# dmuley/sph-code

Hardware: AMD Instinct MI355X
Metric: particle-steps/sec + achieved HBM GB/s, 10^6-particle 3D sphere, 1/2/4/8 GPUs (higher is better)
Workload: dtype f64

## Files before the change

### include/sphx.h

```cpp
#ifndef SPHX_H
#define SPHX_H

#include <stddef.h>
#include <stdint.h>

#ifdef __cplusplus
extern "C" {
#endif

#define SPHX_OK            0
#define SPHX_E_ARG        -1
#define SPHX_E_HIP        -2
#define SPHX_E_NOMEM      -3
#define SPHX_E_STATE      -4

#define SPHX_MAX_K        64
#define SPHX_MAX_SPECIES  32

typedef struct sphx_ctx sphx_ctx;

typedef struct sphx_constants {
    double k_B;
    double amu;
    double m_h;
    double m_0;
    double dt_0;
    double max_age;
    double pos_clamp;
} sphx_constants;

typedef struct sphx_stats {
    double ms_grid;
    double ms_search;
    double ms_prep;
    double ms_density;
    double ms_pi;
    double ms_visc;
    double ms_integrate;
    double ms_total;
    int64_t n;
    int64_t steps;
    int64_t candidates;
    int64_t retries;
    int64_t cells;
    int64_t refresh_steps;
    int64_t rebuild_steps;
    double  cell_size;
    double  ms_gravity;
    int64_t fallback_queries;
    double  ms_species;
    int64_t short_rows;
    int64_t detail_steps;
    int64_t far_queries;
    int64_t outlier_levels;
    int64_t bad_accel;
    int64_t bad_energy;
    int64_t bad_state;
    int64_t bad_h;
    int64_t search_steps;
} sphx_stats;

int         sphx_create(sphx_ctx** out, int device);
void        sphx_destroy(sphx_ctx* ctx);
const char* sphx_last_error(const sphx_ctx* ctx);
int         sphx_version(void);
const char* sphx_build_info(void);
const char* sphx_tunables(const sphx_ctx* ctx);
int sphx_selftest_scan(sphx_ctx* ctx, int n, unsigned seed, long long* mismatches, int* single_launch);
int sphx_selftest_mfma_cull(sphx_ctx* ctx, double E, int blocks, unsigned seed, double* max_err_over_E2,
                            double* wrong_signs, double* kappa);
int         sphx_host_alloc(void** out, size_t bytes);
int         sphx_host_free(void* p);
int         sphx_set_constants(sphx_ctx* ctx, const sphx_constants* c);
int         sphx_get_constants(const sphx_ctx* ctx, sphx_constants* c);
int         sphx_set_tuning(sphx_ctx* ctx, double rscale, double cell_factor);
int         sphx_set_timing_detail(sphx_ctx* ctx, int on);
int         sphx_set_incremental(sphx_ctx* ctx, int verlet, double rscale_build);

int sphx_neighbors(sphx_ctx* ctx, int64_t n, int k, const double* points, double dist,
                   double eps, int64_t* idx, double* dist_out, int64_t* nontriv, double* h);

int sphx_hydro_update(sphx_ctx* ctx, int64_t n, int k, int s, const int64_t* neighbor,
                      const double* points, const double* mass, const double* sizes,
                      const double* f_un, const double* particle_type, const double* T,
                      const double* mu_array, const double* gamma_array,
                      const double* velocities, int visc_mode,
                      double* hydro_accel, double* visc_accel, double* visc_heat,
                      double* rho, double* nden, double* f_un_nb, double* rho_dust);

int sphx_density(sphx_ctx* ctx, int64_t n, int k, const double* points, const double* mass,
                 const double* particle_type, const int64_t* neighbor, double d, double* out);
int sphx_dust_density(sphx_ctx* ctx, int64_t n, int k, const double* points, const double* mass,
                      const int64_t* neighbor, const double* particle_type, const double* sizes,
                      double* out);
int sphx_num_dens(sphx_ctx* ctx, int64_t n, int k, const double* mass, const double* points,
                  const double* mu_array, const int64_t* neighbor, double d, double* out);
int sphx_del_pressure(sphx_ctx* ctx, int64_t n, int k, const double* points, const double* mass,
                      const double* particle_type, const int64_t* neighbor,
                      const double* E_internal, const double* gamma_array, double d,
                      double* out );
int sphx_artificial_viscosity(sphx_ctx* ctx, int64_t n, int k, const int64_t* neighbor,
                              const double* points, const double* particle_type,
                              const double* sizes, const double* mass, const double* densities,
                              const double* velocities, const double* T,
                              const double* gamma_array, const double* mu_array, double d,
                              double* visc_accel , double* visc_heat );
int sphx_crossing_time(sphx_ctx* ctx, int64_t n, int k, const int64_t* neighbor,
                       const double* velocities, const double* sizes,
                       const double* particle_type, double* out );
int sphx_net_impulse(sphx_ctx* ctx, int64_t n, int k, const double* points, const double* mass,
                     const double* sizes, const double* velocities, const double* particle_type,
                     const int64_t* neighbor, const double* mean_grain_mass,
                     const double* mean_cross, double* accel_onto ,
                     double* accel_reaction );

int sphx_gravity_direct(sphx_ctx* ctx, int64_t n, const double* mass, const double* points,
                        const double* sizes, double softening, double G, double* accel);

int sphx_gravity_tree(sphx_ctx* ctx, int64_t n, const double* mass, const double* points,
                      const double* sizes, double softening, double G, int ws, int k_cells,
                      double* accel);

int sphx_agb_yields(sphx_ctx* ctx, int64_t n, const double* masses, const double* metallicities,
                    int nspl, const int32_t* ntx, const int32_t* nty, const double* tx,
                    const double* ty, const double* coeffs, const int32_t* mapto, double divisor,
                    int nspecies, const double* mu_specie, const double* composition,
                    double solar_mass, double* dust_out ,
                    double* gas_out );

int sphx_dt_rule(sphx_ctx* ctx, int64_t n, const double* ct, const int32_t* first, double* dt);
int sphx_clamp_arrays(sphx_ctx* ctx, int64_t n, double* points, double* velocities);
int sphx_leapfrog(sphx_ctx* ctx, int64_t n, double* points, double* velocities, double* total_accel,
                  const double* old_accel, double* E_internal, double* T, const double* mass,
                  const double* mu, const double* gamma, const double* ptype, const double* grav_accel,
                  const double* delp, const double* densities, const double* dust_densities,
                  const double* drag_on_gas, const double* drag_reaction, const double* av_accel,
                  const double* av_heat, double dt);

int sphx_state_upload(sphx_ctx* ctx, int64_t n, int s, const double* pos, const double* vel,
                      const double* mass, const double* ptype, const double* f_un,
                      const double* T, const double* mu, const double* gamma,
                      const double* E_internal, const double* accel_old);
int sphx_state_set_drag(sphx_ctx* ctx, const double* mean_grain_mass, const double* mean_cross);
int sphx_state_set_agb(sphx_ctx* ctx, int nspl, const int32_t* ntx, const int32_t* nty, const double* tx,
                       const double* ty, const double* coeffs, const int32_t* mapto, double divisor,
                       const double* mu_specie, double solar_mass);
int sphx_state_download_species(sphx_ctx* ctx, double* F, double* Z, double* agb_dust);
int sphx_state_set_loop_forms(sphx_ctx* ctx, int on, double d);
int sphx_set_clip_grad(sphx_ctx* ctx, int on);
int sphx_set_visc_mode(sphx_ctx* ctx, int mode);
int sphx_state_set_gravity(sphx_ctx* ctx, int mode, double G);
int sphx_set_gravity_order(sphx_ctx* ctx, int order);
int sphx_step(sphx_ctx* ctx, int nsteps, int k, double dist, int first, double fixed_dt);
int sphx_state_download(sphx_ctx* ctx, double* pos, double* vel, double* accel,
                        double* E_internal, double* T, double* sizes, double* rho,
                        double* nden, double* visc_heat, double* dt_last);
int sphx_state_download_pressure(sphx_ctx* ctx, double* pressure);
int sphx_get_stats(sphx_ctx* ctx, sphx_stats* out);
int sphx_reset_stats(sphx_ctx* ctx);

int sphx_set_stream(sphx_ctx* ctx, void* hip_stream );
int sphx_reset_stream(sphx_ctx* ctx);
int sphx_sync(sphx_ctx* ctx);
int sphx_dev_set_mean_h(sphx_ctx* ctx, double mean_h);
int sphx_dev_search(sphx_ctx* ctx, int64_t n_total, int64_t n_owned, int k, const double* pos,
                    const double* hint, double rscale, double dist, double* h_out);
int sphx_dev_get_order(sphx_ctx* ctx, int64_t n_total, int32_t* out);
int sphx_dev_prep(sphx_ctx* ctx, const double* pos, const double* vel, const double* mass,
                  const double* h, const double* T, const double* mu, const double* gamma,
                  const double* ptype);
int sphx_dev_density(sphx_ctx* ctx, double* rho, double* rho_dust, double* nden, double* hydro_accel);
int sphx_dev_pi(sphx_ctx* ctx, const double* rho_complete, double* Pi, double* Bw, double* ct_out);
int sphx_dev_visc(sphx_ctx* ctx, const double* Bw_complete, const double* mass, double* visc_accel,
                  double* visc_heat);
int sphx_dev_visc_pairwise(sphx_ctx* ctx, const double* rho_complete, const double* mass, double* visc_accel,
                           double* visc_heat, double* ct_out);
int sphx_dev_clamp(sphx_ctx* ctx, int64_t n, double* pos, double* vel);
int sphx_dev_pack_rows(sphx_ctx* ctx, int64_t n, const int64_t* idx, int nf, const double* const* fields,
                       const int32_t* widths, double* rows);
int sphx_dev_regroup(sphx_ctx* ctx, int64_t n_sel, const int64_t* sel, int64_t n_rows, const double* rows,
                     int nf, const double* const* fields_in, const int32_t* widths,
                     double* const* fields_out);
int sphx_dev_need_map(sphx_ctx* ctx, int64_t n, const double* pos, const double* w, const double* g_lo,
                      double g_cs, int G, unsigned char* out);
int sphx_dev_integrate_auto(sphx_ctx* ctx, int64_t n_owned, double* pos, double* vel, double* accel_old,
                            double* E_internal, double* T, const double* mass, const double* mu,
                            const double* gamma, const double* ptype, const double* hydro_accel,
                            const double* visc_accel, const double* visc_heat, const double* red2,
                            int first, double fixed_dt, double* dt_out);
int sphx_dev_loop_prep(sphx_ctx* ctx, const double* pos, const double* vel, const double* mass, const double* T,
                       const double* mu, const double* gamma, const double* ptype, const double* E_internal, double d);
int sphx_dev_loop_pass1(sphx_ctx* ctx, const double* h_complete, double* rho, double* rho_dust, double* nden, double* delp);
int sphx_dev_loop_pass2(sphx_ctx* ctx, const double* rho_complete, double* visc_accel, double* visc_heat, double* ct_out);
int sphx_dev_loop_pass2_interior(sphx_ctx* ctx);
int sphx_dev_set_reach_cap(sphx_ctx* ctx, double cap);
int sphx_dev_select_blobs(sphx_ctx* ctx, int part);
int sphx_dev_blob_split_counts(sphx_ctx* ctx, int32_t counts[3]);
int sphx_dev_integrate_loop(sphx_ctx* ctx, int64_t n_owned, double* pos, double* vel, double* accel_old,
                            double* E_internal, double* T, const double* mass, const double* mu, const double* gamma,
                            const double* ptype, const double* delp, const double* rho, const double* av_accel,
                            const double* av_heat, const double* red2, int first, double fixed_dt, double dt,
                            double* dt_out);
int sphx_dev_drag(sphx_ctx* ctx, const double* mass, const double* ptype, const double* mean_grain_mass,
                  const double* mean_cross, double* drag_on, double* drag_reaction);
int sphx_dev_set_drag_terms(sphx_ctx* ctx, const double* drag_on, const double* drag_reaction, const double* rho,
                            const double* rho_dust);
int sphx_dev_set_agb(sphx_ctx* ctx, int nspecies, int nspl, const int32_t* ntx, const int32_t* nty, const double* tx,
                     const double* ty, const double* coeffs, const int32_t* mapto, double divisor,
                     const double* mu_specie, double solar_mass);
int sphx_dev_species(sphx_ctx* ctx, int nspecies, const double* f_un, const double* mass, double* F, double* Z,
                     double* agb_dust);
int sphx_dev_reach(sphx_ctx* ctx, int64_t n, const double* h, const double* vel, double halo_scale,
                   double skin_frac, double dt_last, double* w);
int sphx_dev_reach_dt(sphx_ctx* ctx, int64_t n, const double* h, const double* vel, double halo_scale,
                      double skin_frac, const double* dt_dev, double* w);
int sphx_dev_plan_mask(sphx_ctx* ctx, int64_t n, const double* pos, const double* g_lo, double g_cs, int G,
                       int world, int rank, const unsigned char* maps, unsigned char* mask, int64_t* counts);
int sphx_dev_step_scalars(sphx_ctx* ctx, int64_t n_owned, const double* h, const double* w_plan, double D,
                          double hclip, const double* ct, double* out4);
int sphx_dev_integrate(sphx_ctx* ctx, int64_t n_owned, double* pos, double* vel, double* accel_old,
                       double* E_internal, double* T, const double* mass, const double* mu,
                       const double* gamma, const double* ptype, const double* hydro_accel,
                       const double* visc_accel, const double* visc_heat, double dt);

#ifdef __cplusplus
}
#endif
#endif
```

### sph-code_amd/_lib.py

```python
import ctypes as C
import os
import threading
import weakref

import numpy as np

HERE = os.path.dirname(os.path.abspath(__file__))
LIB_PATH = os.environ.get("SPHX_LIB") or os.path.join(HERE, "libsphx.so")

c_double_p = C.POINTER(C.c_double)
c_int64_p = C.POINTER(C.c_int64)


class SphxConstants(C.Structure):
    _fields_ = [(n, C.c_double) for n in ("k_B", "amu", "m_h", "m_0", "dt_0", "max_age", "pos_clamp")]


class SphxStats(C.Structure):
    _fields_ = [(n, C.c_double) for n in ("ms_grid", "ms_search", "ms_prep", "ms_density", "ms_pi",
                                          "ms_visc", "ms_integrate", "ms_total")] + \
               [(n, C.c_int64) for n in ("n", "steps", "candidates", "retries", "cells", "refresh_steps",
                                         "rebuild_steps")] + \
               [("cell_size", C.c_double), ("ms_gravity", C.c_double), ("fallback_queries", C.c_int64),
                ("ms_species", C.c_double), ("short_rows", C.c_int64), ("detail_steps", C.c_int64), ("far_queries", C.c_int64),
                ("outlier_levels", C.c_int64), ("bad_accel", C.c_int64), ("bad_energy", C.c_int64), ("bad_state", C.c_int64),
                ("bad_h", C.c_int64), ("search_steps", C.c_int64)]

    def as_dict(self):
        return {n: getattr(self, n) for n, _ in self._fields_}


SPHX_E_STATE = -4
_P = C.c_void_p
_D = c_double_p
_I = c_int64_p
SIGNATURES = {
    "sphx_create": (C.c_int, [C.POINTER(_P), C.c_int]),
    "sphx_destroy": (None, [_P]),
    "sphx_last_error": (C.c_char_p, [_P]),
    "sphx_version": (C.c_int, []),
    "sphx_build_info": (C.c_char_p, []),
    "sphx_tunables": (C.c_char_p, [_P]),
    "sphx_selftest_scan": (C.c_int, [_P, C.c_int, C.c_uint, C.POINTER(C.c_longlong), C.POINTER(C.c_int)]),
    "sphx_selftest_mfma_cull": (C.c_int, [_P, C.c_double, C.c_int, C.c_uint, _D, _D, _D]),
    "sphx_host_alloc": (C.c_int, [C.POINTER(_P), C.c_size_t]),
    "sphx_host_free": (C.c_int, [_P]),
    "sphx_set_constants": (C.c_int, [_P, C.POINTER(SphxConstants)]),
    "sphx_get_constants": (C.c_int, [_P, C.POINTER(SphxConstants)]),
    "sphx_set_tuning": (C.c_int, [_P, C.c_double, C.c_double]),
    "sphx_set_incremental": (C.c_int, [_P, C.c_int, C.c_double]),
    "sphx_neighbors": (C.c_int, [_P, C.c_int64, C.c_int, _D, C.c_double, C.c_double, _I, _D, _I, _D]),
    "sphx_hydro_update": (C.c_int, [_P, C.c_int64, C.c_int, C.c_int, _I] + [_D] * 9 + [C.c_int] + [_D] * 7),
    "sphx_density": (C.c_int, [_P, C.c_int64, C.c_int, _D, _D, _D, _I, C.c_double, _D]),
    "sphx_dust_density": (C.c_int, [_P, C.c_int64, C.c_int, _D, _D, _I, _D, _D, _D]),
    "sphx_num_dens": (C.c_int, [_P, C.c_int64, C.c_int, _D, _D, _D, _I, C.c_double, _D]),
    "sphx_del_pressure": (C.c_int, [_P, C.c_int64, C.c_int, _D, _D, _D, _I, _D, _D, C.c_double, _D]),
    "sphx_artificial_viscosity": (C.c_int, [_P, C.c_int64, C.c_int, _I] + [_D] * 9 + [C.c_double, _D, _D]),
    "sphx_crossing_time": (C.c_int, [_P, C.c_int64, C.c_int, _I, _D, _D, _D, _D]),
    "sphx_net_impulse": (C.c_int, [_P, C.c_int64, C.c_int, _D, _D, _D, _D, _D, _I, _D, _D, _D, _D]),
    "sphx_agb_yields": (C.c_int, [_P, C.c_int64, _D, _D, C.c_int, C.POINTER(C.c_int32), C.POINTER(C.c_int32), _D, _D, _D,
                                  C.POINTER(C.c_int32), C.c_double, C.c_int, _D, _D, C.c_double, _D, _D]),
    "sphx_dt_rule": (C.c_int, [_P, C.c_int64, _D, C.POINTER(C.c_int32), _D]),
    "sphx_clamp_arrays": (C.c_int, [_P, C.c_int64, _D, _D]),
    "sphx_leapfrog": (C.c_int, [_P, C.c_int64] + [_D] * 18 + [C.c_double]),
    "sphx_state_upload": (C.c_int, [_P, C.c_int64, C.c_int] + [_D] * 10),
    "sphx_state_set_drag": (C.c_int, [_P, _D, _D]),
    "sphx_state_set_agb": (C.c_int, [_P, C.c_int, C.POINTER(C.c_int32), C.POINTER(C.c_int32), _D, _D, _D,
                                     C.POINTER(C.c_int32), C.c_double, _D, C.c_double]),
    "sphx_state_download_species": (C.c_int, [_P, _D, _D, _D]),
    "sphx_state_set_loop_forms": (C.c_int, [_P, C.c_int, C.c_double]),
    "sphx_set_clip_grad": (C.c_int, [_P, C.c_int]),
    "sphx_set_visc_mode": (C.c_int, [_P, C.c_int]),
    "sphx_state_set_gravity": (C.c_int, [_P, C.c_int, C.c_double]),
    "sphx_set_gravity_order": (C.c_int, [_P, C.c_int]),
    "sphx_gravity_direct": (C.c_int, [_P, C.c_int64, _D, _D, _D, C.c_double, C.c_double, _D]),
    "sphx_gravity_tree": (C.c_int, [_P, C.c_int64, _D, _D, _D, C.c_double, C.c_double, C.c_int, C.c_int, _D]),
    "sphx_step": (C.c_int, [_P, C.c_int, C.c_int, C.c_double, C.c_int, C.c_double]),
    "sphx_state_download": (C.c_int, [_P] + [_D] * 10),
    "sphx_state_download_pressure": (C.c_int, [_P, _D]),
    "sphx_get_stats": (C.c_int, [_P, C.POINTER(SphxStats)]),
    "sphx_reset_stats": (C.c_int, [_P]),
    "sphx_set_stream": (C.c_int, [_P, C.c_void_p]),
    "sphx_reset_stream": (C.c_int, [_P]),
    "sphx_sync": (C.c_int, [_P]),
    "sphx_dev_set_mean_h": (C.c_int, [_P, C.c_double]),
    "sphx_dev_search": (C.c_int, [_P, C.c_int64, C.c_int64, C.c_int, _P, _P, C.c_double, C.c_double, _P]),
    "sphx_dev_get_order": (C.c_int, [_P, C.c_int64, _P]),
    "sphx_dev_prep": (C.c_int, [_P] + [_P] * 8),
    "sphx_dev_density": (C.c_int, [_P] + [_P] * 4),
    "sphx_dev_pi": (C.c_int, [_P] + [_P] * 4),
    "sphx_dev_visc": (C.c_int, [_P] + [_P] * 4),
    "sphx_dev_visc_pairwise": (C.c_int, [_P] + [_P] * 5),
    "sphx_dev_clamp": (C.c_int, [_P, C.c_int64, _P, _P]),
    "sphx_dev_pack_rows": (C.c_int, [_P, C.c_int64, _P, C.c_int, C.POINTER(C.c_void_p), C.POINTER(C.c_int32), _P]),
    "sphx_dev_regroup": (C.c_int, [_P, C.c_int64, _P, C.c_int64, _P, C.c_int, C.POINTER(C.c_void_p),
                                   C.POINTER(C.c_int32), C.POINTER(C.c_void_p)]),
    "sphx_dev_need_map": (C.c_int, [_P, C.c_int64, _P, _P, C.POINTER(C.c_double), C.c_double, C.c_int, _P]),
    "sphx_dev_integrate_auto": (C.c_int, [_P, C.c_int64] + [_P] * 13 + [C.c_int, C.c_double, _P]),
    "sphx_dev_reach": (C.c_int, [_P, C.c_int64, _P, _P, C.c_double, C.c_double, C.c_double, _P]),
    "sphx_set_timing_detail": (C.c_int, [_P, C.c_int]),
    "sphx_dev_reach_dt": (C.c_int, [_P, C.c_int64, _P, _P, C.c_double, C.c_double, _P, _P]),
    "sphx_dev_plan_mask": (C.c_int, [_P, C.c_int64, _P, C.POINTER(C.c_double), C.c_double, C.c_int, C.c_int, C.c_int, _P, _P, _P]),
    "sphx_dev_step_scalars": (C.c_int, [_P, C.c_int64, _P, _P, C.c_double, C.c_double, _P, _P]),
    "sphx_dev_integrate": (C.c_int, [_P, C.c_int64] + [_P] * 12 + [C.c_double]),
    "sphx_dev_drag": (C.c_int, [_P] + [_P] * 6),
    "sphx_dev_set_drag_terms": (C.c_int, [_P] + [_P] * 4),
    "sphx_dev_set_agb": (C.c_int, [_P, C.c_int, C.c_int, C.POINTER(C.c_int32), C.POINTER(C.c_int32), _D, _D, _D,
                                   C.POINTER(C.c_int32), C.c_double, _D, C.c_double]),
    "sphx_dev_species": (C.c_int, [_P, C.c_int] + [_P] * 5),
    "sphx_dev_loop_prep": (C.c_int, [_P] + [_P] * 8 + [C.c_double]),
    "sphx_dev_loop_pass1": (C.c_int, [_P] + [_P] * 5),
    "sphx_dev_loop_pass2": (C.c_int, [_P] + [_P] * 4),
    "sphx_dev_loop_pass2_interior": (C.c_int, [_P]),
    "sphx_dev_set_reach_cap": (C.c_int, [_P, C.c_double]),
    "sphx_dev_select_blobs": (C.c_int, [_P, C.c_int]),
    "sphx_dev_blob_split_counts": (C.c_int, [_P, _P]),
    "sphx_dev_integrate_loop": (C.c_int, [_P, C.c_int64] + [_P] * 14 + [C.c_int, C.c_double, C.c_double, _P]),
}

_lib = None
_lock = threading.Lock()


def load_library():
    global _lib
    with _lock:
        if _lib is not None:
            return _lib
        if not os.path.exists(LIB_PATH):
            raise RuntimeError(
                "libsphx.so is not built (%s). Run `python -c 'import __graft_entry__ as g; g.build()'` "
                "or `python sph-code_amd/build.py`. There is no CPU fallback." % LIB_PATH)
        lib = C.CDLL(LIB_PATH)
        for name, (res, args) in SIGNATURES.items():
            fn = getattr(lib, name)
            fn.restype = res
            fn.argtypes = args
        _lib = lib
        return lib


def f64(a, shape=None):
    out = np.ascontiguousarray(a, dtype=np.float64)
    if shape is not None and out.shape != shape:
        raise ValueError("expected shape %s, got %s" % (shape, out.shape))
    return out


def i64(a, shape=None):
    out = np.ascontiguousarray(a, dtype=np.int64)
    if shape is not None and out.shape != shape:
        raise ValueError("expected shape %s, got %s" % (shape, out.shape))
    return out


class _PinnedPool:
    MIN_BYTES = 8 << 20
    KEEP_PER_SIZE = 3

    def __init__(self):
        self.free = {}
        self.lock = threading.Lock()

    def empty(self, shape, dtype):
        dtype = np.dtype(dtype)
        nbytes = int(np.prod(shape)) * dtype.itemsize
        if nbytes < self.MIN_BYTES:
            return np.empty(shape, dtype)
        with self.lock:
            lst = self.free.get(nbytes)
            ptr = lst.pop() if lst else None
        if ptr is None:
            lib = load_library()
            p = _P()
            if lib.sphx_host_alloc(C.byref(p), nbytes) != 0 or not p.value:
                return np.empty(shape, dtype)
            ptr = p.value
        buf = (C.c_byte * nbytes).from_address(ptr)
        weakref.finalize(buf, self._release, ptr, nbytes)
        return np.frombuffer(buf, dtype=dtype).reshape(shape)

    def _release(self, ptr, nbytes):
        with self.lock:
            lst = self.free.setdefault(nbytes, [])
            if len(lst) < self.KEEP_PER_SIZE:
                lst.append(ptr)
                return
        try:
            load_library().sphx_host_free(_P(ptr))
        except Exception:
            pass


pinned = _PinnedPool()


def dp(a):
    return None if a is None else a.ctypes.data_as(c_double_p)


def ip(a):
    return None if a is None else a.ctypes.data_as(c_int64_p)


class Context:

    def __init__(self, device=None):
        self.lib = load_library()
        if device is None:
            device = int(os.environ.get("LOCAL_RANK", "0"))
        self.device = device
        h = C.c_void_p()
        rc = self.lib.sphx_create(C.byref(h), device)
        if rc != 0 or not h:
            raise RuntimeError("sphx_create(device=%d) failed with %d: no usable MI355X/HIP device "
                               "(libsphx has no CPU path)" % (device, rc))
        self.h = h

    def close(self):
        if getattr(self, "h", None):
            self.lib.sphx_destroy(self.h)
            self.h = None

    def __del__(self):
        try:
            self.close()
        except Exception:
            pass

    def check(self, rc):
        if rc == 0:
            return
        msg = self.lib.sphx_last_error(self.h)
        msg = msg.decode() if msg else ""
        if rc == -1:
            raise ValueError("libsphx: " + msg)
        raise RuntimeError("libsphx error %d: %s" % (rc, msg))

    def constants(self):
        c = SphxConstants()
        self.check(self.lib.sphx_get_constants(self.h, C.byref(c)))
        return c

    def set_constants(self, **kw):
        c = self.constants()
        for k_, v in kw.items():
            setattr(c, k_, v)
        self.check(self.lib.sphx_set_constants(self.h, C.byref(c)))

    def set_tuning(self, rscale=0.0, cell_factor=0.0):
        self.check(self.lib.sphx_set_tuning(self.h, float(rscale), float(cell_factor)))

    def set_incremental(self, verlet=True, rscale_build=0.0):
        self.check(self.lib.sphx_set_incremental(self.h, 1 if verlet else 0, float(rscale_build)))

    def stats(self):
        s = SphxStats()
        self.check(self.lib.sphx_get_stats(self.h, C.byref(s)))
        return s.as_dict()

    def reset_stats(self):
        self.check(self.lib.sphx_reset_stats(self.h))

    def build_info(self):
        return {"library": self.lib.sphx_build_info().decode(), "tunables": self.lib.sphx_tunables(self.h).decode(),
                "lib_path": LIB_PATH}

    def set_timing_detail(self, on=True):
        self.check(self.lib.sphx_set_timing_detail(self.h, 1 if on else 0))


_default = None


def default_context():
    global _default
    if _default is None:
        _default = Context()
    return _default
```

### sph-code_amd/csrc/sphx_api.hip

```cpp
#include "sphx_internal.h"
#include <stdarg.h>
#include <stdlib.h>
#include <new>

int sphx_set_err(sphx_ctx* ctx, int code, const char* fmt, ...) {
    if (ctx) {
        va_list ap;
        va_start(ap, fmt);
        vsnprintf(ctx->err, sizeof(ctx->err), fmt, ap);
        va_end(ap);
    }
    return code;
}

void sphx_release(sphx_ctx* ctx, DevBuf& b) {
    for (size_t q = 0; q < ctx->allocs.size(); ++q)
        if (ctx->allocs[q] == b.p) { ctx->allocs[q] = ctx->allocs.back(); ctx->allocs.pop_back(); break; }
    if (b.p) (void)hipFree(b.p);
    b.p = nullptr;
    b.cap = 0;
}

int sphx_ensure(sphx_ctx* ctx, DevBuf& b, size_t bytes, hipStream_t in_use_on) {
    if (bytes == 0) bytes = 8;
    if (b.cap >= bytes) return SPHX_OK;
    if (b.p) {
        HIPCHK(hipStreamSynchronize(in_use_on));
        sphx_release(ctx, b);
    }
    size_t want = bytes + bytes / 8 + 256;
    hipError_t e = hipMalloc(&b.p, want);
    if (e != hipSuccess) {
        b.p = nullptr;
        return sphx_set_err(ctx, SPHX_E_NOMEM, "hipMalloc(%zu) failed: %s", want, hipGetErrorString(e));
    }
    b.cap = want;
    ctx->allocs.push_back(b.p);
    return SPHX_OK;
}

static void default_constants(sphx_constants* c) {
    c->k_B = 1.380649e-23;
    c->amu = 1.66053906892e-27;
    c->m_h = 1.0008 * c->amu;
    c->m_0 = 31.622776601683793 * 1.989e30;
    c->dt_0 = 60. * 60. * 24. * 365. * 250000.;
    c->max_age = 3e7 * 60. * 60. * 24. * 365.;
    c->pos_clamp = 1e11 * 149597870700.0;
}

extern "C" int sphx_version(void) { return 100; }

extern "C" const char* sphx_build_info(void) { return "gfx950 experiments=0"; }
extern "C" const char* sphx_tunables(const sphx_ctx* ctx) { return ctx ? ctx->tunables : ""; }

extern "C" int sphx_host_alloc(void** out, size_t bytes) {
    if (!out) return SPHX_E_ARG;
    *out = nullptr;
    if (bytes == 0) bytes = 8;
    if (hipHostMalloc(out, bytes, hipHostMallocDefault) != hipSuccess) {
        (void)hipGetLastError();
        *out = nullptr;
        return SPHX_E_NOMEM;
    }
    return SPHX_OK;
}
extern "C" int sphx_host_free(void* p) {
    if (p && hipHostFree(p) != hipSuccess) return SPHX_E_HIP;
    return SPHX_OK;
}

static hipError_t sphx_stream_create(hipStream_t* st, int side) {
    int least = 0, greatest = 0;
    if (hipDeviceGetStreamPriorityRange(&least, &greatest) != hipSuccess) return hipStreamCreateWithFlags(st, hipStreamNonBlocking);
    return hipStreamCreateWithPriority(st, hipStreamNonBlocking, side ? least : greatest);
}

extern "C" int sphx_create(sphx_ctx** out, int device) {
    if (!out) return SPHX_E_ARG;
    *out = nullptr;
    int count = 0;
    if (hipGetDeviceCount(&count) != hipSuccess || count <= 0 || device < 0 || device >= count) {
        fprintf(stderr, "sphx_create: no usable HIP device %d (found %d). libsphx has no CPU path.\n",
                device, count);
        return SPHX_E_HIP;
    }
    sphx_ctx* ctx = new (std::nothrow) sphx_ctx();
    if (!ctx) return SPHX_E_NOMEM;
    ctx->device = device;
    memset(&ctx->stats, 0, sizeof(ctx->stats));
    memset(&ctx->grid, 0, sizeof(ctx->grid));
    default_constants(&ctx->cst);
    auto env = [&](const char* name) -> const char* {
        const char* e = getenv(name);
        if (e) {
            const size_t used = strlen(ctx->tunables);
            snprintf(ctx->tunables + used, sizeof(ctx->tunables) - used, "%s%s=%s", used ? " " : "", name, e);
        }
        return e;
    };
    if (const char* e = env("SPHX_RSCALE")) { double v = atof(e); if (v >= 1.0) ctx->rscale = v; }
    if (const char* e = env("SPHX_CELL")) { double v = atof(e); if (v > 0.0) ctx->cell_factor = v; }
    if (const char* e = env("SPHX_RSCALE_BUILD")) { double v = atof(e); if (v >= 1.0) ctx->rscale_build = v; }
    if (const char* e = env("SPHX_VERLET")) ctx->use_verlet = atoi(e) != 0;
    if (const char* e = env("SPHX_BLOB")) ctx->use_blob = atoi(e) != 0;
    if (const char* e = env("SPHX_BLOB_CURVE")) ctx->blob_curve = atoi(e);
    if (const char* e = env("SPHX_KNN_GROUP")) ctx->use_group = atoi(e) != 0;
    if (const char* e = env("SPHX_HCLIP")) { double v = atof(e); if (v > 1.0) ctx->h_clip_factor = v; }
    if (const char* e = env("SPHX_TIMING_DETAIL")) ctx->timing_detail = atoi(e) != 0;
    if (const char* e = env("SPHX_MAX_CELLS")) { long long v = atoll(e); if (v > 0) ctx->max_cells = v; }
    if (const char* e = env("SPHX_CELL_FEEDBACK")) ctx->cell_feedback = atoi(e) != 0;
    if (const char* e = env("SPHX_CELL_FB_HI")) ctx->cell_fb_hi = atof(e);
    if (const char* e = env("SPHX_CELL_FB_LO")) ctx->cell_fb_lo = atof(e);
    if (const char* e = env("SPHX_DRAG_LDS")) ctx->drag_lds = atoi(e) != 0;
    if (const char* e = env("SPHX_BLOB_SPLIT")) ctx->blob_split_on = atoi(e) != 0;
    if (const char* e = env("SPHX_SPECIES_FUSED")) ctx->species_fused = atoi(e) != 0;
    if (const char* e = env("SPHX_SPECIES_LDS")) ctx->species_lds = atoi(e) != 0;
    if (const char* e = env("SPHX_HINT_DISTRUST")) ctx->distrust_mode = atoi(e);
    if (const char* e = env("SPHX_OUTLIER_LEVELS")) ctx->olev_mode = atoi(e);
    if (const char* e = env("SPHX_BOX_SIGMAS")) { double v = atof(e); if (v >= 1.0) ctx->box_sigmas = v; }
    if (const char* e = env("SPHX_GRAV_KERNEL")) ctx->grav_per_thread = atoi(e) == 0;
    if (const char* e = env("SPHX_GRAV_ORDER")) { int v = atoi(e); if (v == 1 || v == 2) ctx->grav_order = v; }
    if (const char* e = env("SPHX_GRAV_WS")) { int v = atoi(e); if (v >= 1 && v <= 4) ctx->grav_ws = v; }
    if (const char* e = env("SPHX_LDS")) ctx->use_lds = atoi(e) != 0;
    if (const char* e = env("SPHX_BLOB_SLOTS")) ctx->blob_slots = atoi(e);
    if (const char* e = env("SPHX_BLOB_WGS")) {
        int cus = 256;
        (void)hipDeviceGetAttribute(&cus, hipDeviceAttributeMultiprocessorCount, ctx->device);
        if (atoi(e) > 0) ctx->blob_grid = ((cus * atoi(e) + 7) / 8) * 8;
    }
    bool ok = hipSetDevice(device) == hipSuccess &&
              sphx_stream_create(&ctx->stream, 0) == hipSuccess &&
              hipHostMalloc(&ctx->pinned, 16384, hipHostMallocDefault) == hipSuccess;
    ctx->own_stream = ctx->stream;
    for (int i = 0; ok && i < 10; ++i) ok = hipEventCreate(&ctx->ev[i]) == hipSuccess;
    for (int r = 0; ok && r < 3; ++r)
        for (int i = 0; ok && i < 10; ++i) ok = hipEventCreate(&ctx->evring[r][i]) == hipSuccess;
    for (int r = 0; ok && r < 2; ++r)
        ok = hipEventCreateWithFlags(&ctx->lag_bev[r], hipEventDisableTiming) == hipSuccess &&
             hipEventCreateWithFlags(&ctx->lag_hev[r], hipEventDisableTiming) == hipSuccess;
    if (ok) ok = sphx_stream_create(&ctx->side_stream, 1) == hipSuccess &&
                 hipEventCreateWithFlags(&ctx->ev_join, hipEventDisableTiming) == hipSuccess &&
                 hipEventCreateWithFlags(&ctx->ev_perm, hipEventDisableTiming) == hipSuccess;
    if (ok) ok = sphx_ensure(ctx, ctx->scal, SC_NSLOTS * 8) == SPHX_OK &&
                 hipMemsetAsync(ctx->scal.p, 0, SC_NSLOTS * 8, ctx->stream) == hipSuccess &&
                 sphx_ensure(ctx, ctx->badc, (size_t)BADC_BUCKETS * BADC_STRIDE * sizeof(u64)) == SPHX_OK &&
                 hipMemsetAsync(ctx->badc.p, 0, (size_t)BADC_BUCKETS * BADC_STRIDE * sizeof(u64), ctx->stream) == hipSuccess;
    if (!ok) {
        fprintf(stderr, "sphx_create: HIP initialisation failed on device %d\n", device);
        delete ctx;
        return SPHX_E_HIP;
    }
    *out = ctx;
    return SPHX_OK;
}

extern "C" void sphx_destroy(sphx_ctx* ctx) {
    if (!ctx) return;
    (void)hipSetDevice(ctx->device);
    if (ctx->stream) (void)hipStreamSynchronize(ctx->stream);
    for (void* p : ctx->allocs) (void)hipFree(p);
    for (int i = 0; i < 10; ++i)
        if (ctx->ev[i]) (void)hipEventDestroy(ctx->ev[i]);
    for (int r = 0; r < 3; ++r)
        for (int i = 0; i < 10; ++i)
            if (ctx->evring[r][i]) (void)hipEventDestroy(ctx->evring[r][i]);
    for (int r = 0; r < 2; ++r) {
        if (ctx->lag_bev[r]) (void)hipEventDestroy(ctx->lag_bev[r]);
        if (ctx->lag_hev[r]) (void)hipEventDestroy(ctx->lag_hev[r]);
    }
    if (ctx->pinned) (void)hipHostFree(ctx->pinned);
    if (ctx->olev_ev) (void)hipEventDestroy(ctx->olev_ev);
    if (ctx->ev_join) (void)hipEventDestroy(ctx->ev_join);
    if (ctx->ev_perm) (void)hipEventDestroy(ctx->ev_perm);
    if (ctx->side_stream) (void)hipStreamDestroy(ctx->side_stream);
    if (ctx->own_stream) (void)hipStreamDestroy(ctx->own_stream);
    delete ctx;
}

extern "C" const char* sphx_last_error(const sphx_ctx* ctx) { return ctx ? ctx->err : "null context"; }

extern "C" int sphx_set_constants(sphx_ctx* ctx, const sphx_constants* c) {
    if (!ctx || !c) return SPHX_E_ARG;
    ctx->cst = *c;
    return SPHX_OK;
}
extern "C" int sphx_set_tuning(sphx_ctx* ctx, double rscale, double cell_factor) {
    if (!ctx) return SPHX_E_ARG;
    if (rscale > 0.0) {
        if (rscale < 1.0) return sphx_set_err(ctx, SPHX_E_ARG, "rscale %g < 1", rscale);
        ctx->rscale = rscale;
    }
    if (cell_factor > 0.0) ctx->cell_factor = cell_factor;
    return SPHX_OK;
}
extern "C" int sphx_set_incremental(sphx_ctx* ctx, int verlet, double rscale_build) {
    if (!ctx) return SPHX_E_ARG;
    ctx->use_verlet = verlet != 0;
    if (!ctx->use_verlet) ctx->list_valid = false;
    if (rscale_build > 0.0) {
        if (rscale_build < 1.0) return sphx_set_err(ctx, SPHX_E_ARG, "rscale_build %g < 1", rscale_build);
        ctx->rscale_build = rscale_build;
    }
    return SPHX_OK;
}
extern "C" int sphx_get_constants(const sphx_ctx* ctx, sphx_constants* c) {
    if (!ctx || !c) return SPHX_E_ARG;
    *c = ctx->cst;
    return SPHX_OK;
}

static int upload(sphx_ctx* ctx, DevBuf& b, const void* host, size_t bytes) {
    SPHX_TRY(sphx_ensure(ctx, b, bytes));
    HIPCHK(hipMemcpyAsync(b.p, host, bytes, hipMemcpyHostToDevice, ctx->stream));
    return SPHX_OK;
}
static int download(sphx_ctx* ctx, void* host, const void* dev, size_t bytes) {
    if (!host) return SPHX_OK;
    HIPCHK(hipMemcpyAsync(host, dev, bytes, hipMemcpyDeviceToHost, ctx->stream));
    return SPHX_OK;
}

extern "C" int sphx_neighbors(sphx_ctx* ctx, int64_t n, int k, const double* points, double dist,
                              double eps, int64_t* idx, double* dist_out, int64_t* nontriv,
                              double* h) {
    (void)eps;
    if (!ctx) return SPHX_E_ARG;
    NEED(points);
    if (n < 1) return sphx_set_err(ctx, SPHX_E_ARG, "n=%lld < 1", (long long)n);
    if (k < 1 || k > SPHX_MAX_K) return sphx_set_err(ctx, SPHX_E_ARG, "N_NEIGH=%d not in 1..%d", k, SPHX_MAX_K);
    HIPCHK(hipSetDevice(ctx->device));
    ctx->map_perm = nullptr;
    ctx->qorder = nullptr;
    const size_t nb = (size_t)n * sizeof(double);
    SPHX_TRY(upload(ctx, ctx->in_a, points, 3 * nb));
    SPHX_TRY(sphx_ensure(ctx, ctx->in_b, nb));
    SPHX_TRY(sphx_ensure(ctx, ctx->in_c, nb));
    SPHX_TRY(sphx_ensure(ctx, ctx->in_d, nb));
    SPHX_TRY(sphx_ensure(ctx, ctx->in_e, nb));
    SPHX_TRY(sphx_ensure(ctx, ctx->in_f, nb));
    SPHX_TRY(sphx_ensure(ctx, ctx->in_g, nb));
    double *x = ctx->in_b.as<double>(), *y = ctx->in_c.as<double>(), *z = ctx->in_d.as<double>();
    double *xs = ctx->in_e.as<double>(), *ys = ctx->in_f.as<double>(), *zs = ctx->in_g.as<double>();
    SPHX_TRY(sphx_aos_to_soa3(ctx, n, ctx->in_a.as<double>(), x, y, z));
    ctx->clip_valid = false;
    SPHX_TRY(sphx_build_grid(ctx, n, k, x, y, z, 0.0));
    SPHX_TRY(sphx_gather3(ctx, n, ctx->perm.as<int>(), x, y, z, xs, ys, zs));
    SPHX_TRY(sphx_ensure(ctx, ctx->idx64, (size_t)n * k * sizeof(int64_t)));
    SPHX_TRY(sphx_ensure(ctx, ctx->dist_out, (size_t)n * k * sizeof(double)));
    SPHX_TRY(sphx_ensure(ctx, ctx->nontriv, (size_t)n * sizeof(int64_t)));
    SPHX_TRY(sphx_ensure(ctx, ctx->h_api, nb));
    KnnOut o;
    o.nbr = nullptr; o.h_sorted = nullptr;
    o.idx64 = ctx->idx64.as<int64_t>(); o.dist = ctx->dist_out.as<double>();
    o.nontriv = ctx->nontriv.as<int64_t>(); o.h_by_id = ctx->h_api.as<double>();
    KnnIn in;
    in.xs = xs; in.ys = ys; in.zs = zs;
    in.id = ctx->perm.as<int>();
    in.rbound = dist;
    SPHX_TRY(sphx_knn(ctx, n, k, in, o));
    SPHX_TRY(download(ctx, idx, o.idx64, (size_t)n * k * sizeof(int64_t)));
    SPHX_TRY(download(ctx, dist_out, o.dist, (size_t)n * k * sizeof(double)));
    SPHX_TRY(download(ctx, nontriv, o.nontriv, (size_t)n * sizeof(int64_t)));
    SPHX_TRY(download(ctx, h, o.h_by_id, nb));
    HIPCHK(hipStreamSynchronize(ctx->stream));
    return SPHX_OK;
}

extern "C" int sphx_hydro_update(sphx_ctx* ctx, int64_t n, int k, int s, const int64_t* neighbor,
                                 const double* points, const double* mass, const double* sizes,
                                 const double* f_un, const double* particle_type, const double* T,
                                 const double* mu_array, const double* gamma_array,
                                 const double* velocities, int visc_mode, double* hydro_accel,
                                 double* visc_accel, double* visc_heat, double* rho, double* nden,
                                 double* f_un_nb, double* rho_dust) {
    if (!ctx) return SPHX_E_ARG;
    NEED(points); NEED(mass); NEED(sizes); NEED(particle_type); NEED(T);
// ... 141 lines not shown
    if (!ctx->has_state) return sphx_set_err(ctx, SPHX_E_STATE, "sphx_state_set_loop_forms before sphx_state_upload");
    if (on && !(d > 0.0)) return sphx_set_err(ctx, SPHX_E_ARG, "the loop forms need the driver's global d > 0 (drv:68)");
    if (on && ctx->use_verlet) return sphx_set_err(ctx, SPHX_E_STATE, "loop-form steps are not combined with incremental search");
    if (on && ctx->visc_mode != 0)
        return sphx_set_err(ctx, SPHX_E_ARG, "loop-form steps have their own (pairwise) viscosity: visc_mode must be 0");
    ctx->loop_forms = on ? 1 : 0;
    ctx->loop_d = d;
    return SPHX_OK;
}

extern "C" int sphx_set_gravity_order(sphx_ctx* ctx, int order) {
    if (!ctx) return SPHX_E_ARG;
    if (order != 1 && order != 2) return sphx_set_err(ctx, SPHX_E_ARG, "gravity order %d not 1 (monopole) or 2 (quadrupole)", order);
    ctx->grav_order = order;
    return SPHX_OK;
}

extern "C" int sphx_set_clip_grad(sphx_ctx* ctx, int on) {
    if (!ctx) return SPHX_E_ARG;
    ctx->clip_grad = on ? 1 : 0;
    return SPHX_OK;
}

extern "C" int sphx_set_visc_mode(sphx_ctx* ctx, int mode) {
    if (!ctx) return SPHX_E_ARG;
    if (mode != 0 && mode != 1)
        return sphx_set_err(ctx, SPHX_E_ARG, "visc_mode %d unknown (0 = ref_axis0, 1 = pairwise)", mode);
    if (mode != 0 && ctx->loop_forms)
        return sphx_set_err(ctx, SPHX_E_ARG, "loop-form steps have their own (pairwise) viscosity: visc_mode must be 0");
    ctx->visc_mode = mode;
    return SPHX_OK;
}

extern "C" int sphx_state_set_gravity(sphx_ctx* ctx, int mode, double G) {
    if (!ctx) return SPHX_E_ARG;
    if (!ctx->has_state) return sphx_set_err(ctx, SPHX_E_STATE, "sphx_state_set_gravity before sphx_state_upload");
    if (mode < 0 || mode > 2) return sphx_set_err(ctx, SPHX_E_ARG, "gravity mode %d not in {0, 1, 2}", mode);
    if (mode == 2 && ctx->use_verlet)
        return sphx_set_err(ctx, SPHX_E_STATE, "tree gravity needs the cell grid of every step: not with incremental search");
    ctx->gravity = mode;
    ctx->grav_G = G;
    return SPHX_OK;
}

static PrepIn prep_in_of_state(const StateArrays& s) {
    PrepIn in;
    in.x = s.x.as<double>(); in.y = s.y.as<double>(); in.z = s.z.as<double>(); in.ps = 1;
    in.vx = s.vx.as<double>(); in.vy = s.vy.as<double>(); in.vz = s.vz.as<double>(); in.vs = 1;
    in.m = s.m.as<double>(); in.h = s.hprev.as<double>(); in.T = s.T.as<double>();
    in.mu = s.mu.as<double>(); in.gam = s.gam.as<double>(); in.ptype = s.ptype.as<double>();
    return in;
}

static int step_cell_hint(sphx_ctx* ctx, int64_t n, double* cell_hint) {
    *cell_hint = 0.0;
    if (ctx->step_count == 0) return SPHX_OK;
    const double* hs;
    if (ctx->lag_hvalid[ctx->lag_hslot]) {
        HIPCHK(hipEventSynchronize(ctx->lag_halias[ctx->lag_hslot] ? ctx->lag_halias[ctx->lag_hslot]
                                                                     : ctx->lag_hev[ctx->lag_hslot]));
        hs = (const double*)((char*)ctx->pinned + LAG_OFF + 512 * ctx->lag_hslot + 256);
        const u64* sv = (const u64*)hs;
        for (int q = 0; q < 10; ++q) ctx->knn_lag[q] = sv[(SC_NFAILQ - SC_HSUM) + q];
        ctx->knn_lag_valid = true;
    } else {
        HIPCHK(hipMemcpyAsync((char*)ctx->pinned + 256, ctx->scal.as<double>() + SC_HSUM, 4 * sizeof(double),
                              hipMemcpyDeviceToHost, ctx->stream));
        HIPCHK(hipStreamSynchronize(ctx->stream));
        hs = (const double*)((char*)ctx->pinned + 256);
    }
    const double hmean = hs[3] > 0.0 ? hs[0] / hs[3] : 0.0;
    if (hmean > 0.0 && isfinite(hmean)) {
        *cell_hint = ctx->cell_factor * sphx_cell_feedback(ctx, n) * hmean;
        ctx->h_clip = ctx->h_clip_factor * hmean;
    }
    return SPHX_OK;
}

static int step_search(sphx_ctx* ctx, int k, double dist, hipEvent_t* ev) {
    const int64_t n = ctx->n;
    if (ctx->use_verlet) SPHX_TRY(sphx_clamp(ctx, n, ctx->st));
    SPHX_TRY(sphx_ensure(ctx, ctx->nbr, (size_t)k * ctx->npad * sizeof(int)));
    if (ctx->use_verlet && ctx->list_valid && ctx->list_n == n && ctx->list_k == k) {
        StateArrays& r = ctx->st;
        HIPCHK(hipEventRecord(ev[1], ctx->stream));
        int64_t nfail = 0;
        SPHX_TRY(sphx_knn_refresh(ctx, n, k, r.x.as<double>(), r.y.as<double>(), r.z.as<double>(),
                                  ctx->nbr.as<int>(), r.hprev.as<double>(), &nfail));
        if (nfail == 0) {
            ctx->stats.refresh_steps++;
            return SPHX_OK;
        }
        ctx->list_valid = false;
    }
    double cell_hint = 0.0;
    SPHX_TRY(step_cell_hint(ctx, n, &cell_hint));
    {
        StateArrays& r = ctx->st;
        const bool blob = ctx->use_blob && !ctx->use_verlet;
        GridBuildOpts g;
        g.lagged = true;
        g.alias_ev = ev[1];
        g.sort_cells_later = blob;
        if (!ctx->use_verlet) { g.clamp_vel[0] = r.vx.as<double>(); g.clamp_vel[1] = r.vy.as<double>(); g.clamp_vel[2] = r.vz.as<double>(); }
        SPHX_TRY(sphx_build_grid(ctx, n, k, r.x.as<double>(), r.y.as<double>(), r.z.as<double>(), cell_hint, g));
        if (blob) SPHX_TRY(sphx_build_blob_order(ctx, n, true));
    }
    const bool split = ctx->side_stream && !ctx->use_verlet;
    SPHX_TRY(sphx_permute_state(ctx, n, split, ev[1]));
    StateArrays& r = ctx->st;
    KnnIn in;
    in.xs = r.x.as<double>(); in.ys = r.y.as<double>(); in.zs = r.z.as<double>();
    in.id = r.id.as<int>(); in.inv = ctx->inv.as<int>();
    in.rsearch = r.hprev.as<double>();
    in.hinted = ctx->step_count > 0 && !ctx->use_verlet;
    in.lag_external = true;
    in.rscale = ctx->rscale;
    in.rbound = dist;
    KnnOut o;
    o.nbr = ctx->nbr.as<int>();
    o.h_sorted = r.hprev.as<double>();
    o.idx64 = nullptr; o.dist = nullptr; o.nontriv = nullptr; o.h_by_id = nullptr;
    if (ctx->use_verlet) {
        SPHX_TRY(sphx_ensure(ctx, ctx->list64, (size_t)n * 64 * sizeof(int)));
        SPHX_TRY(sphx_ensure(ctx, ctx->dref, (size_t)n * sizeof(double)));
        o.list64 = ctx->list64.as<int>();
        o.dref = ctx->dref.as<double>();
        in.rscale = ctx->rscale_build;
    }
    SPHX_TRY(sphx_knn(ctx, n, k, in, o));
    if (split) HIPCHK(hipStreamWaitEvent(ctx->stream, ctx->ev_perm, 0));
    if (ctx->use_verlet) {
        SPHX_TRY(sphx_save_list_positions(ctx, n, r.x.as<double>(), r.y.as<double>(), r.z.as<double>()));
        ctx->list_valid = true;
        ctx->list_n = n;
        ctx->list_k = k;
    }
    ctx->stats.rebuild_steps++;
    return SPHX_OK;
}

static int step_h_sums_out(sphx_ctx* ctx, int64_t n, const double* h, hipStream_t stream) {
    SPHX_TRY(sphx_hsum(ctx, n, h, stream));
    const int hsl = ctx->lag_hslot ^ 1;
    HIPCHK(hipMemcpyAsync((char*)ctx->pinned + LAG_OFF + 512 * hsl + 256, ctx->scal.as<double>() + SC_HSUM,
                          (SC_KGDBG + 2 - SC_HSUM + 1) * sizeof(double), hipMemcpyDeviceToHost, stream));
    HIPCHK(hipEventRecord(ctx->lag_hev[hsl], stream));
    ctx->lag_halias[hsl] = nullptr;
    ctx->lag_hvalid[hsl] = true;
    ctx->lag_hslot = hsl;
    return SPHX_OK;
}

static int step_sums(sphx_ctx* ctx, int k, hipEvent_t* ev, hipEvent_t search_end, bool detail) {
    const int64_t n = ctx->n;
    StateArrays& s = ctx->st;
    const bool pairwise = ctx->visc_mode == 1 && !ctx->loop_forms;
    const bool fork = ctx->qorder && ctx->use_lds && !ctx->loop_forms && ctx->side_stream;
    if (fork) HIPCHK(hipStreamWaitEvent(ctx->side_stream, search_end, 0));
    else SPHX_TRY(step_h_sums_out(ctx, n, s.hprev.as<double>(), ctx->stream));
    if (ctx->qorder && ctx->use_lds) SPHX_TRY(sphx_blob_translate(ctx, n, k));
    const bool species = ctx->s > 0 && ctx->fun_id.p;
    if (ctx->loop_forms) {
        if (ctx->drag || species)
            SPHX_TRY(sphx_prep(ctx, n, prep_in_of_state(s), pairwise, ctx->stream));
        if (detail) HIPCHK(hipEventRecord(ev[3], ctx->stream));
        SPHX_TRY(sphx_loop_step_sums(ctx, n, k, ctx->loop_d));
        if (detail) HIPCHK(hipEventRecord(ev[9], ctx->stream));
        if (species) SPHX_TRY(sphx_step_species(ctx, n, k));
        if (detail) HIPCHK(hipEventRecord(ev[4], ctx->stream));
        if (detail) HIPCHK(hipEventRecord(ev[5], ctx->stream));
    } else {
        SPHX_TRY(sphx_prep(ctx, n, prep_in_of_state(s), pairwise, fork ? ctx->side_stream : ctx->stream));
        if (fork) {
            HIPCHK(hipEventRecord(ctx->ev_join, ctx->side_stream));
            HIPCHK(hipStreamWaitEvent(ctx->stream, ctx->ev_join, 0));
            SPHX_TRY(step_h_sums_out(ctx, n, s.hprev.as<double>(), ctx->side_stream));
        }
        if (detail) HIPCHK(hipEventRecord(ev[3], ctx->stream));
        const bool sp_fused = species && ctx->species_fused && ctx->species_lds && ctx->use_lds && ctx->qorder && ctx->blob_lists &&
                              !ctx->map_perm && ctx->sp == 16 && ctx->s <= 16 && k <= SPHX_MAX_K;
        if (sp_fused) {
            const int S = ctx->s;
            SPHX_TRY(sphx_ensure(ctx, ctx->rho, (size_t)n * sizeof(double)));
            SPHX_TRY(sphx_ensure(ctx, ctx->rhod, (size_t)n * sizeof(double)));
            SPHX_TRY(sphx_ensure(ctx, ctx->nden, (size_t)n * sizeof(double)));
            SPHX_TRY(sphx_ensure(ctx, ctx->G, (size_t)n * 3 * sizeof(double)));
            SPHX_TRY(sphx_ensure(ctx, ctx->ha, (size_t)n * 3 * sizeof(double)));
            SPHX_TRY(sphx_ensure(ctx, ctx->F, (size_t)n * S * sizeof(double)));
            if (ctx->agb_on) {
                SPHX_TRY(sphx_ensure(ctx, ctx->Zmet, (size_t)n * sizeof(double)));
                SPHX_TRY(sphx_ensure(ctx, ctx->agb_dust, (size_t)n * S * sizeof(double)));
            }
            SPHX_TRY(sphx_blob_density_species(ctx, n, k, true, S, ctx->fun_id.as<double>(), s.id.as<int>(),
                                               s.m.as<double>(), ctx->F.as<double>(), ctx->Zmet.as<double>(),
                                               ctx->agb_dust.as<double>(), (ctx->agb_on && ctx->Zmet.p && ctx->agb_dust.p) ? 1 : 0));
        } else {
            SPHX_TRY(sphx_pass_density(ctx, n, k, true));
        }
        if (detail) HIPCHK(hipEventRecord(ev[9], ctx->stream));
        if (species && !sp_fused) SPHX_TRY(sphx_step_species(ctx, n, k));
        if (detail) HIPCHK(hipEventRecord(ev[4], ctx->stream));
        if (ctx->visc_mode == 1) {
            SPHX_TRY(sphx_pass_visc_pw(ctx, n, k, s.m.as<double>()));
        } else {
            SPHX_TRY(sphx_pass_pi(ctx, n, k, s.hprev.as<double>(), s.ptype.as<double>()));
            if (detail) HIPCHK(hipEventRecord(ev[5], ctx->stream));
            SPHX_TRY(sphx_pass_visc(ctx, n, k, s.m.as<double>()));
        }
    }
    if (ctx->drag)
        SPHX_TRY(sphx_pass_drag(ctx, n, k, s.m.as<double>(), s.ptype.as<double>(), s.mgm.as<double>(), s.mcs.as<double>()));
    return SPHX_OK;
}

static int one_step(sphx_ctx* ctx, int k, double dist, int first, double fixed_dt, bool call_first, bool call_last) {
    const int64_t n = ctx->n;
    const int ring = (int)(ctx->step_count % 3);
    hipEvent_t* ev = ctx->evring[ring];
    const bool detail = ctx->timing_detail;
    ctx->ev_detail[ring] = detail;
    const bool rec0 = detail || call_first, rec7 = detail || call_last;
    ctx->ev_has07[ring] = (rec0 ? 1 : 0) | (rec7 ? 2 : 0) | (ctx->visc_mode == 1 && !ctx->loop_forms ? 4 : 0);
    ctx->map_perm = nullptr;
    ctx->qorder = nullptr;
    ctx->blob_lists = false;
    ctx->blob_split_valid = false;
    ctx->pass_part = 0;
    ctx->nbr_api_valid = false;
    if (rec0) HIPCHK(hipEventRecord(ev[0], ctx->stream));
    SPHX_TRY(step_search(ctx, k, dist, ev));
    HIPCHK(hipEventRecord(ev[2], ctx->stream));
    SPHX_TRY(step_sums(ctx, k, ev, ev[2], detail));
    if (detail) HIPCHK(hipEventRecord(ev[6], ctx->stream));
    StateArrays& s = ctx->st;
    if (ctx->gravity) {
        SPHX_TRY(sphx_ensure(ctx, ctx->grav, (size_t)n * 3 * sizeof(double)));
        double* eps = ctx->scal.as<double>() + SC_GRAV_EPS;
        SPHX_TRY(sphx_median(ctx, n, s.hprev.as<double>(), eps));
        if (ctx->gravity == 1)
            SPHX_TRY(sphx_gravity_launch(ctx, n, s.x.as<double>(), s.y.as<double>(), s.z.as<double>(), 1,
                                         s.m.as<double>(), eps, 0.0, ctx->grav_G, nullptr, ctx->grav.as<double>()));
        else
            SPHX_TRY(sphx_gravity_tree_launch(ctx, n, s.x.as<double>(), s.y.as<double>(), s.z.as<double>(),
                                              s.m.as<double>(), ctx->grav_ws, eps, 0.0, ctx->grav_G, nullptr,
                                              ctx->grav.as<double>()));
    }
    if (detail) HIPCHK(hipEventRecord(ev[8], ctx->stream));
    SPHX_TRY(sphx_integrate(ctx, n, 1, first, fixed_dt));
    if (rec7) HIPCHK(hipEventRecord(ev[7], ctx->stream));
    ctx->step_count++;
    return SPHX_OK;
}

static int collect_stats(sphx_ctx* ctx, int ring) {
    if (!(ctx->ev_pending & (1u << ring))) return SPHX_OK;
    ctx->ev_pending &= ~(1u << ring);
    hipEvent_t* ev = ctx->evring[ring];
    const int has = ctx->ev_has07[ring];
    HIPCHK(hipEventSynchronize((has & 2) ? ev[7] : ev[2]));
    sphx_stats& st = ctx->stats;
    float ms[7] = {0.f, 0.f, 0.f, 0.f, 0.f, 0.f, 0.f};
    HIPCHK(hipEventElapsedTime(&ms[1], ev[1], ev[2]));
    st.ms_search += ms[1];
    st.steps += 1;
    st.search_steps += 1;
    st.n = ctx->n;
    if (!ctx->ev_detail[ring]) return SPHX_OK;
    float tot;
    HIPCHK(hipEventElapsedTime(&tot, ev[0], ev[7]));
    HIPCHK(hipEventElapsedTime(&ms[0], ev[0], ev[1]));
    st.ms_grid += ms[0]; st.ms_total += tot;
    for (int i = 2; i < 6; ++i) {
        if ((has & 4) && i >= 4) break;
        HIPCHK(hipEventElapsedTime(&ms[i], ev[i], ev[i + 1]));
    }
    if (has & 4) HIPCHK(hipEventElapsedTime(&ms[5], ev[4], ev[6]));
    st.ms_prep += ms[2];
    float mg = 0.f, mi = 0.f;
    HIPCHK(hipEventElapsedTime(&mg, ev[6], ev[8]));
    HIPCHK(hipEventElapsedTime(&mi, ev[8], ev[7]));
    ms[6] = mi;
    st.ms_gravity += mg;
    {
        float md = 0.f, msp = 0.f;
        HIPCHK(hipEventElapsedTime(&md, ev[3], ev[9]));
        HIPCHK(hipEventElapsedTime(&msp, ev[9], ev[4]));
        ms[3] = md;
        st.ms_species += msp;
    }
    st.ms_density += ms[3]; st.ms_pi += ms[4]; st.ms_visc += ms[5]; st.ms_integrate += ms[6];
    st.detail_steps += 1;
    return SPHX_OK;
}

extern "C" int sphx_step(sphx_ctx* ctx, int nsteps, int k, double dist, int first, double fixed_dt) {
    if (!ctx) return SPHX_E_ARG;
    if (!ctx->has_state) return sphx_set_err(ctx, SPHX_E_STATE, "sphx_step before sphx_state_upload");
    if (k < 1 || k > SPHX_MAX_K) return sphx_set_err(ctx, SPHX_E_ARG, "N_NEIGH=%d not in 1..%d", k, SPHX_MAX_K);
    if (nsteps < 1) return sphx_set_err(ctx, SPHX_E_ARG, "nsteps=%d < 1", nsteps);
    HIPCHK(hipSetDevice(ctx->device));
    if (!(dist > 0.0) || !isfinite(dist)) dist = 0.0;
    ctx->k = k;
    const bool per_call = !ctx->timing_detail;
    if (per_call) HIPCHK(hipEventRecord(ctx->ev[8], ctx->stream));
    for (int it = 0; it < nsteps; ++it) {
        const int ring = (int)(ctx->step_count % 3);
        SPHX_TRY(collect_stats(ctx, ring));
        SPHX_TRY(one_step(ctx, k, dist, first && it == 0, fixed_dt, false, false));
        ctx->ev_pending |= 1u << ring;
        SPHX_TRY(collect_stats(ctx, (ring + 1) % 3));
    }
    if (per_call) HIPCHK(hipEventRecord(ctx->ev[9], ctx->stream));
    HIPCHK(hipMemcpyAsync(ctx->pinned, ctx->scal.p, SC_NSLOTS * 8, hipMemcpyDeviceToHost, ctx->stream));
    HIPCHK(hipStreamSynchronize(ctx->stream));
    for (int r = 0; r < 3; ++r) SPHX_TRY(collect_stats(ctx, (int)((ctx->step_count + r) % 3)));
    if (per_call) {
        float tot = 0.f;
        HIPCHK(hipEventElapsedTime(&tot, ctx->ev[8], ctx->ev[9]));
        ctx->stats.ms_total += tot;
    }
    const u64* sc = (const u64*)ctx->pinned;
    ctx->dt_last = ((const double*)ctx->pinned)[SC_DT];
    ctx->stats.candidates = (int64_t)sc[SC_CAND];
    ctx->stats.retries = (int64_t)sc[SC_RETRY];
    ctx->stats.fallback_queries = (int64_t)(u32)sc[SC_NFAILQ];
    ctx->stats.short_rows = (int64_t)sc[SC_SHORT];
    SPHX_TRY(sphx_badc_read(ctx));
    return SPHX_OK;
}

extern "C" int sphx_state_download(sphx_ctx* ctx, double* pos, double* vel, double* accel,
                                   double* E_internal, double* T, double* sizes, double* rho,
                                   double* nden, double* visc_heat, double* dt_last) {
    if (!ctx) return SPHX_E_ARG;
    if (!ctx->has_state) return sphx_set_err(ctx, SPHX_E_STATE, "no state uploaded");
    HIPCHK(hipSetDevice(ctx->device));
    const int64_t n = ctx->n;
    const size_t nb = (size_t)n * sizeof(double);
    StateArrays& s = ctx->st;
    const int* id = s.id.as<int>();
    SPHX_TRY(sphx_ensure(ctx, ctx->out_a, 3 * nb));
    double* stage = ctx->out_a.as<double>();
    struct V3 { double* host; DevBuf *a, *b, *c; };
    V3 v3[] = {{pos, &s.x, &s.y, &s.z}, {vel, &s.vx, &s.vy, &s.vz}, {accel, &s.ax, &s.ay, &s.az}};
    for (V3& v : v3) {
        if (!v.host) continue;
        SPHX_TRY(sphx_soa3_to_aos_by_id(ctx, n, id, v.a->as<double>(), v.b->as<double>(), v.c->as<double>(), stage));
        SPHX_TRY(download(ctx, v.host, stage, 3 * nb));
        HIPCHK(hipStreamSynchronize(ctx->stream));
    }
    struct V1 { double* host; const double* dev; };
    const bool stepped = ctx->step_count > 0;
    V1 v1[] = {{E_internal, s.E.as<double>()}, {T, s.T.as<double>()}, {sizes, s.hprev.as<double>()},
               {rho, stepped ? ctx->rho.as<double>() : nullptr},
               {nden, stepped ? ctx->nden.as<double>() : nullptr},
               {visc_heat, stepped ? ctx->vh.as<double>() : nullptr}};
    for (V1& v : v1) {
        if (!v.host) continue;
        if (!v.dev) { memset(v.host, 0, nb); continue; }
        SPHX_TRY(sphx_scatter_rows_by_id(ctx, n, 1, id, v.dev, stage));
        SPHX_TRY(download(ctx, v.host, stage, nb));
        HIPCHK(hipStreamSynchronize(ctx->stream));
    }
    if (dt_last) *dt_last = ctx->dt_last;
    return SPHX_OK;
}

int sphx_agb_table_set(sphx_ctx* ctx, int S, int nspl, const int32_t* ntx, const int32_t* nty, const double* tx, const double* ty,
                       const double* coeffs, const int32_t* mapto, double divisor, const double* mu_specie, double solar_mass) {
    ctx->agb_on = false;
    if (nspl == 0) return SPHX_OK;
    if (S < 7 || S > AGB_MAX_SPEC) return sphx_set_err(ctx, SPHX_E_ARG, "AGB table: %d species (7..%d)", S, AGB_MAX_SPEC);
    if (!ntx || !nty || !tx || !ty || !coeffs || !mapto || !mu_specie)
        return sphx_set_err(ctx, SPHX_E_ARG, "AGB table: NULL argument");
    if (nspl < 1 || nspl > AGB_MAX_SPL) return sphx_set_err(ctx, SPHX_E_ARG, "AGB table: %d splines", nspl);
    if (!(divisor != 0.0)) return sphx_set_err(ctx, SPHX_E_ARG, "AGB table: divisor is 0");
    HIPCHK(hipSetDevice(ctx->device));
    AgbTable& t = ctx->agb;
    t.nspl = nspl; t.nspec = S;
    size_t ntx_tot = 0, nty_tot = 0, nc_tot = 0;
    for (int o = 0; o < nspl; ++o) {
        if (ntx[o] < 4 || nty[o] < 4) return sphx_set_err(ctx, SPHX_E_ARG, "AGB table: spline %d has fewer than 4 knots", o);
        if (mapto[o] < 0 || mapto[o] >= S) return sphx_set_err(ctx, SPHX_E_ARG, "AGB table: mapto[%d]=%d out of range", o, mapto[o]);
        ntx_tot += ntx[o]; nty_tot += nty[o]; nc_tot += (size_t)(ntx[o] - 2) * (nty[o] - 2);
    }
    size_t ox = 0, oy = ntx_tot, oc = ntx_tot + nty_tot;
    for (int o = 0; o < nspl; ++o) {
        t.tx_off[o] = (int)ox; t.ty_off[o] = (int)oy; t.c_off[o] = (int)oc;
        t.ntx[o] = ntx[o]; t.nty[o] = nty[o]; t.mapto[o] = mapto[o];
        ox += ntx[o]; oy += nty[o]; oc += (size_t)(ntx[o] - 2) * (nty[o] - 2);
    }
    for (int s = 0; s < S; ++s) t.mu[s] = mu_specie[s];
    t.divisor = divisor; t.solar = solar_mass;
    SPHX_TRY(sphx_ensure(ctx, ctx->agb_knots, (ntx_tot + nty_tot + nc_tot + 6 * (size_t)nspl) * sizeof(double)));
    double* kd = ctx->agb_knots.as<double>();
    {
        double meta[6 * AGB_MAX_SPL];
        t.covered = 0u;
        for (int o = 0; o < nspl; ++o) {
            bool later = false;
            for (int o2 = o + 1; o2 < nspl; ++o2) later = later || mapto[o2] == mapto[o];
// ... 112 lines not shown
```

### sph-code_amd/csrc/sphx_blob.hip

```cpp
#include "sphx_blob.h"
#include "sphx_wave.h"
#pragma clang fp contract(off)
#include <float.h>
#include <stdlib.h>
#include <stdio.h>

#define DD_TAB 2048
#define DD_PROBES 64
__device__ __forceinline__ unsigned dd_hash(int j) { return ((unsigned)j * 2654435761u) >> 21; }

__global__ __launch_bounds__(BLOB_T) void blob_dedup_kernel(int n, int npad, int k, int slots,
                                                            const int* __restrict__ nbr, u16* slot16,
                                                            int* uniq, const int* __restrict__ qorder,
                                                            const int* __restrict__ omap, int n_active,
                                                            unsigned char* bclass) {
    __builtin_amdgcn_s_setprio(DEDUP_PRIO);
    extern __shared__ u16 dd_tile[];
    __shared__ int key[DD_TAB];
    __shared__ u16 slot_of[DD_TAB];
    __shared__ int wave_tot[BLOB_T / 64];
    const int b = xcd_block(blockIdx.x, gridDim.x);
    const int t = threadIdx.x >> 1, half = threadIdx.x & 1;
    const int p = b * BLOB_P + t;
    for (int q = threadIdx.x; q < DD_TAB; q += BLOB_T) key[q] = -1;
    __syncthreads();
    {
        const int nm = (k + 1) >> 1;
        const bool live = p < n;
        int jn[DD_BATCH];
#pragma unroll
        for (int u = 0; u < DD_BATCH; ++u) {
            const int kk = 2 * u + half;
            jn[u] = (kk < k && live) ? nbr[(size_t)kk * npad + p] : -1;
        }
        for (int m0 = 0; m0 < nm; m0 += DD_BATCH) {
            int jb[DD_BATCH];
#pragma unroll
            for (int u = 0; u < DD_BATCH; ++u) {
                jb[u] = jn[u];
                const int kk = 2 * (m0 + DD_BATCH + u) + half;
                jn[u] = (kk < k && live) ? nbr[(size_t)kk * npad + p] : -1;
            }
            unsigned hb[DD_BATCH];
            int eb[DD_BATCH];
#pragma unroll
            for (int u = 0; u < DD_BATCH; ++u) {
                hb[u] = dd_hash(jb[u] < 0 ? 0 : jb[u]);
                eb[u] = key[hb[u]];
            }
#pragma unroll
            for (int u = 0; u < DD_BATCH; ++u)
                if (jb[u] >= 0 && eb[u] == -1) {
                    const int old = atomicCAS(&key[hb[u]], -1, jb[u]);
                    eb[u] = (old == -1) ? jb[u] : old;
                }
#pragma unroll
            for (int u = 0; u < DD_BATCH; ++u) {
                const int kk = 2 * (m0 + u) + half;
                if (kk >= k) continue;
                const int j = jb[u];
                unsigned s = SLOT_NONE;
                if (j >= 0) {
                    unsigned h = hb[u];
                    s = SLOT_OVER;
                    if (eb[u] == j) {
                        s = h;
                    } else {
                        for (int probe = 1; probe < DD_PROBES; ++probe) {
                            h = (h + 1) & (DD_TAB - 1);
                            int e = key[h];
                            if (e == -1) {
                                e = atomicCAS(&key[h], -1, j);
                                if (e == -1) e = j;
                            }
                            if (e == j) { s = h; break; }
                        }
                    }
                }
                dd_tile[kk * BLOB_P + t] = (u16)s;
            }
        }
    }
    __syncthreads();
    constexpr int EPT = DD_TAB / BLOB_T;
    const int e0 = threadIdx.x * EPT;
    int cnt = 0;
#pragma unroll
    for (int q = 0; q < EPT; ++q) cnt += key[e0 + q] != -1;
    const int incl = wave_scan_incl(cnt);
    const int lane = threadIdx.x & 63, wv = threadIdx.x >> 6;
    if (lane == 63) wave_tot[wv] = incl;
    __syncthreads();
    int base = incl - cnt, total = 0;
#pragma unroll
    for (int w = 0; w < BLOB_T / 64; ++w) {
        const int tw = wave_tot[w];
        if (w < wv) base += tw;
        total += tw;
    }
    int* uq = uniq + (size_t)b * BLOB_S;
    int needs_ghost = 0;
#pragma unroll
    for (int q = 0; q < EPT; ++q) {
        const int j = key[e0 + q];
        if (j != -1) {
            slot_of[e0 + q] = (u16)(base < slots ? base : SLOT_OVER);
            if (base < slots) uq[base] = j;
            ++base;
            if (bclass && omap[j] >= n_active) needs_ghost = 1;
        }
    }
    for (int q = (total < slots ? total : slots) + threadIdx.x; q < BLOB_S; q += BLOB_T) uq[q] = -1;
    __syncthreads();
    const int pieces = k * (BLOB_P / 8);
    for (int q = threadIdx.x; q < pieces; q += BLOB_T) {
        u16* src = dd_tile + q * 8;
        const int kk = q / (BLOB_P / 8), c = q % (BLOB_P / 8);
        unsigned v[8];
#pragma unroll
        for (int u = 0; u < 8; ++u) {
            const unsigned e = src[u];
            v[u] = e < DD_TAB ? (unsigned)slot_of[e] : e;
            if (v[u] == SLOT_OVER) needs_ghost = 1;
        }
        if ((size_t)b * BLOB_P + c * 8 < (size_t)npad)
            *reinterpret_cast<uint4*>(slot16 + (size_t)kk * npad + (size_t)b * BLOB_P + c * 8) =
                make_uint4(v[0] | (v[1] << 16), v[2] | (v[3] << 16), v[4] | (v[5] << 16), v[6] | (v[7] << 16));
    }
    if (bclass) {
        const int owned_q = (half == 0 && p < n && omap[qorder[p]] < n_active) ? 1 : 0;
        const int any_owned = __syncthreads_or(owned_q);
        const int any_ghost = __syncthreads_or(needs_ghost);
        if (threadIdx.x == 0) bclass[b] = (unsigned char)(!any_owned ? 2 : (any_ghost ? 1 : 0));
    }
}

#define SPLIT_T 1024
__global__ __launch_bounds__(SPLIT_T) void blob_split_kernel(int nblk, const unsigned char* __restrict__ bclass, int* list,
                                                             int* cnt) {
    __shared__ int wsum[2][SPLIT_T / 64];
    const int per = (nblk + SPLIT_T - 1) / SPLIT_T;
    const int b0 = threadIdx.x * per, b1 = (b0 + per < nblk) ? b0 + per : nblk;
    int c0 = 0, c1 = 0;
    for (int b = b0; b < b1; ++b) { const int c = bclass[b]; c0 += c == 0; c1 += c == 1; }
    const int i0 = wave_scan_incl(c0), i1 = wave_scan_incl(c1);
    const int lane = threadIdx.x & 63, wv = threadIdx.x >> 6;
    if (lane == 63) { wsum[0][wv] = i0; wsum[1][wv] = i1; }
    __syncthreads();
    int o0 = i0 - c0, o1 = i1 - c1, t0 = 0, t1 = 0;
    for (int w = 0; w < SPLIT_T / 64; ++w) {
        if (w < wv) { o0 += wsum[0][w]; o1 += wsum[1][w]; }
        t0 += wsum[0][w]; t1 += wsum[1][w];
    }
    for (int b = b0; b < b1; ++b) {
        const int c = bclass[b];
        if (c == 0) list[o0++] = b;
        else if (c == 1) list[t0 + o1++] = b;
    }
// ... 94 lines not shown
                if (m0 + NB < nm) load_slots(sl, tile, m0 + NB, half, t);
                const size_t col0 = (size_t)(LPP * m0 + half) * npad + p;
                const bool fast = all_staged(cur);
                double wo[NB];
                if (fast && !clip) density_batch<true, false>(a, wo, cur, img, rec, nbr, col0, LPP * (size_t)npad, xr, yr, zr, hi2, ci, Ai);
                else if (fast) density_batch<true, true>(a, wo, cur, img, rec, nbr, col0, LPP * (size_t)npad, xr, yr, zr, hi2, ci, Ai);
                else if (!clip) density_batch<false, false>(a, wo, cur, img, rec, nbr, col0, LPP * (size_t)npad, xr, yr, zr, hi2, ci, Ai);
                else density_batch<false, true>(a, wo, cur, img, rec, nbr, col0, LPP * (size_t)npad, xr, yr, zr, hi2, ci, Ai);
            }
            const double s_rho = group_total(a.rho), s_rd = group_total(a.rd), s_n = group_total(a.n);
            const double gx = group_total(a.gx), gy = group_total(a.gy), gz = group_total(a.gz);
            if (!half) {
                rho[o] = s_rho; rhod[o] = s_rd; nden[o] = s_n;
                rho_s[i] = s_rho;
                if (G) { G[3 * (size_t)o + 0] = -gx; G[3 * (size_t)o + 1] = -gy; G[3 * (size_t)o + 2] = -gz; }
                ha[3 * (size_t)o + 0] = -gx / s_rho;
                ha[3 * (size_t)o + 1] = -gy / s_rho;
                ha[3 * (size_t)o + 2] = -gz / s_rho;
            }
        }
        __syncthreads();
    }
}

template <bool FAST>
__device__ __forceinline__ void pi_batch(double& s_pi, double& maxrel, const unsigned (&sl)[NB], const double2* img,
                                         const double* lrho, const RecB* __restrict__ recb,
                                         const double* __restrict__ rho_s, const int* __restrict__ nbr, size_t col0,
                                         size_t colstep, const Q4& r0, const Q4& rv, double rho_i, double cs_i) {
    Q4 q0b[NB], qvb[NB];
    double rhob[NB];
#pragma unroll
    for (int u = 0; u < NB; ++u) {
        if (FAST || sl[u] < SLOT_OVER) {
            q0b[u] = lload4(img, (int)sl[u], 0); qvb[u] = lload4(img, (int)sl[u], 1);
            rhob[u] = lrho[sl[u]];
        } else if (sl[u] == SLOT_OVER) {
            const int jj = nbr[col0 + u * colstep];
            const double* qb = reinterpret_cast<const double*>(&recb[jj]);
            q0b[u] = gload4(qb); qvb[u] = gload4(qb + 4);
            rhob[u] = rho_s[jj];
        } else { q0b[u] = r0; qvb[u] = rv; rhob[u] = rho_i; }
    }
    if (FAST) __builtin_amdgcn_sched_barrier(0);
#pragma unroll
    for (int u = 0; u < NB; ++u) {
        if (!FAST && sl[u] == SLOT_NONE) continue;
        const PiPair t = pi_term<SqrtMid>(q0b[u], qvb[u], rhob[u], r0, rv, rho_i, cs_i);
        s_pi += t.pi;
        maxrel = fmax(maxrel, t.rel);
    }
}

__global__ __launch_bounds__(PASS_T, PASS_MINW) void blob_pi_kernel(int n, int npad, int k, int nblk,
                                                         const int* __restrict__ nbr,
                                                         const u16* __restrict__ slot16,
                                                         const int* __restrict__ uniq,
                                                         const int* __restrict__ qorder,
                                                         const int* __restrict__ omap, int n_active,
                                                         const RecB* __restrict__ recb,
                                                         const double* __restrict__ rho_s,
                                                         const RecSelf* __restrict__ selfr, RecBC* bc, double* Pi,
                                                         double* BwOut, u64* ct_bits, BlobSel sel) {
    extern __shared__ double2 img[];
    double* lrho = reinterpret_cast<double*>(img + 4 * BLOB_S);
    u16* tile = reinterpret_cast<u16*>(lrho + BLOB_S);
    const int t = threadIdx.x / LPP, half = threadIdx.x & (LPP - 1);
    u64 my_ct = SPHX_CT_NONE;
    const int nsel = blob_sel_count(sel, nblk);
    for (int bi = blockIdx.x; bi < nsel; bi += gridDim.x) {
        const int b = blob_sel_at(sel, bi, nsel);
        const int p = b * BLOB_P + t;
        const int i = (p < n) ? qorder[p] : 0;
        stage<1>(img, lrho, tile, recb, rho_s, 1, nullptr, 0, uniq + (size_t)b * BLOB_S, slot16, npad, k, b);
        const RecSelf sf = selfr[i];
        const double rho_i = rho_s[i];
        const double* selfq = reinterpret_cast<const double*>(&recb[i]);
        const Q4 self0 = gload4(selfq), selfv = gload4(selfq + 4);
        const int o = (p < n) ? (omap ? omap[i] : i) : 0x7FFFFFFF;
        __syncthreads();
        if (o < n_active) {
            Q4 r0 = self0, rv = selfv;
            {
                const unsigned sl0 = tile[t];
                if (sl0 < SLOT_OVER) { r0 = lload4(img, (int)sl0, 0); rv = lload4(img, (int)sl0, 1); }
                else if (sl0 == SLOT_OVER) {
                    const double* rq = reinterpret_cast<const double*>(&recb[nbr[p]]);
                    r0 = gload4(rq); rv = gload4(rq + 4);
                }
            }
            const double cs_i = sf.csi, ms_i = sf.mg, h_i = sf.h;
            double s_pi = 0.0, maxrel = 0.0;
            const int nm = KPAD(k) / LPP;
            unsigned sl[NB];
            load_slots(sl, tile, 0, half, t);
            for (int m0 = 0; m0 < nm; m0 += NB) {
                unsigned cur[NB];
#pragma unroll
                for (int u = 0; u < NB; ++u) cur[u] = sl[u];
                if (m0 + NB < nm) load_slots(sl, tile, m0 + NB, half, t);
                const size_t col0 = (size_t)(LPP * m0 + half) * npad + p;
                if (all_staged(cur))
                    pi_batch<true>(s_pi, maxrel, cur, img, lrho, recb, rho_s, nbr, col0, LPP * (size_t)npad, r0, rv, rho_i, cs_i);
                else
                    pi_batch<false>(s_pi, maxrel, cur, img, lrho, recb, rho_s, nbr, col0, LPP * (size_t)npad, r0, rv, rho_i, cs_i);
            }
            s_pi = group_total(s_pi);
            maxrel = group_max(maxrel);
            if (!half) {
                Pi[o] = s_pi;
                const double bw = fmax(ms_i, 0.0) * s_pi;
                bc[i].Bw = bw;
                if (BwOut) BwOut[o] = bw;
                if (ms_i > 0.0) {
                    const u64 cb = ct_vote_bits(h_i, maxrel);
                    my_ct = cb < my_ct ? cb : my_ct;
                }
            }
        }
        __syncthreads();
    }
    block_min_vote<PASS_T>(my_ct, ct_bits);
}

template <bool FAST, bool CLIP>
__device__ __forceinline__ void visc_batch(ViscAcc& a, const unsigned (&sl)[NB], const double2* img,
                                           const double* lc1, const RecB* __restrict__ recb,
                                           const RecBC* __restrict__ bc, const int* __restrict__ nbr, size_t col0,
                                           size_t colstep, const Q4& r0, const Q4& rv, double hi2, double ci,
                                           double Bi) {
    Q4 q0b[NB], qvb[NB];
    double c1b[NB];
#pragma unroll
    for (int u = 0; u < NB; ++u) {
        if (FAST || sl[u] < SLOT_OVER) {
            q0b[u] = lload4(img, (int)sl[u], 0); qvb[u] = lload4(img, (int)sl[u], 1);
            c1b[u] = lc1[sl[u]];
        } else if (sl[u] == SLOT_OVER) {
            const int jj = nbr[col0 + u * colstep];
            const double* qb = reinterpret_cast<const double*>(&recb[jj]);
            q0b[u] = gload4(qb); qvb[u] = gload4(qb + 4);
            const double2 tt = *reinterpret_cast<const double2*>(&bc[jj]);
            qvb[u].d = tt.x; c1b[u] = tt.y;
        } else { q0b[u] = r0; qvb[u] = rv; c1b[u] = 0.0; }
    }
    if (FAST) __builtin_amdgcn_sched_barrier(0);
#pragma unroll
    for (int u = 0; u < NB; ++u) {
        if (!FAST && sl[u] == SLOT_NONE) continue;
        visc_term<SqrtMid>(a, q0b[u], qvb[u], qvb[u].d, c1b[u], r0, rv, hi2, ci, Bi, CLIP);
    }
}

__global__ __launch_bounds__(PASS_T, PASS_MINW) void blob_visc_kernel(int n, int npad, int k, int nblk,
                                                           const int* __restrict__ nbr,
                                                           const u16* __restrict__ slot16,
                                                           const int* __restrict__ uniq,
                                                           const int* __restrict__ qorder, int clip,
                                                           const int* __restrict__ omap, int n_active,
                                                           const RecB* __restrict__ recb,
                                                           const RecBC* __restrict__ bc,
                                                           const double* __restrict__ m, double* va, double* vh,
                                                           BlobSel sel) {
    extern __shared__ double2 img[];
    double* lc1 = reinterpret_cast<double*>(img + 4 * BLOB_S);
    u16* tile = reinterpret_cast<u16*>(lc1 + BLOB_S);
    const int t = threadIdx.x / LPP, half = threadIdx.x & (LPP - 1);
    const double* bcd = reinterpret_cast<const double*>(bc);
    const int nsel = blob_sel_count(sel, nblk);
    for (int bi = blockIdx.x; bi < nsel; bi += gridDim.x) {
        const int b = blob_sel_at(sel, bi, nsel);
        const int p = b * BLOB_P + t;
        const int i = (p < n) ? qorder[p] : 0;
        stage<2>(img, lc1, tile, recb, bcd, 2, bcd + 1, 2, uniq + (size_t)b * BLOB_S, slot16, npad, k, b);
        const double2 bci = *reinterpret_cast<const double2*>(&bc[i]);
        const double* selfq = reinterpret_cast<const double*>(&recb[i]);
        const Q4 self0 = gload4(selfq), selfv = gload4(selfq + 4);
        const int o = (p < n) ? (omap ? omap[i] : i) : 0x7FFFFFFF;
        const double mi = (o < n_active) ? m[o] : 0.0;
        __syncthreads();
        if (o < n_active) {
            Q4 r0 = self0, rv = selfv;
            {
                const unsigned sl0 = tile[t];
                if (sl0 < SLOT_OVER) { r0 = lload4(img, (int)sl0, 0); rv = lload4(img, (int)sl0, 1); }
                else if (sl0 == SLOT_OVER) {
                    const double* rq = reinterpret_cast<const double*>(&recb[nbr[p]]);
                    r0 = gload4(rq); rv = gload4(rq + 4);
                }
            }
            const double hi2 = self0.d, ci = -6.0 * bci.y, Bi = bci.x;
            ViscAcc a{0.0, 0.0, 0.0, 0.0};
            const int nm = KPAD(k) / LPP;
            unsigned sl[NB];
            load_slots(sl, tile, 0, half, t);
            for (int m0 = 0; m0 < nm; m0 += NB) {
                unsigned cur[NB];
#pragma unroll
                for (int u = 0; u < NB; ++u) cur[u] = sl[u];
                if (m0 + NB < nm) load_slots(sl, tile, m0 + NB, half, t);
                const size_t col0 = (size_t)(LPP * m0 + half) * npad + p;
                const bool fast = all_staged(cur);
                if (fast && !clip) visc_batch<true, false>(a, cur, img, lc1, recb, bc, nbr, col0, LPP * (size_t)npad, r0, rv, hi2, ci, Bi);
                else if (fast) visc_batch<true, true>(a, cur, img, lc1, recb, bc, nbr, col0, LPP * (size_t)npad, r0, rv, hi2, ci, Bi);
                else if (!clip) visc_batch<false, false>(a, cur, img, lc1, recb, bc, nbr, col0, LPP * (size_t)npad, r0, rv, hi2, ci, Bi);
                else visc_batch<false, true>(a, cur, img, lc1, recb, bc, nbr, col0, LPP * (size_t)npad, r0, rv, hi2, ci, Bi);
            }
            const double ax = group_total(a.x), ay = group_total(a.y), az = group_total(a.z), heat = group_total(a.h);
            if (!half) {
                va[3 * (size_t)o + 0] = -ax; va[3 * (size_t)o + 1] = -ay; va[3 * (size_t)o + 2] = -az;
                vh[o] = heat * mi / 2.0;
            }
        }
        __syncthreads();
    }
}

template <bool FAST, bool CLIP>
__device__ __forceinline__ void visc_pw_batch(ViscAcc& a, double& maxrel, const unsigned (&sl)[NB], const double2* img,
                                              const double* lrho, const RecB* __restrict__ recb,
                                              const double* __restrict__ rho_s, const RecBC* __restrict__ bc,
                                              const int* __restrict__ nbr, size_t col0, size_t colstep, const Q4& r0,
                                              const Q4& rv, double rho_i, double cs_i, double hi2, double ci) {
    Q4 q0b[NB], qvb[NB];
    double rhob[NB], mcb[NB];
#pragma unroll
    for (int u = 0; u < NB; ++u) {
        if (FAST || sl[u] < SLOT_OVER) {
            q0b[u] = lload4(img, (int)sl[u], 0); qvb[u] = lload4(img, (int)sl[u], 1);
            rhob[u] = lrho[sl[u]];
            mcb[u] = bc[nbr[col0 + u * colstep]].Bw;
        } else if (sl[u] == SLOT_OVER) {
            const int jj = nbr[col0 + u * colstep];
            const double* qb = reinterpret_cast<const double*>(&recb[jj]);
            q0b[u] = gload4(qb); qvb[u] = gload4(qb + 4);
            rhob[u] = rho_s[jj]; mcb[u] = bc[jj].Bw;
        } else { q0b[u] = r0; qvb[u] = rv; rhob[u] = rho_i; mcb[u] = 0.0; }
    }
    if (FAST) __builtin_amdgcn_sched_barrier(0);
#pragma unroll
    for (int u = 0; u < NB; ++u) {
        if (!FAST && sl[u] == SLOT_NONE) continue;
        maxrel = fmax(maxrel, visc_pw_term<SqrtMid>(a, q0b[u], qvb[u], rhob[u], mcb[u], r0, rv, rho_i, cs_i, hi2, ci, CLIP));
    }
}

__global__ __launch_bounds__(PASS_T, PASS_MINW) void blob_visc_pw_kernel(int n, int npad, int k, int nblk,
                                                              const int* __restrict__ nbr,
                                                              const u16* __restrict__ slot16,
                                                              const int* __restrict__ uniq,
                                                              const int* __restrict__ qorder, int clip,
                                                              const int* __restrict__ omap, int n_active,
                                                              const RecB* __restrict__ recb,
                                                              const double* __restrict__ rho_s,
                                                              const RecBC* __restrict__ bc,
                                                              const RecSelf* __restrict__ selfr,
                                                              const double* __restrict__ m, double* va, double* vh,
                                                              u64* ct_bits, BlobSel sel) {
    extern __shared__ double2 img[];
    double* lrho = reinterpret_cast<double*>(img + 4 * BLOB_S);
    u16* tile = reinterpret_cast<u16*>(lrho + BLOB_S);
    const int t = threadIdx.x / LPP, half = threadIdx.x & (LPP - 1);
    u64 my_ct = SPHX_CT_NONE;
    const int nsel = blob_sel_count(sel, nblk);
    for (int bi = blockIdx.x; bi < nsel; bi += gridDim.x) {
        const int b = blob_sel_at(sel, bi, nsel);
        const int p = b * BLOB_P + t;
        const int i = (p < n) ? qorder[p] : 0;
        stage<1>(img, lrho, tile, recb, rho_s, 1, nullptr, 0, uniq + (size_t)b * BLOB_S, slot16, npad, k, b);
        const RecSelf sf = selfr[i];
        const double rho_i = rho_s[i], mci = bc[i].Bw;
        const double* selfq = reinterpret_cast<const double*>(&recb[i]);
        const Q4 self0 = gload4(selfq), selfv = gload4(selfq + 4);
        const int o = (p < n) ? (omap ? omap[i] : i) : 0x7FFFFFFF;
        const double mi = (o < n_active) ? m[o] : 0.0;
        __syncthreads();
        if (o < n_active) {
            Q4 r0 = self0, rv = selfv;
            {
                const unsigned sl0 = tile[t];
                if (sl0 < SLOT_OVER) { r0 = lload4(img, (int)sl0, 0); rv = lload4(img, (int)sl0, 1); }
                else if (sl0 == SLOT_OVER) {
                    const double* rq = reinterpret_cast<const double*>(&recb[nbr[p]]);
                    r0 = gload4(rq); rv = gload4(rq + 4);
                }
            }
            const double cs_i = sf.csi, h_i = sf.h, hi2 = self0.d, ci = -6.0 * mci;
            ViscAcc a{0.0, 0.0, 0.0, 0.0};
            double maxrel = 0.0;
            const int nm = KPAD(k) / LPP;
            unsigned sl[NB];
            load_slots(sl, tile, 0, half, t);
            for (int m0 = 0; m0 < nm; m0 += NB) {
                unsigned cur[NB];
#pragma unroll
                for (int u = 0; u < NB; ++u) cur[u] = sl[u];
                if (m0 + NB < nm) load_slots(sl, tile, m0 + NB, half, t);
                const size_t col0 = (size_t)(LPP * m0 + half) * npad + p;
                const bool fast = all_staged(cur);
                if (fast && !clip) visc_pw_batch<true, false>(a, maxrel, cur, img, lrho, recb, rho_s, bc, nbr, col0, LPP * (size_t)npad, r0, rv, rho_i, cs_i, hi2, ci);
                else if (fast) visc_pw_batch<true, true>(a, maxrel, cur, img, lrho, recb, rho_s, bc, nbr, col0, LPP * (size_t)npad, r0, rv, rho_i, cs_i, hi2, ci);
                else if (!clip) visc_pw_batch<false, false>(a, maxrel, cur, img, lrho, recb, rho_s, bc, nbr, col0, LPP * (size_t)npad, r0, rv, rho_i, cs_i, hi2, ci);
                else visc_pw_batch<false, true>(a, maxrel, cur, img, lrho, recb, rho_s, bc, nbr, col0, LPP * (size_t)npad, r0, rv, rho_i, cs_i, hi2, ci);
            }
            const double ax = group_total(a.x), ay = group_total(a.y), az = group_total(a.z), heat = group_total(a.h);
            maxrel = group_max(maxrel);
            if (!half) {
                va[3 * (size_t)o + 0] = -ax; va[3 * (size_t)o + 1] = -ay; va[3 * (size_t)o + 2] = -az;
                vh[o] = heat * mi / 2.0;
                if (sf.mg > 0.0) {
                    const u64 cb = ct_vote_bits(h_i, maxrel);
                    my_ct = cb < my_ct ? cb : my_ct;
                }
            }
        }
        __syncthreads();
    }
    block_min_vote<PASS_T>(my_ct, ct_bits);
}

template <int SPEC_MAXM>
__device__ __forceinline__ void species_sweeps(const double (&w)[SPEC_MAXM], double2* img, const u16* tile,
                                               const int* __restrict__ uq, const int* __restrict__ nbr, int n, int npad,
                                               int nm, int p, int i, int t, int half, bool live, int S,
                                               const double* __restrict__ fun, const int* __restrict__ row_of,
                                               const double* __restrict__ m, const AgbTable& agb, int agb_on, double* F,
                                               double* Zout, double* agb_out) {
    double tot[16];
#pragma unroll
    for (int hh = 0; hh < 2; ++hh) {
        __syncthreads();
        {
            int ju[NSTAGE];
#pragma unroll
            for (int r = 0; r < NSTAGE; ++r) {
                const int s = threadIdx.x + r * PASS_T;
                ju[r] = (s < BLOB_S) ? uq[s] : -1;
            }
            double2 c[NSTAGE][4];
#pragma unroll
            for (int r = 0; r < NSTAGE; ++r) {
                const int jr = ju[r] < 0 ? 0 : ju[r];
                const double2* g = reinterpret_cast<const double2*>(fun + (size_t)(row_of ? row_of[jr] : jr) * 16) + 4 * hh;
                c[r][0] = g[0]; c[r][1] = g[1]; c[r][2] = g[2]; c[r][3] = g[3];
            }
#pragma unroll
            for (int r = 0; r < NSTAGE; ++r) {
                const int s = threadIdx.x + r * PASS_T;
                if (ju[r] >= 0) {
                    img[0 * BLOB_S + s] = c[r][0]; img[1 * BLOB_S + s] = c[r][1];
                    img[2 * BLOB_S + s] = c[r][2]; img[3 * BLOB_S + s] = c[r][3];
                }
            }
        }
        __syncthreads();
        double acc[8];
#pragma unroll
        for (int q = 0; q < 8; ++q) acc[q] = 0.0;
#pragma unroll
        for (int mm = 0; mm < SPEC_MAXM; ++mm) {
            if (mm < nm) {
                const unsigned sl = tile[(LPP * mm + half) * BLOB_P + t];
                if (sl != SLOT_NONE && live) {
                    Q4 f0, f1;
// ... 165 lines not shown
                                                           const double* __restrict__ mgm,
                                                           const double* __restrict__ mcs,
                                                           const int* __restrict__ id, double* onto, DragScatter sc) {
    extern __shared__ double2 img[];
    u16* tile = reinterpret_cast<u16*>(img + (FILL ? 4 * BLOB_S : 0));
    int* cntL = reinterpret_cast<int*>(tile + KPAD(k) * BLOB_P);
    int* baseL = cntL + BLOB_S;
    unsigned char* dust = reinterpret_cast<unsigned char*>(baseL + BLOB_S);
    const int t = threadIdx.x / LPP, part = threadIdx.x & (LPP - 1);
    const int nm = KPAD(k) / LPP;
    for (int bi = blockIdx.x; bi < nblk; bi += gridDim.x) {
        const int b = xcd_block(bi, nblk);
        const int p = b * BLOB_P + t;
        const bool live = p < n;
        const int i = live ? qorder[p] : 0;
        const int* uq = uniq + (size_t)b * BLOB_S;
        if (FILL) {
            stage<0>(img, nullptr, tile, recb, nullptr, 0, nullptr, 0, uq, slot16, npad, k, b);
        } else {
            const int pieces = KPAD(k) * (BLOB_P / 8);
            for (int q = threadIdx.x; q < pieces; q += PASS_T) {
                const int kk = q / (BLOB_P / 8), c = q % (BLOB_P / 8);
                uint4 v = make_uint4(0xFFFFFFFFu, 0xFFFFFFFFu, 0xFFFFFFFFu, 0xFFFFFFFFu);
                if (kk < k) v = *reinterpret_cast<const uint4*>(slot16 + (size_t)kk * npad + (size_t)b * BLOB_P + c * 8);
                *reinterpret_cast<uint4*>(tile + kk * BLOB_P + c * 8) = v;
            }
        }
        for (int s = threadIdx.x; s < BLOB_S; s += PASS_T) {
            const int j = uq[s];
            dust[s] = (j >= 0 && ptype[j] == 2.0) ? 1 : 0;
            cntL[s] = 0;
        }
        __syncthreads();
        if (live) {
            for (int m0 = 0; m0 < nm; ++m0) {
                const int kk = LPP * m0 + part;
                const unsigned sl = tile[kk * BLOB_P + t];
                if (sl < SLOT_OVER) {
                    if (dust[sl] && uq[sl] != i) atomicAdd(&cntL[sl], 1);
                } else if (sl == SLOT_OVER && !FILL) {
                    const int j = nbr[(size_t)kk * npad + p];
                    if (j != i && ptype[j] == 2.0) atomicAdd(&sc.cnt[j], 1);
                }
            }
        }
        __syncthreads();
        if (!FILL) {
            for (int s = threadIdx.x; s < BLOB_S; s += PASS_T)
                if (cntL[s]) atomicAdd(&sc.cnt[uq[s]], cntL[s]);
            __syncthreads();
            continue;
        }
        for (int s = threadIdx.x; s < BLOB_S; s += PASS_T) {
            const int c = cntL[s];
            if (c) {
                const int j = uq[s];
                baseL[s] = sc.start[j] + atomicSub(&sc.cnt[j], c) - c;
                cntL[s] = 0;
            }
        }
        const double* rq = reinterpret_cast<const double*>(&recb[i]);
        const Q4 r0 = gload4(rq), rv = gload4(rq + 4);
        __syncthreads();
        double ox = 0.0, oy = 0.0, oz = 0.0;
        if (live) {
            unsigned dm = 0;
            for (int m0 = 0; m0 < nm; ++m0) {
                const int kk = LPP * m0 + part;
                const unsigned sl = tile[kk * BLOB_P + t];
                bool d = false;
                if (sl < SLOT_OVER) d = dust[sl] != 0;
                else if (sl == SLOT_OVER) d = ptype[nbr[(size_t)kk * npad + p]] == 2.0;
                dm |= (d ? 1u : 0u) << m0;
            }
            while (dm) {
                const int m0 = __builtin_ctz(dm);
                dm &= dm - 1;
                const int kk = LPP * m0 + part;
                const unsigned sl = tile[kk * BLOB_P + t];
                int j;
                Q4 q0, qv;
                if (sl < SLOT_OVER) {
                    j = uq[sl];
                    q0 = lload4(img, (int)sl, 0); qv = lload4(img, (int)sl, 1);
                } else {
                    j = nbr[(size_t)kk * npad + p];
                    const double* qb = reinterpret_cast<const double*>(&recb[j]);
                    q0 = gload4(qb); qv = gload4(qb + 4);
                }
                const Vec3 f = drag_term(ox, oy, oz, q0, qv, r0, rv, j, m, mgm, mcs);
                if (j != i) {
                    const int slot = (sl < SLOT_OVER) ? baseL[sl] + atomicAdd(&cntL[sl], 1)
                                                      : sc.start[j] + atomicSub(&sc.cnt[j], 1) - 1;
                    sphx_drag_put(sc, slot, ((u64)(unsigned)id[i] << 8) | (u64)kk, -f.x, -f.y, -f.z);
                }
            }
        }
        const double tx = group_total(ox), ty = group_total(oy), tz = group_total(oz);
        if (live && part == 0) { onto[3 * (size_t)i] = tx; onto[3 * (size_t)i + 1] = ty; onto[3 * (size_t)i + 2] = tz; }
        __syncthreads();
    }
}

BlobSel sphx_blob_sel(sphx_ctx* ctx, int part) {
    if (!ctx->blob_split_valid) return BlobSel{nullptr, nullptr, 0};
    const int* list = ctx->blob_split.as<int>();
    return BlobSel{list, list + (size_t)ctx->blob_split_nblk, part == 0 ? 3 : part};
}

int sphx_blob_grid(sphx_ctx* ctx, int nblk) {
    if (ctx->blob_grid <= 0) {
        int cus = 256;
        (void)hipDeviceGetAttribute(&cus, hipDeviceAttributeMultiprocessorCount, ctx->device);
        ctx->blob_grid = ((cus * 2 + 7) / 8) * 8;
    }
    return nblk < ctx->blob_grid ? nblk : ctx->blob_grid;
}

int sphx_lds_opt_in(sphx_ctx* ctx, const void* kernel, size_t bytes) {
    for (int q = 0; q < ctx->n_lds_raised; ++q)
        if (ctx->lds_raised[q] == kernel) return SPHX_OK;
    if (ctx->n_lds_raised == SPHX_LDS_KERNELS)
        return sphx_set_err(ctx, SPHX_E_HIP, "sphx_lds_opt_in: more than %d kernels", SPHX_LDS_KERNELS);
    HIPCHK(hipFuncSetAttribute(kernel, hipFuncAttributeMaxDynamicSharedMemorySize, (int)bytes));
    ctx->lds_raised[ctx->n_lds_raised++] = kernel;
    return SPHX_OK;
}

template <class Kern, class... Rest>
static int blob_launch(sphx_ctx* ctx, Kern kern, int per_slot, size_t extra, int64_t n, int k, Rest... rest) {
    const int64_t npad = sphx_pad64(n);
    const int nblk = (int)((npad + BLOB_P - 1) / BLOB_P);
    SPHX_TRY(sphx_lds_opt_in(ctx, reinterpret_cast<const void*>(kern), IMG_BYTES(per_slot, SPHX_MAX_K) + extra));
    hipLaunchKernelGGL(kern, dim3(sphx_blob_grid(ctx, nblk)), dim3(PASS_T), IMG_BYTES(per_slot, k) + extra, ctx->stream, (int)n,
                       (int)npad, k, nblk, ctx->nbr.as<int>(), ctx->slot16.as<u16>(), ctx->uniq.as<int>(), ctx->qorder, rest...);
    HIPCHK(hipGetLastError());
    return SPHX_OK;
}
static int blob_n_active(const sphx_ctx* ctx, int64_t n) { return ctx->map_perm ? ctx->map_nactive : (int)n; }

int sphx_blob_density(sphx_ctx* ctx, int64_t n, int k, bool lean) {
    return blob_launch(ctx, blob_density_kernel, 64, 0, n, k, ctx->clip_grad, ctx->map_perm, blob_n_active(ctx, n),
                       ctx->rec1.as<RecA>(), ctx->rho_s.as<double>(), ctx->rho.as<double>(), ctx->rhod.as<double>(),
                       ctx->nden.as<double>(), lean ? nullptr : ctx->G.as<double>(), ctx->ha.as<double>(),
                       sphx_blob_sel(ctx, ctx->pass_part));
}

int sphx_blob_pi(sphx_ctx* ctx, int64_t n, int k, u64* ct_bits) {
    return blob_launch(ctx, blob_pi_kernel, 72, 0, n, k, ctx->map_perm, blob_n_active(ctx, n), ctx->recv.as<RecB>(),
                       ctx->rho_s.as<double>(), ctx->self_s.as<RecSelf>(), ctx->bc_s.as<RecBC>(), ctx->Pi.as<double>(),
                       ctx->map_perm ? ctx->Bw.as<double>() : nullptr, ct_bits, sphx_blob_sel(ctx, ctx->pass_part));
}

int sphx_blob_visc(sphx_ctx* ctx, int64_t n, int k, const double* m) {
    return blob_launch(ctx, blob_visc_kernel, 72, 0, n, k, ctx->clip_grad, ctx->map_perm, blob_n_active(ctx, n),
                       ctx->recv.as<RecB>(), ctx->bc_s.as<RecBC>(), m, ctx->va.as<double>(), ctx->vh.as<double>(),
                       sphx_blob_sel(ctx, ctx->pass_part));
}

int sphx_blob_visc_pw(sphx_ctx* ctx, int64_t n, int k, const double* m, u64* ct_bits) {
    return blob_launch(ctx, blob_visc_pw_kernel, 72, 0, n, k, ctx->clip_grad, ctx->map_perm, blob_n_active(ctx, n),
                       ctx->recv.as<RecB>(), ctx->rho_s.as<double>(), ctx->bc_s.as<RecBC>(), ctx->self_s.as<RecSelf>(), m,
                       ctx->va.as<double>(), ctx->vh.as<double>(), ct_bits, sphx_blob_sel(ctx, ctx->pass_part));
}

int sphx_blob_density_species(sphx_ctx* ctx, int64_t n, int k, bool lean, int S, const double* fun, const int* row_of,
                              const double* m_sorted, double* F, double* Z, double* agb, int agb_on) {
    const auto kern = (KPAD(k) / LPP <= 10) ? blob_density_species_kernel<10> : blob_density_species_kernel<16>;
    return blob_launch(ctx, kern, 64, 0, n, k, ctx->clip_grad, ctx->rec1.as<RecA>(), ctx->rho_s.as<double>(), ctx->rho.as<double>(),
                       ctx->rhod.as<double>(), ctx->nden.as<double>(), lean ? nullptr : ctx->G.as<double>(),
                       ctx->ha.as<double>(), S, fun, row_of, m_sorted, ctx->agb, agb_on, F, Z, agb);
}

int sphx_blob_species(sphx_ctx* ctx, int64_t n, int k, int S, const double* fun, const int* row_of, const double* m_sorted, double* F,
                      double* Z, double* agb, int agb_on) {
    const auto kern = (KPAD(k) / LPP <= 10) ? blob_species_kernel<10> : blob_species_kernel<16>;
    return blob_launch(ctx, kern, 64, 0, n, k, S, ctx->rec1.as<RecA>(), fun, row_of, m_sorted, ctx->agb, agb_on, F, Z, agb);
}

int sphx_blob_drag(sphx_ctx* ctx, int64_t n, int k, bool count_only, const double* m, const double* ptype, const double* mgm,
                   const double* mcs, const int* id, double* onto, const DragScatter& sc) {
    if (count_only)
        return blob_launch(ctx, blob_drag_kernel<false>, 0, DRAG_XLDS, n, k, nullptr, m, ptype, mgm, mcs, id, onto, sc);
    return blob_launch(ctx, blob_drag_kernel<true>, 64, DRAG_XLDS, n, k, ctx->recv.as<RecB>(), m, ptype, mgm, mcs, id, onto, sc);
}
```

### sph-code_amd/csrc/sphx_integrate.hip

```cpp
#include "sphx_internal.h"
#pragma clang fp contract(off)
#include <float.h>

#include "sphx_leapfrog.h"
#define nan_to_num sphx_nan_to_num

__global__ __launch_bounds__(256) void clamp_kernel(int n, double lim, double* x, double* y, double* z,
                                                    double* vx, double* vy, double* vz) {
    int i = blockIdx.x * blockDim.x + threadIdx.x;
    if (i >= n) return;
    double* p[3] = {x, y, z};
    double* v[3] = {vx, vy, vz};
#pragma unroll
    for (int c = 0; c < 3; ++c) {
        p[c][i] = sphx_clamp_pos(p[c][i], lim);
        v[c][i] = nan_to_num(v[c][i]);
    }
}

int sphx_clamp(sphx_ctx* ctx, int64_t n, StateArrays& s) {
    hipLaunchKernelGGL(clamp_kernel, dim3((unsigned)((n + 255) / 256)), dim3(256), 0, ctx->stream, (int)n,
                       ctx->cst.pos_clamp, s.x.as<double>(), s.y.as<double>(), s.z.as<double>(),
                       s.vx.as<double>(), s.vy.as<double>(), s.vz.as<double>());
    HIPCHK(hipGetLastError());
// ... 34 lines not shown
        double2* dst = reinterpret_cast<double2*>(a.fun_dst + (size_t)t * a.s);
        for (int q = 0; q < a.s / 2; ++q) dst[q] = src[q];
    }
}

int sphx_permute_state(sphx_ctx* ctx, int64_t n, bool split, hipEvent_t after_first) {
    StateArrays& a = ctx->st;
    StateArrays& b = ctx->alt;
    DevBuf* src[] = {&a.x, &a.y, &a.z, &a.hprev, &a.vx, &a.vy, &a.vz, &a.ax, &a.ay, &a.az,
                     &a.m, &a.T, &a.mu, &a.gam, &a.E, &a.ptype};
    DevBuf* dst[] = {&b.x, &b.y, &b.z, &b.hprev, &b.vx, &b.vy, &b.vz, &b.ax, &b.ay, &b.az,
                     &b.m, &b.T, &b.mu, &b.gam, &b.E, &b.ptype};
    GatherArgs g;
    g.bs_porder = nullptr;
    if (ctx->blob_scatter_pending) {
        g.bs_g = ctx->grid; g.bs_b = ctx->blob_scatter_bits;
        g.bs_cell_of = ctx->cell_of.as<int>(); g.bs_cell_start = ctx->cell_start.as<int>();
        g.bs_mstart = ctx->blob_scatter_mstart; g.bs_porder = ctx->porder.as<int>();
        g.bs_mcount = ctx->mcount.as<int>();
        ctx->blob_scatter_pending = false;
    }
    g.n = (int)n; g.narr = 16; g.s = ctx->sp;
    g.perm = ctx->perm.as<int>();
    for (int q = 0; q < 16; ++q) {
        SPHX_TRY(sphx_ensure(ctx, *dst[q], (size_t)n * sizeof(double)));
        g.src[q] = src[q]->as<double>();
        g.dst[q] = dst[q]->as<double>();
    }
    if (ctx->drag) {
        SPHX_TRY(sphx_ensure(ctx, b.mgm, (size_t)n * sizeof(double)));
        SPHX_TRY(sphx_ensure(ctx, b.mcs, (size_t)n * sizeof(double)));
        g.src[16] = a.mgm.as<double>(); g.dst[16] = b.mgm.as<double>();
        g.src[17] = a.mcs.as<double>(); g.dst[17] = b.mcs.as<double>();
        g.narr = 18;
    }
    SPHX_TRY(sphx_ensure(ctx, b.id, (size_t)n * sizeof(int)));
    g.id_src = a.id.as<int>(); g.id_dst = b.id.as<int>(); g.inv = nullptr;
    g.fun_src = nullptr; g.fun_dst = nullptr;
    split = split && ctx->side_stream && ctx->ev_perm;
    GatherArgs rest = g;
    if (split) {
        rest.narr = g.narr - 4;
        for (int q = 0; q < rest.narr; ++q) { rest.src[q] = g.src[q + 4]; rest.dst[q] = g.dst[q + 4]; }
        rest.id_src = nullptr;
        rest.bs_porder = nullptr;
        g.narr = 4;
        g.fun_src = nullptr; g.fun_dst = nullptr;
    }
    hipLaunchKernelGGL(gather_kernel, dim3((unsigned)((n + 255) / 256)), dim3(256), 0, ctx->stream, g);
    HIPCHK(hipEventRecord(after_first, ctx->stream));
    if (split) {
        HIPCHK(hipStreamWaitEvent(ctx->side_stream, after_first, 0));
        hipLaunchKernelGGL(gather_kernel, dim3((unsigned)((n + 255) / 256)), dim3(256), 0, ctx->side_stream, rest);
        HIPCHK(hipEventRecord(ctx->ev_perm, ctx->side_stream));
    }
    HIPCHK(hipGetLastError());
    StateArrays tmp = ctx->st; ctx->st = ctx->alt; ctx->alt = tmp;
    return SPHX_OK;
}

__global__ __launch_bounds__(256) void hsum_kernel(int n, const double* h, double clip, double* partial,
                                                   unsigned* ticket, double* out_sum, double* out_cnt, u64* counters) {
    __shared__ double sm[4], sc[4];
    __shared__ bool last;
    double s = 0.0, c = 0.0;
    unsigned nbad = 0;
    for (int i = blockIdx.x * blockDim.x + threadIdx.x; i < n; i += gridDim.x * blockDim.x) {
        const double v = h[i];
        if (v > 0.0 && (clip <= 0.0 || v <= clip)) { s += v; c += 1.0; }
        nbad += (v > 0.0 && v <= DBL_MAX) ? 0u : 1u;
    }
    if (__ballot(nbad != 0u)) {
#pragma unroll
        for (int o = 32; o > 0; o >>= 1) nbad += __shfl_xor(nbad, o, 64);
        if ((threadIdx.x & 63) == 0)
            atomicAdd(&counters[(((blockIdx.x << 2) | (threadIdx.x >> 6)) & (BADC_BUCKETS - 1)) * BADC_STRIDE + BAD_H], (u64)nbad);
    }
#pragma unroll
    for (int o = 32; o > 0; o >>= 1) { s += __shfl_xor(s, o, 64); c += __shfl_xor(c, o, 64); }
    if ((threadIdx.x & 63) == 0) { sm[threadIdx.x >> 6] = s; sc[threadIdx.x >> 6] = c; }
    __syncthreads();
    if (threadIdx.x == 0) {
        partial[2 * blockIdx.x] = sm[0] + sm[1] + sm[2] + sm[3];
        partial[2 * blockIdx.x + 1] = sc[0] + sc[1] + sc[2] + sc[3];
        __threadfence();
        last = atomicInc(ticket, gridDim.x - 1) == gridDim.x - 1;
    }
    __syncthreads();
    if (last) {
        __threadfence();
        double ts = 0.0, tc = 0.0;
        for (unsigned b = threadIdx.x; b < gridDim.x; b += blockDim.x) {
            ts += __builtin_nontemporal_load(&partial[2 * b]);
            tc += __builtin_nontemporal_load(&partial[2 * b + 1]);
        }
#pragma unroll
        for (int o = 32; o > 0; o >>= 1) { ts += __shfl_xor(ts, o, 64); tc += __shfl_xor(tc, o, 64); }
        __syncthreads();
        if ((threadIdx.x & 63) == 0) { sm[threadIdx.x >> 6] = ts; sc[threadIdx.x >> 6] = tc; }
        __syncthreads();
        if (threadIdx.x == 0) {
            *out_sum = (sm[0] + sm[1]) + (sm[2] + sm[3]);
            *out_cnt = (sc[0] + sc[1]) + (sc[2] + sc[3]);
        }
    }
}
#define HSUM_BLOCKS 512
int sphx_hsum(sphx_ctx* ctx, int64_t n, const double* h, hipStream_t stream) {
    double* out = ctx->scal.as<double>() + SC_HSUM;
    double* cnt = ctx->scal.as<double>() + SC_HCNT;
    const bool fresh = ctx->hsum_tmp.p == nullptr;
    SPHX_TRY(sphx_ensure(ctx, ctx->hsum_tmp, (size_t)(2 * HSUM_BLOCKS + 2) * sizeof(double), stream));
    double* partial = ctx->hsum_tmp.as<double>();
    unsigned* ticket = reinterpret_cast<unsigned*>(partial + 2 * HSUM_BLOCKS);
    if (fresh) HIPCHK(hipMemsetAsync(ticket, 0, sizeof(double), stream));
    int blocks = (int)((n + 255) / 256);
    if (blocks > HSUM_BLOCKS) blocks = HSUM_BLOCKS;
    hipLaunchKernelGGL(hsum_kernel, dim3(blocks), dim3(256), 0, stream, (int)n, h, ctx->h_clip, partial, ticket,
                       out, cnt, ctx->badc.as<u64>());
    HIPCHK(hipGetLastError());
    return SPHX_OK;
}

__global__ void prime_ct_kernel(u64* ct_bits) { *ct_bits = SPHX_CT_NONE; }
int sphx_prime_ct(sphx_ctx* ctx, u64* ct_bits) {
    hipLaunchKernelGGL(prime_ct_kernel, dim3(1), dim3(1), 0, ctx->stream, ct_bits);
    HIPCHK(hipGetLastError());
    return SPHX_OK;
}

__global__ void dt_kernel(u64* ct_bits, double* dt_out, int first, double fixed_dt, double dt_0,
                          double max_age) {
    if (threadIdx.x != 0 || blockIdx.x != 0) return;
    double dt;
    const u64 b = *ct_bits;
    *ct_bits = SPHX_CT_NONE;
    if (fixed_dt > 0.0) {
        dt = fixed_dt;
    } else {
        const double ct = sphx_ct_value(b == SPHX_CT_NONE, __longlong_as_double((long long)b), dt_0);
        dt = sphx_dt_rule(ct, first, dt_0, max_age);
    }
    *dt_out = dt;
}

int sphx_compute_dt(sphx_ctx* ctx, int first, double fixed_dt) {
    hipLaunchKernelGGL(dt_kernel, dim3(1), dim3(64), 0, ctx->stream, ctx->scal.as<u64>() + SC_CT_BITS,
                       ctx->scal.as<double>() + SC_DT, first, fixed_dt, ctx->cst.dt_0, ctx->cst.max_age);
    HIPCHK(hipGetLastError());
    ctx->ct_primed = true;
    return SPHX_OK;
}

struct IntegArgs {
    int n;
    double *x, *y, *z, *vx, *vy, *vz, *ax, *ay, *az;
    double *E, *T;
    const double *m, *mu, *gam, *ptype;
    const double *ha, *va, *vh;
    const double *rho, *rhod, *drag_on, *drag_re;
    const double* grav;
    const double* G;
    const double* dt;
    double m_h, kB;
    int no_old;
    const u64* ct_bits;
    double* dt_out;
    int first;
    double fixed_dt, dt_0, max_age;
    u64* counters;
};
__global__ __launch_bounds__(256) void integrate_kernel(IntegArgs a) {
    int i = blockIdx.x * blockDim.x + threadIdx.x;
    if (i >= a.n) return;
    double dt;
    if (a.ct_bits) {
        if (a.fixed_dt > 0.0) {
            dt = a.fixed_dt;
        } else {
            const u64 b = *a.ct_bits;
            const double ct = sphx_ct_value(b == SPHX_CT_NONE, __longlong_as_double((long long)b), a.dt_0);
            dt = sphx_dt_rule(ct, a.first, a.dt_0, a.max_age);
        }
        if (i == 0) *a.dt_out = dt;
    } else {
        dt = *a.dt;
    }
    const double g = (a.ptype[i] == 0.0) ? 1.0 : 0.0;
    const double v[3] = {a.vx[i], a.vy[i], a.vz[i]};
    double pa[3], vis[3];
    bool bad_acc = false;
#pragma unroll
    for (int c = 0; c < 3; ++c) {
        if (a.G) {
            const double praw = a.G[3 * (size_t)i + c] / a.rho[i] * g;
            pa[c] = nan_to_num(praw);
            vis[c] = a.va[3 * (size_t)i + c];
            bad_acc = bad_acc || !sphx_finite(praw) || !sphx_finite(vis[c]);
        } else {
            const double praw = -a.ha[3 * (size_t)i + c] * g, vraw = -a.va[3 * (size_t)i + c] * g;
            pa[c] = nan_to_num(praw);
            vis[c] = nan_to_num(vraw);
            bad_acc = bad_acc || !sphx_finite(praw) || !sphx_finite(vraw);
        }
        if (a.drag_on) {
            const double draw = a.drag_on[3 * (size_t)i + c] * a.rhod[i] / a.rho[i] * g, rraw = a.drag_re[3 * (size_t)i + c];
            const double dg = nan_to_num(draw);
            vis[c] = dg + nan_to_num(rraw) + vis[c];
            bad_acc = bad_acc || !sphx_finite(draw) || !sphx_finite(rraw);
        }
    }
    double x[3] = {a.x[i], a.y[i], a.z[i]};
    double vv[3] = {v[0], v[1], v[2]};
    double gr[3], old[3], tot[3];
#pragma unroll
    for (int c = 0; c < 3; ++c) gr[c] = a.grav ? a.grav[3 * (size_t)i + c] : 0.0;
    old[0] = a.ax[i]; old[1] = a.ay[i]; old[2] = a.az[i];
    sphx_leapfrog_update(dt, x, vv, vis, pa, a.grav ? gr : nullptr, a.no_old ? nullptr : old, tot);
    a.x[i] = x[0]; a.y[i] = x[1]; a.z[i] = x[2];
    a.vx[i] = vv[0]; a.vy[i] = vv[1]; a.vz[i] = vv[2];
    a.ax[i] = tot[0]; a.ay[i] = tot[1]; a.az[i] = tot[2];
    double E = a.E[i], T;
    const double heat = a.vh[i];
    const bool bad_en = !sphx_finite(E) || !sphx_finite(heat * dt);
    sphx_energy_update(dt, heat, a.mu[i], a.gam[i], a.m[i], a.m_h, a.kB, E, T);
    a.E[i] = E;
    a.T[i] = T;
    if (a.counters) {
        bool bad_st = false;
#pragma unroll
        for (int c = 0; c < 3; ++c) bad_st = bad_st || !sphx_finite(x[c]) || !sphx_finite(vv[c]);
        sphx_count_bad(a.counters, BAD_ACCEL, bad_acc);
        sphx_count_bad(a.counters, BAD_ENERGY, bad_en);
        sphx_count_bad(a.counters, BAD_STATE, bad_st);
    }
}

int sphx_integrate(sphx_ctx* ctx, int64_t n, int fold_dt, int first, double fixed_dt) {
    StateArrays& s = ctx->st;
    IntegArgs a;
    a.ct_bits = fold_dt ? ctx->scal.as<u64>() + SC_CT_BITS : nullptr;
    a.dt_out = ctx->scal.as<double>() + SC_DT;
    a.first = first; a.fixed_dt = fixed_dt; a.dt_0 = ctx->cst.dt_0; a.max_age = ctx->cst.max_age;
    a.n = (int)n;
    a.x = s.x.as<double>(); a.y = s.y.as<double>(); a.z = s.z.as<double>();
    a.vx = s.vx.as<double>(); a.vy = s.vy.as<double>(); a.vz = s.vz.as<double>();
    a.ax = s.ax.as<double>(); a.ay = s.ay.as<double>(); a.az = s.az.as<double>();
    SPHX_TRY(sphx_ensure(ctx, ctx->alt.T, (size_t)n * sizeof(double)));
    a.E = s.E.as<double>(); a.T = ctx->alt.T.as<double>();
    a.m = s.m.as<double>(); a.mu = s.mu.as<double>(); a.gam = s.gam.as<double>();
    a.ptype = s.ptype.as<double>();
    a.ha = ctx->ha.as<double>(); a.va = ctx->va.as<double>(); a.vh = ctx->vh.as<double>();
    a.rho = ctx->rho.as<double>(); a.rhod = ctx->rhod.as<double>();
    a.drag_on = ctx->drag ? ctx->drag_on.as<double>() : nullptr;
    a.drag_re = ctx->drag ? ctx->drag_re.as<double>() : nullptr;
    a.grav = ctx->gravity ? ctx->grav.as<double>() : nullptr;
    a.G = ctx->loop_forms ? ctx->G.as<double>() : nullptr;
    a.dt = ctx->scal.as<double>() + SC_DT;
    a.m_h = ctx->cst.m_h; a.kB = ctx->cst.k_B;
    a.no_old = 0;
    a.counters = ctx->badc.as<u64>();
    hipLaunchKernelGGL(integrate_kernel, dim3((unsigned)((n + 255) / 256)), dim3(256), 0, ctx->stream, a);
    HIPCHK(hipGetLastError());
    { DevBuf t = s.T; s.T = ctx->alt.T; ctx->alt.T = t; }
    ctx->tprev_valid = true;
    return SPHX_OK;
}

__global__ __launch_bounds__(256) void pressure_by_id(int n, const int* id, const double* nden, const double* T, double kB,
                                                      double* out) {
    const int t = blockIdx.x * blockDim.x + threadIdx.x;
    if (t < n) out[id[t]] = nden[t] * kB * T[t];
}
extern "C" int sphx_state_download_pressure(sphx_ctx* ctx, double* pressure) {
    if (!ctx || !pressure) return SPHX_E_ARG;
    if (!ctx->has_state) return sphx_set_err(ctx, SPHX_E_STATE, "no state uploaded");
    HIPCHK(hipSetDevice(ctx->device));
    const int64_t n = ctx->n;
    if (ctx->step_count < 1 || !ctx->tprev_valid || !ctx->alt.T.p) { memset(pressure, 0, (size_t)n * sizeof(double)); return SPHX_OK; }
    SPHX_TRY(sphx_ensure(ctx, ctx->out_a, (size_t)n * sizeof(double)));
    hipLaunchKernelGGL(pressure_by_id, dim3((unsigned)((n + 255) / 256)), dim3(256), 0, ctx->stream, (int)n,
                       ctx->st.id.as<int>(), ctx->nden.as<double>(), ctx->alt.T.as<double>(), ctx->cst.k_B, ctx->out_a.as<double>());
    HIPCHK(hipGetLastError());
    HIPCHK(hipMemcpyAsync(pressure, ctx->out_a.p, (size_t)n * sizeof(double), hipMemcpyDeviceToHost, ctx->stream));
    HIPCHK(hipStreamSynchronize(ctx->stream));
    return SPHX_OK;
}

__global__ __launch_bounds__(256) void dt_rule_kernel(int n, const double* ct, const int* first, double dt_0,
                                                      double max_age, double* out) {
    int i = blockIdx.x * blockDim.x + threadIdx.x;
    if (i < n) out[i] = sphx_dt_rule(ct[i], first[i], dt_0, max_age);
}
static int up_(sphx_ctx* ctx, DevBuf& b, const void* host, size_t bytes) {
    SPHX_TRY(sphx_ensure(ctx, b, bytes));
    HIPCHK(hipMemcpyAsync(b.p, host, bytes, hipMemcpyHostToDevice, ctx->stream));
    return SPHX_OK;
}

extern "C" int sphx_dt_rule(sphx_ctx* ctx, int64_t n, const double* ct, const int32_t* first, double* dt) {
    if (!ctx) return SPHX_E_ARG;
    NEED(ct); NEED(first); NEED(dt);
    if (n < 1) return SPHX_OK;
    HIPCHK(hipSetDevice(ctx->device));
    SPHX_TRY(up_(ctx, ctx->in_a, ct, (size_t)n * 8));
    SPHX_TRY(up_(ctx, ctx->in_b, first, (size_t)n * 4));
    SPHX_TRY(sphx_ensure(ctx, ctx->out_a, (size_t)n * 8));
    hipLaunchKernelGGL(dt_rule_kernel, dim3((unsigned)((n + 255) / 256)), dim3(256), 0, ctx->stream, (int)n,
                       ctx->in_a.as<double>(), ctx->in_b.as<int>(), ctx->cst.dt_0, ctx->cst.max_age, ctx->out_a.as<double>());
    HIPCHK(hipGetLastError());
    HIPCHK(hipMemcpyAsync(dt, ctx->out_a.p, (size_t)n * 8, hipMemcpyDeviceToHost, ctx->stream));
    HIPCHK(hipStreamSynchronize(ctx->stream));
    return SPHX_OK;
}

__global__ __launch_bounds__(256) void clamp_aos_kernel(int n3, double lim, double* pos, double* vel) {
    int e = blockIdx.x * blockDim.x + threadIdx.x;
    if (e >= n3) return;
    pos[e] = sphx_clamp_pos(pos[e], lim);
    vel[e] = nan_to_num(vel[e]);
}
extern "C" int sphx_clamp_arrays(sphx_ctx* ctx, int64_t n, double* points, double* velocities) {
    if (!ctx) return SPHX_E_ARG;
    NEED(points); NEED(velocities);
    if (n < 1) return SPHX_OK;
    HIPCHK(hipSetDevice(ctx->device));
    const size_t nb3 = (size_t)n * 24;
    SPHX_TRY(up_(ctx, ctx->in_a, points, nb3));
    SPHX_TRY(up_(ctx, ctx->in_b, velocities, nb3));
    hipLaunchKernelGGL(clamp_aos_kernel, dim3((unsigned)((3 * n + 255) / 256)), dim3(256), 0, ctx->stream, (int)(3 * n),
                       ctx->cst.pos_clamp, ctx->in_a.as<double>(), ctx->in_b.as<double>());
    HIPCHK(hipGetLastError());
    HIPCHK(hipMemcpyAsync(points, ctx->in_a.p, nb3, hipMemcpyDeviceToHost, ctx->stream));
    HIPCHK(hipMemcpyAsync(velocities, ctx->in_b.p, nb3, hipMemcpyDeviceToHost, ctx->stream));
    HIPCHK(hipStreamSynchronize(ctx->stream));
    return SPHX_OK;
}

extern "C" int sphx_leapfrog(sphx_ctx* ctx, int64_t n, double* points, double* velocities, double* total_accel,
                             const double* old_accel, double* E_internal, double* T, const double* mass,
                             const double* mu, const double* gamma, const double* ptype, const double* grav_accel,
                             const double* delp, const double* densities, const double* dust_densities,
                             const double* drag_on_gas, const double* drag_reaction, const double* av_accel,
                             const double* av_heat, double dt) {
    if (!ctx) return SPHX_E_ARG;
    NEED(points); NEED(velocities); NEED(total_accel); NEED(E_internal); NEED(T); NEED(mass); NEED(mu);
    NEED(gamma); NEED(ptype); NEED(delp); NEED(densities); NEED(av_accel); NEED(av_heat);
    if ((drag_on_gas != nullptr) != (drag_reaction != nullptr) || (drag_on_gas && !dust_densities))
        return sphx_set_err(ctx, SPHX_E_ARG, "sphx_leapfrog: drag needs drag_on_gas, drag_reaction and dust_densities");
    if (n < 1) return SPHX_OK;
    if (n > 0x7FFFFFF0ll) return sphx_set_err(ctx, SPHX_E_ARG, "n=%lld out of range", (long long)n);
    HIPCHK(hipSetDevice(ctx->device));
    const size_t nb = (size_t)n * 8;
    DevBuf& w = ctx->out_b;
    SPHX_TRY(sphx_ensure(ctx, w, 40 * nb));
    double* base = w.as<double>();
    size_t off = 0;
    auto take = [&](size_t cols) { double* q = base + off; off += cols * (size_t)n; return q; };
    double *x = take(1), *y = take(1), *z = take(1), *vx = take(1), *vy = take(1), *vz = take(1);
    double *ax = take(1), *ay = take(1), *az = take(1), *E = take(1), *Tt = take(1);
    double *m = take(1), *muu = take(1), *gm = take(1), *pt = take(1), *rho = take(1), *rhod = take(1), *heat = take(1);
    double *aos = take(3), *G = take(3), *av = take(3), *gr = take(3), *don = take(3), *dre = take(3);
    auto h2d = [&](double* d, const double* h, size_t cols) {
        return hipMemcpyAsync(d, h, cols * nb, hipMemcpyHostToDevice, ctx->stream);
    };
    HIPCHK(h2d(aos, points, 3));
    SPHX_TRY(sphx_aos_to_soa3(ctx, n, aos, x, y, z));
    HIPCHK(hipStreamSynchronize(ctx->stream));
    HIPCHK(h2d(aos, velocities, 3));
    SPHX_TRY(sphx_aos_to_soa3(ctx, n, aos, vx, vy, vz));
    HIPCHK(hipStreamSynchronize(ctx->stream));
    if (old_accel) {
        HIPCHK(h2d(aos, old_accel, 3));
        SPHX_TRY(sphx_aos_to_soa3(ctx, n, aos, ax, ay, az));
        HIPCHK(hipStreamSynchronize(ctx->stream));
    }
    HIPCHK(h2d(E, E_internal, 1)); HIPCHK(h2d(m, mass, 1)); HIPCHK(h2d(muu, mu, 1)); HIPCHK(h2d(gm, gamma, 1));
    HIPCHK(h2d(pt, ptype, 1)); HIPCHK(h2d(rho, densities, 1)); HIPCHK(h2d(heat, av_heat, 1));
    HIPCHK(h2d(G, delp, 3)); HIPCHK(h2d(av, av_accel, 3));
    if (dust_densities) HIPCHK(h2d(rhod, dust_densities, 1));
    if (grav_accel) HIPCHK(h2d(gr, grav_accel, 3));
    if (drag_on_gas) { HIPCHK(h2d(don, drag_on_gas, 3)); HIPCHK(h2d(dre, drag_reaction, 3)); }
    double* dtd = ctx->scal.as<double>() + 15;
    HIPCHK(hipMemcpyAsync(dtd, &dt, 8, hipMemcpyHostToDevice, ctx->stream));
    IntegArgs a;
    a.ct_bits = nullptr; a.dt_out = nullptr; a.first = 0; a.fixed_dt = 0.0; a.dt_0 = 0.0; a.max_age = 0.0;
    a.n = (int)n;
    a.x = x; a.y = y; a.z = z; a.vx = vx; a.vy = vy; a.vz = vz; a.ax = ax; a.ay = ay; a.az = az;
    a.E = E; a.T = Tt; a.m = m; a.mu = muu; a.gam = gm; a.ptype = pt;
    a.ha = nullptr; a.va = av; a.vh = heat; a.rho = rho; a.rhod = rhod;
    a.drag_on = drag_on_gas ? don : nullptr; a.drag_re = drag_on_gas ? dre : nullptr;
    a.grav = grav_accel ? gr : nullptr;
    a.G = G;
    a.dt = dtd;
    a.m_h = ctx->cst.m_h; a.kB = ctx->cst.k_B;
    a.no_old = old_accel ? 0 : 1;
    a.counters = nullptr;
    hipLaunchKernelGGL(integrate_kernel, dim3((unsigned)((n + 255) / 256)), dim3(256), 0, ctx->stream, a);
    HIPCHK(hipGetLastError());
    struct Out { double* host; double *a, *b, *c; } outs[] = {{points, x, y, z}, {velocities, vx, vy, vz}, {total_accel, ax, ay, az}};
    for (Out& o : outs) {
        SPHX_TRY(sphx_soa3_to_aos_by_id(ctx, n, nullptr, o.a, o.b, o.c, aos));
        HIPCHK(hipMemcpyAsync(o.host, aos, 3 * nb, hipMemcpyDeviceToHost, ctx->stream));
        HIPCHK(hipStreamSynchronize(ctx->stream));
    }
    HIPCHK(hipMemcpyAsync(E_internal, E, nb, hipMemcpyDeviceToHost, ctx->stream));
    HIPCHK(hipMemcpyAsync(T, Tt, nb, hipMemcpyDeviceToHost, ctx->stream));
    HIPCHK(hipStreamSynchronize(ctx->stream));
    return SPHX_OK;
}

__global__ __launch_bounds__(256) void aos_to_soa3(int n, const double* aos, double* x, double* y, double* z) {
    int i = blockIdx.x * blockDim.x + threadIdx.x;
    if (i >= n) return;
    x[i] = aos[3 * (size_t)i]; y[i] = aos[3 * (size_t)i + 1]; z[i] = aos[3 * (size_t)i + 2];
}
int sphx_aos_to_soa3(sphx_ctx* ctx, int64_t n, const double* aos, double* x, double* y, double* z) {
    hipLaunchKernelGGL(aos_to_soa3, dim3((unsigned)((n + 255) / 256)), dim3(256), 0, ctx->stream, (int)n, aos, x, y, z);
// ... 50 lines not shown
```

### sph-code_amd/csrc/sphx_internal.h

```cpp
#pragma once
#include <hip/hip_runtime.h>
#include <stdint.h>
#include <stdio.h>
#include <string.h>
#include <math.h>
#include <float.h>
#include <vector>
#include "../../include/sphx.h"
#include "sphx_agb.h"

#define SPHX_WAVE 64
#define SPHX_W6_C 1.5666814710608448

typedef unsigned long long u64;
typedef unsigned int u32;

struct DevBuf {
    void* p = nullptr;
    size_t cap = 0;
    template <class T> T* as() const { return (T*)p; }
};

struct __attribute__((aligned(64))) RecA {
    double x, y, z;
    double h2;
    double c1;
    double ms;
    double A;
    double Nw;
};
struct __attribute__((aligned(64))) RecB {
    double x, y, z, h2;
    double vx, vy, vz;
    double cs;
};
struct __attribute__((aligned(16))) RecBC {
    double Bw;
    double c1;
};
struct __attribute__((aligned(32))) RecSelf {
    double csi;
    double h;
    double mg;
    double pad;
};

struct GridParams {
    double xmin, ymin, zmin;
    double cell, inv_cell;
    int nx, ny, nz;
    int ncells;
    float fnx1, fny1, fnz1;
};

#define OLEV_N 32
#define OLEV_MAX 20
#define OLEV_MIN_RC 8.0f
struct OutLevels {
    int L;
    double cx, cy, cz;
    double hmax;
    const int* start;
    const int* list;
};
__device__ __forceinline__ bool sphx_outside_box(const GridParams& g, double x, double y, double z) {
    const double tx = (x - g.xmin) * g.inv_cell, ty = (y - g.ymin) * g.inv_cell, tz = (z - g.zmin) * g.inv_cell;
    return tx < 0.0 || tx >= (double)g.nx || ty < 0.0 || ty >= (double)g.ny || tz < 0.0 || tz >= (double)g.nz;
}

struct BlobBits { int bx, by, bz; int hilbert; };
__device__ __forceinline__ unsigned hilbert_rank(unsigned x, unsigned y, unsigned z, int b) {
    unsigned X[3] = {x, y, z};
    const unsigned M = 1u << (b - 1);
    for (unsigned Q = M; Q > 1; Q >>= 1) {
        const unsigned P = Q - 1;
#pragma unroll
        for (int i = 0; i < 3; ++i) {
            if (X[i] & Q) X[0] ^= P;
            else { const unsigned t = (X[0] ^ X[i]) & P; X[0] ^= t; X[i] ^= t; }
        }
    }
    X[1] ^= X[0]; X[2] ^= X[1];
    unsigned t = 0;
    for (unsigned Q = M; Q > 1; Q >>= 1)
        if (X[2] & Q) t ^= Q - 1;
    X[0] ^= t; X[1] ^= t; X[2] ^= t;
    unsigned out = 0;
    for (int q = 0; q < b; ++q) {
        out |= ((X[2] >> q) & 1u) << (3 * q);
        out |= ((X[1] >> q) & 1u) << (3 * q + 1);
        out |= ((X[0] >> q) & 1u) << (3 * q + 2);
    }
    return out;
}
__device__ __forceinline__ unsigned blob_rank(int cx, int cy, int cz, BlobBits b) {
    if (b.hilbert) return hilbert_rank((unsigned)cx, (unsigned)cy, (unsigned)cz, b.hilbert);
    unsigned out = 0;
    int pos = 0;
    for (int q = 0; q < 11; ++q) {
        if (q < b.bx) out |= (unsigned)((cx >> q) & 1) << pos++;
        if (q < b.by) out |= (unsigned)((cy >> q) & 1) << pos++;
        if (q < b.bz) out |= (unsigned)((cz >> q) & 1) << pos++;
    }
    return out;
}

struct StateArrays {
    DevBuf x, y, z, vx, vy, vz, ax, ay, az;
    DevBuf m, T, mu, gam, E, hprev;
    DevBuf ptype;
    DevBuf id;
    DevBuf fun;
    DevBuf mgm, mcs;
};

#define SPHX_LDS_KERNELS 16

struct sphx_ctx {
    int device = 0;
    hipStream_t stream = nullptr;
    hipStream_t own_stream = nullptr;
    hipStream_t side_stream = nullptr;
    sphx_constants cst;
    char tunables[1024] = {0};
    double rscale = 1.08, cell_factor = 0.55;
    double rscale_build = 1.3;
    bool use_verlet = false;
    bool use_blob = true;
    int blob_curve = 0;
    bool use_group = true;
    bool use_lds = true;
    bool drag_lds = true;
    bool blob_split_on = true;
    bool species_lds = true;
    bool species_fused = true;
    int blob_grid = 0;
    int blob_slots = 1 << 20;
    int olev_mode = 2;
    int distrust_mode = 0;
    bool cell_feedback = true;
    double cell_fb_hi = 0.30, cell_fb_lo = 0.10;
    int64_t max_cells = 0;
    double box_sigmas = 3.0;
    double h_clip_factor = 8.0;
    double reach_cap = 0.0;
    bool timing_detail = false;
    int clip_grad = 0;
    int visc_mode = 0;
    bool drag = false;
    int loop_forms = 0;
    double loop_d = 0.0;
    int gravity = 0;
    double grav_G = 0.0;
    int grav_order = 2;
    bool grav_per_thread = false;
    int grav_ws = 1;
    bool agb_on = false;
    AgbTable agb;
    double dev_hmean = 0.0;

    char err[512] = {0};
    sphx_stats stats;
    int64_t n = 0, npad = 0;
    int k = 0, s = 0;
    int sp = 0;
    bool has_state = false;
    int64_t step_count = 0;
    double dt_last = 0.0;
    bool tprev_valid = false;
    bool ct_primed = false;
    bool recs_pw = false;
    bool nbr_api_valid = false;
    int64_t nbr_api_n = 0;
    int nbr_api_k = 0;
    bool list_valid = false;
    int64_t list_n = 0;
    int list_k = 0;
    const int* map_perm = nullptr;
    int map_nactive = 0;
    const int* qorder = nullptr;
    bool blob_lists = false;
    bool blob_split_valid = false;
    int blob_split_nblk = 0;
    int pass_part = 0;
    bool loop2_interior_done = false;
    bool dev_ev_pending = false;
    const double *dev_drag_on = nullptr, *dev_drag_re = nullptr, *dev_drag_rho = nullptr, *dev_drag_rhod = nullptr;
    GridParams grid;
    const double* tbox = nullptr;
    double tbox_h[6] = {0, 0, 0, 0, 0, 0};
    double clip_lo[3] = {0, 0, 0}, clip_hi[3] = {0, 0, 0};
    bool clip_valid = false;
    double h_clip = 0.0;
    double cell_scale = 1.0;
    bool cells_unsorted = false;
    bool blob_scatter_pending = false;
    BlobBits blob_scatter_bits;
    const int* blob_scatter_mstart = nullptr;
    bool bbox_ticket_zeroed = false;
    const void* cell_fill_zeroed = nullptr;
    const void* mcount_zeroed = nullptr;
    int mcount_zeroed_M = 0;
    const void* fcount_zeroed = nullptr;
    int64_t fcount_zeroed_n = 0;
    const void* ds_cnt_zeroed = nullptr;
    const void* olev_fill_zeroed = nullptr;
    unsigned lbs_epoch[2] = {0u, 0u};
    const void* lds_raised[SPHX_LDS_KERNELS] = {nullptr};
    int n_lds_raised = 0;
    OutLevels olev;
    bool olev_ev_valid = false;
    u64 farq_seen = 0;
    int64_t farq_last = 0;
    int64_t list_len_last = 0;
    bool knn_lag_valid = false;
    u64 knn_lag[10] = {0, 0, 0, 0, 0, 0, 0, 0, 0, 0};
    u64 densep_seen = 0;
    int64_t densep_last = 0;
    u64 crowded_seen = 0;
    int64_t crowded_last = 0;
    bool distrust = false;
    u64 badhint_seen = 0;
    bool ev_detail[3] = {false, false, false};
    int ev_has07[3] = {0, 0, 0};
    unsigned ev_pending = 0;
    hipEvent_t lag_balias[2] = {nullptr, nullptr}, lag_halias[2] = {nullptr, nullptr};
    bool lag_bvalid[2] = {false, false}, lag_hvalid[2] = {false, false};
    int64_t lag_bn[2] = {0, 0};
    int lag_bslot = 0, lag_hslot = 0;

    std::vector<void*> allocs;
    DevBuf rec1, recv;
    DevBuf rho_s, bc_s, self_s;
    DevBuf drag_on, drag_re;
    DevBuf need_pyr;
    DevBuf fun_id;
    DevBuf crowded;
    DevBuf loop_side;
    DevBuf ds_cnt, ds_start, ds_ent;
    DevBuf lrec_a, lrec_v;
    DevBuf grav, grav_sort, grav_tmp;
    DevBuf grav_pyr, grav_cell;
    DevBuf grav_quad;
    DevBuf list64, dref, pos0, pos4;
    DevBuf nbr;
    DevBuf porder, mcount, mstart;
    DevBuf agb_knots, Zmet, agb_dust;
    DevBuf fail_list;
    DevBuf olev_start, olev_fill, olev_list, olev_key;
    DevBuf lbs_state[2];
    DevBuf cell_rank;
    DevBuf tie_list;
    DevBuf slot16, uniq;
    DevBuf blob_class, blob_split;
    DevBuf rho, rhod, nden, G, Pi, Bw, va, vh, ha, F;
    DevBuf scal;
    DevBuf cell_of, cell_start, cell_fill, perm, inv, scan_tmp, bbox_tmp;
    DevBuf in_a, in_b, in_c, in_d, in_e, in_f, in_g, in_h, in_i, in_j, out_a, out_b, out_c;
    DevBuf idx64, dist_out, nontriv, h_api;
    StateArrays st, alt;
    DevBuf badc;
    DevBuf scal_tmp;
    DevBuf hsum_tmp;
    hipEvent_t ev_join = nullptr;
    hipEvent_t ev_perm = nullptr;
    hipEvent_t olev_ev = nullptr;
    hipEvent_t ev[10] = {nullptr};
    hipEvent_t evring[3][10] = {{nullptr}};
    hipEvent_t lag_bev[2] = {nullptr, nullptr}, lag_hev[2] = {nullptr, nullptr};
    void* pinned = nullptr;
};

int sphx_set_err(sphx_ctx* ctx, int code, const char* fmt, ...);
int sphx_ensure(sphx_ctx* ctx, DevBuf& b, size_t bytes, hipStream_t in_use_on);
static inline int sphx_ensure(sphx_ctx* ctx, DevBuf& b, size_t bytes) { return sphx_ensure(ctx, b, bytes, ctx->stream); }
void sphx_release(sphx_ctx* ctx, DevBuf& b);

#define HIPCHK(expr)                                                                         \
    do {                                                                                     \
        hipError_t e_ = (expr);                                                              \
        if (e_ != hipSuccess)                                                                \
            return sphx_set_err(ctx, SPHX_E_HIP, "%s:%d %s -> %s", __FILE__, __LINE__,       \
                                #expr, hipGetErrorString(e_));                               \
    } while (0)
#define NEED(p)                                                                              \
    do {                                                                                     \
        if (!(p)) return sphx_set_err(ctx, SPHX_E_ARG, "%s: argument %s is NULL", __func__, #p); \
    } while (0)
#define SPHX_TRY(expr)                                                                       \
    do {                                                                                     \
        int r_ = (expr);                                                                     \
        if (r_ != SPHX_OK) return r_;                                                        \
    } while (0)

static inline int64_t sphx_pad64(int64_t n) { return (n + 63) & ~int64_t(63); }

__device__ __forceinline__ int xcd_block(int b, int nb) {
    const int q = nb >> 3, r = nb & 7, x = b & 7, s = b >> 3;
    return x * q + (x < r ? x : r) + s;
}

#ifndef SPHX_SUM_PARTS
#define SPHX_SUM_PARTS 4
#endif

#define LAG_OFF 1024

__device__ __forceinline__ double sphx_nan_to_num(double v) {
    if (v != v) return 0.0;
    if (v > DBL_MAX) return DBL_MAX;
    if (v < -DBL_MAX) return -DBL_MAX;
    return v;
}

#define SPHX_CT_NONE 0x7FF0000000000000ull
int sphx_prime_ct(sphx_ctx* ctx, u64* ct_bits);

enum {
    SC_CT_BITS = 0,
    SC_DT = 1,
    SC_CAND = 2,
    SC_RETRY = 3,
    SC_HSUM = 4,
    SC_DISP2 = 5,
    SC_NFAIL = 6,
    SC_HCNT = 7,
    SC_GRAV_EPS = 8,
    SC_NFAILQ = 9,
    SC_SHORT = 10,
    SC_FARQ = 11,
    SC_BADHINT = 12,
    SC_CROWDED = 13,
    SC_DENSEP = 14,
    SC_KGDBG = 16,
    SC_NSLOTS = 24
};

enum {
    BAD_ACCEL = 0,
    BAD_ENERGY = 1,
    BAD_STATE = 2,
    BAD_H = 3,
    BADC_BUCKETS = 64, BADC_STRIDE = 16
};
int sphx_badc_read(sphx_ctx* ctx);

int sphx_bbox(sphx_ctx* ctx, int64_t n, const double* x, const double* y, const double* z,
              double out_minmax[13], bool use_clip);
int sphx_median(sphx_ctx* ctx, int64_t n, const double* v, double* out_dev);
int sphx_gravity_launch(sphx_ctx* ctx, int64_t n, const double* x, const double* y, const double* z, int ps,
                        const double* m, const double* eps_dev, double eps, double G, const int* omap,
                        double* acc);
int sphx_gravity_tree_launch(sphx_ctx* ctx, int64_t n, const double* x, const double* y, const double* z,
                             const double* m, int ws, const double* eps_dev, double eps, double G, const int* omap,
                             double* acc);
int sphx_dev_collect(sphx_ctx* ctx);
int sphx_loop_step_sums(sphx_ctx* ctx, int64_t n, int k, double d);
int sphx_build_blob_order(sphx_ctx* ctx, int64_t n, bool defer_scatter = false);
static inline double sphx_cell_feedback(sphx_ctx* ctx, int64_t n) {
    if (ctx->cell_feedback && n > 0) {
        const double dense = (double)ctx->densep_last / (double)n;
        if (dense > ctx->cell_fb_hi) ctx->cell_scale = ctx->cell_scale * 0.97 > 0.35 ? ctx->cell_scale * 0.97 : 0.35;
        else if (dense < ctx->cell_fb_lo) ctx->cell_scale = ctx->cell_scale * 1.01 < 1.0 ? ctx->cell_scale * 1.01 : 1.0;
    }
    return ctx->cell_scale;
}
int sphx_blob_translate(sphx_ctx* ctx, int64_t n, int k);
int sphx_blob_density_species(sphx_ctx* ctx, int64_t n, int k, bool lean, int S, const double* fun, const int* row_of,
                              const double* m_sorted, double* F, double* Z, double* agb, int agb_on);
int sphx_blob_density(sphx_ctx* ctx, int64_t n, int k, bool lean);
int sphx_blob_pi(sphx_ctx* ctx, int64_t n, int k, u64* ct_bits);
int sphx_blob_visc(sphx_ctx* ctx, int64_t n, int k, const double* m);
int sphx_blob_visc_pw(sphx_ctx* ctx, int64_t n, int k, const double* m, u64* ct_bits);
int sphx_blob_species(sphx_ctx* ctx, int64_t n, int k, int S, const double* fun, const int* row_of, const double* m_sorted, double* F,
                      double* Z, double* agb, int agb_on);
struct GridBuildOpts {
    bool lagged = false;
    hipEvent_t alias_ev = nullptr;
    bool sort_cells_later = false;
    double* clamp_vel[3] = {nullptr, nullptr, nullptr};
};
int sphx_build_grid(sphx_ctx* ctx, int64_t n, int k, const double* x, const double* y, const double* z, double cell_hint,
                    const GridBuildOpts& opts = GridBuildOpts());
int sphx_excl_scan_int(sphx_ctx* ctx, const int* in, int* out, int n);
struct alignas(32) DragEntry { u64 key; double x, y, z; };
struct DragScatter { int* cnt; const int* start; DragEntry* ent; };
__device__ __forceinline__ void sphx_drag_put(const DragScatter& sc, int slot, u64 key, double x, double y, double z) {
    double2* q = reinterpret_cast<double2*>(sc.ent + slot);
    q[0] = make_double2(__longlong_as_double((long long)key), x);
    q[1] = make_double2(y, z);
}
int sphx_drag_scatter_plan(sphx_ctx* ctx, int64_t n, int k, const int* nbr, const double* ptype, const int* qorder, DragScatter* out,
                           bool blob = false);
int sphx_drag_scatter_reduce(sphx_ctx* ctx, int64_t n, const DragScatter& d, double* react);
int sphx_blob_drag(sphx_ctx* ctx, int64_t n, int k, bool count_only, const double* m, const double* ptype, const double* mgm,
                   const double* mcs, const int* id, double* onto, const DragScatter& sc);
int sphx_build_outlier_levels(sphx_ctx* ctx, int64_t n, const double* xs, const double* ys, const double* zs);
struct KnnIn {
    const double *xs, *ys, *zs;
    const int32_t* id;
    const int32_t* inv = nullptr;
    const double* rsearch = nullptr;
    double rscale = 1.0, rbound = 0.0;
    bool hinted = false;
    bool hint_by_id = false;
    bool lag_external = false;
};
struct KnnOut {
    int32_t* nbr;
    int32_t* list64 = nullptr;
    double* dref = nullptr;
    double* h_sorted;
    int64_t* idx64;
    double* dist;
    int64_t* nontriv;
    double* h_by_id;
};
int sphx_knn(sphx_ctx* ctx, int64_t n, int k, const KnnIn& in, const KnnOut& out);
struct PrepIn {
    const double *x, *y, *z; int ps;
    const double *vx, *vy, *vz; int vs;
    const double *m, *h, *T, *mu, *gam, *ptype;
    void pos_aos(const double* p) { x = p; y = p + 1; z = p + 2; ps = 3; }
    void vel_aos(const double* v) { vx = v; vy = v + 1; vz = v + 2; vs = 3; }
};
int sphx_prep(sphx_ctx* ctx, int64_t n, const PrepIn& in, bool pairwise, hipStream_t stream);
int sphx_pass_density(sphx_ctx* ctx, int64_t n, int k, bool lean = false);
int sphx_pass_pi(sphx_ctx* ctx, int64_t n, int k, const double* h, const double* ptype);
int sphx_pass_visc(sphx_ctx* ctx, int64_t n, int k, const double* m);
int sphx_pass_visc_pw(sphx_ctx* ctx, int64_t n, int k, const double* m);
int sphx_pass_species(sphx_ctx* ctx, int64_t n, int k, int s, const double* fun, double* F);
int sphx_step_species(sphx_ctx* ctx, int64_t n, int k);
int sphx_species_on(sphx_ctx* ctx, int64_t n, int k, int S, int SP, const double* fun, const int* row_of, const double* m_sorted,
                    double* F, double* Z, double* agb);
int sphx_agb_table_set(sphx_ctx* ctx, int S, int nspl, const int32_t* ntx, const int32_t* nty, const double* tx, const double* ty,
                       const double* coeffs, const int32_t* mapto, double divisor, const double* mu_specie, double solar_mass);
int sphx_transpose_nbr(sphx_ctx* ctx, int64_t n, int k, const int64_t* nb_rowmajor);

int sphx_clamp(sphx_ctx* ctx, int64_t n, StateArrays& s);
int sphx_permute_state(sphx_ctx* ctx, int64_t n, bool split, hipEvent_t after_first);
int sphx_hsum(sphx_ctx* ctx, int64_t n, const double* h, hipStream_t stream);
int sphx_compute_dt(sphx_ctx* ctx, int first, double fixed_dt);
int sphx_integrate(sphx_ctx* ctx, int64_t n, int fold_dt = 0, int first = 0, double fixed_dt = 0.0);
int sphx_pass_drag(sphx_ctx* ctx, int64_t n, int k, const double* m, const double* ptype, const double* mgm,
                   const double* mcs);
int sphx_aos_to_soa3(sphx_ctx* ctx, int64_t n, const double* aos, double* x, double* y, double* z);
int sphx_soa3_to_aos_by_id(sphx_ctx* ctx, int64_t n, const int* id, const double* x, const double* y,
                           const double* z, double* aos);
int sphx_scatter_rows_by_id(sphx_ctx* ctx, int64_t n, int w, const int* id, const double* in, double* out);
int sphx_gather3(sphx_ctx* ctx, int64_t n, const int* perm, const double* x, const double* y,
                 const double* z, double* xs, double* ys, double* zs);
int sphx_iota(sphx_ctx* ctx, int64_t n, int* out);
int sphx_knn_refresh(sphx_ctx* ctx, int64_t n, int k, const double* x, const double* y, const double* z,
                     int32_t* nbr, double* h_sorted, int64_t* nfail_out);
int sphx_save_list_positions(sphx_ctx* ctx, int64_t n, const double* x, const double* y, const double* z);
```

### sph-code_amd/csrc/sphx_leapfrog.h

```cpp
#pragma once
#include <float.h>

__device__ __forceinline__ double sphx_dt_rule(double ct, int first, double dt_0, double max_age) {
    double dt = first ? dt_0 / 10.0 : fmax(dt_0 / 5.0, fmin(dt_0 * 2.0, ct));
    if (ct > max_age) dt = max_age / 100.0;
    return dt;
}

__device__ __forceinline__ double sphx_ct_value(bool none, double ct_min, double dt_0) {
    return none ? dt_0 / 10.0 : ct_min + 0.0001;
}

__device__ __forceinline__ double sphx_clamp_pos(double q, double lim) {
    q = (q > lim) ? lim : q;
    q = (q < -lim) ? -lim : q;
    return sphx_nan_to_num(q);
}

__device__ __forceinline__ void sphx_leapfrog_update(double dt, double x[3], double v[3], double vis[3],
                                                     const double pa[3], const double* grav, const double* old,
                                                     double tot[3]) {
    const double vn = sqrt((v[0] * v[0] + v[1] * v[1]) + v[2] * v[2]);
    const double an = sqrt((vis[0] * vis[0] + vis[1] * vis[1]) + vis[2] * vis[2]);
    if (vn - an * dt < 0.0) {
#pragma unroll
        for (int c = 0; c < 3; ++c) vis[c] = -v[c] / dt;
    }
#pragma unroll
    for (int c = 0; c < 3; ++c) {
        tot[c] = grav ? (grav[c] + pa[c]) + vis[c] : pa[c] + vis[c];
        x[c] = x[c] + ((tot[c] * (dt * dt)) / 2.0 + v[c] * dt);
        v[c] = old ? v[c] + (tot[c] + old[c]) / 2.0 * dt
                   : v[c] + tot[c] * dt;
    }
}

__device__ __forceinline__ bool sphx_finite(double v) { return v - v == 0.0; }
__device__ __forceinline__ void sphx_count_bad(unsigned long long* counters, int which, bool bad) {
    const unsigned long long m = __ballot(bad);
    if (m && (unsigned long long)__builtin_amdgcn_mbcnt_hi((unsigned)(m >> 32), __builtin_amdgcn_mbcnt_lo((unsigned)m, 0u)) == 0ull && bad) {
        const unsigned bucket = ((blockIdx.x << 2) | (threadIdx.x >> 6)) & 63u;
        atomicAdd(&counters[bucket * 16u + (unsigned)which], (unsigned long long)__popcll(m));
    }
}

__device__ __forceinline__ void sphx_energy_update(double dt, double heat, double mu, double gam, double m,
                                                   double m_h, double kB, double& E, double& T) {
    E = sphx_nan_to_num(E) + sphx_nan_to_num(heat * dt);
    T = sphx_nan_to_num(E * (mu * m_h) / (gam * m * kB));
}
```

### sph-code_amd/csrc/sphx_sums.hip

```cpp
#include "sphx_internal.h"
#include "sphx_wave.h"
#include "sphx_pair.h"
#pragma clang fp contract(off)
#include <float.h>
#include <stdlib.h>

struct PrepArgs {
    int n;
    const double *x, *y, *z; int ps;
    const double *vx, *vy, *vz; int vs;
    const double *m, *h, *T, *mu, *gam, *ptype;
    double kB, amu;
    RecA* ra; RecB* rb; RecBC* bc; RecSelf* self;
    const int* perm;
    int which, n_active;
    int pairwise;
};

__global__ __launch_bounds__(256) void prep_kernel(PrepArgs a) {
    const int t = blockIdx.x * blockDim.x + threadIdx.x;
    if (t >= a.n) return;
    const int i = a.perm ? a.perm[t] : t;
    if (a.which && ((i < a.n_active) != (a.which == 1))) return;
    const double m = a.m[i], h = a.h[i], T = a.T[i], mu = a.mu[i], gam = a.gam[i], pt = a.ptype[i];
// ... 93 lines not shown
    DensAcc acc[SPHX_SUM_PARTS] = {};
    for (int kk0 = 0; kk0 < k; kk0 += NBATCH) {
      int jb[NBATCH];
      Q4 q0b[NBATCH], q1b[NBATCH];
#pragma unroll
      for (int u = 0; u < NBATCH; ++u) jb[u] = (kk0 + u < k) ? nbr[(size_t)(kk0 + u) * npad + p] : -1;
#pragma unroll
      for (int u = 0; u < NBATCH; ++u) {
          const double* q = reinterpret_cast<const double*>(&rec[jb[u] < 0 ? i : jb[u]]);
          q0b[u] = gload4(q); q1b[u] = gload4(q + 4);
      }
#pragma unroll
      for (int u = 0; u < NBATCH; ++u) {
        if (jb[u] < 0) continue;
        density_term<SqrtLib>(acc[u & (SPHX_SUM_PARTS - 1)], q0b[u], q1b[u], xr, yr, zr, hi2, ci, Ai, clip != 0);
      }
    }
    const double s_rho = parts_total(acc, &DensAcc::rho), s_rd = parts_total(acc, &DensAcc::rd), s_n = parts_total(acc, &DensAcc::n);
    const double gx = parts_total(acc, &DensAcc::gx), gy = parts_total(acc, &DensAcc::gy), gz = parts_total(acc, &DensAcc::gz);
    rho[o] = s_rho; rhod[o] = s_rd; nden[o] = s_n;
    rho_s[i] = s_rho;
    if (G) { G[3 * (size_t)o + 0] = -gx; G[3 * (size_t)o + 1] = -gy; G[3 * (size_t)o + 2] = -gz; }
    ha[3 * (size_t)o + 0] = -gx / s_rho;
    ha[3 * (size_t)o + 1] = -gy / s_rho;
    ha[3 * (size_t)o + 2] = -gz / s_rho;
}

int sphx_pass_density(sphx_ctx* ctx, int64_t n, int k, bool lean) {
    SPHX_TRY(sphx_ensure(ctx, ctx->rho, (size_t)n * sizeof(double)));
    SPHX_TRY(sphx_ensure(ctx, ctx->rhod, (size_t)n * sizeof(double)));
    SPHX_TRY(sphx_ensure(ctx, ctx->nden, (size_t)n * sizeof(double)));
    SPHX_TRY(sphx_ensure(ctx, ctx->G, (size_t)n * 3 * sizeof(double)));
    SPHX_TRY(sphx_ensure(ctx, ctx->ha, (size_t)n * 3 * sizeof(double)));
    if (ctx->qorder && ctx->blob_lists) return sphx_blob_density(ctx, n, k, lean);
    hipLaunchKernelGGL(pass_density_kernel, dim3((unsigned)((n + 255) / 256)), dim3(256), 0, ctx->stream,
                       (int)n, (int)sphx_pad64(n), k, ctx->clip_grad, ctx->nbr.as<int>(), ctx->rec1.as<RecA>(),
                       ctx->rho_s.as<double>(), ctx->qorder, OutMap{ctx->map_perm, ctx->map_perm ? ctx->map_nactive : (int)n},
                       ctx->rho.as<double>(), ctx->rhod.as<double>(), ctx->nden.as<double>(),
                       lean ? nullptr : ctx->G.as<double>(), ctx->ha.as<double>());
    HIPCHK(hipGetLastError());
    return SPHX_OK;
}

__global__ __launch_bounds__(256) void pass_pi_kernel(int n, int npad, int k, const int* __restrict__ nbr,
                                                      const RecB* __restrict__ recb,
                                                      const double* __restrict__ rho_s,
                                                      const RecSelf* __restrict__ selfr, RecBC* bc,
                                                      const int* __restrict__ qorder, OutMap om, double* Pi, double* BwOut,
                                                      u64* ct_bits) {
    const int p = xcd_block(blockIdx.x, gridDim.x) * blockDim.x + threadIdx.x;
    u64 my_ct = SPHX_CT_NONE;
    const int i = (p < n) ? (qorder ? qorder[p] : p) : n;
    const int o = (i < n) ? out_index(om, i) : 0x7FFFFFFF;
    if (i < n && o < om.n_active) {
        int j0 = nbr[p];
        if (j0 < 0) j0 = i;
        const double* rq = reinterpret_cast<const double*>(&recb[j0]);
        const Q4 r0 = gload4(rq), rv = gload4(rq + 4);
        const RecSelf sf = selfr[i];
        const double rho_i = rho_s[i], cs_i = sf.csi, ms_i = sf.mg, h_i = sf.h;
        double a_pi[SPHX_SUM_PARTS] = {}, maxrel = 0.0;
        for (int kk0 = 0; kk0 < k; kk0 += NBATCH) {
          int jb[NBATCH];
          Q4 q0b[NBATCH], qvb[NBATCH];
          double rhob[NBATCH];
#pragma unroll
          for (int u = 0; u < NBATCH; ++u) jb[u] = (kk0 + u < k) ? nbr[(size_t)(kk0 + u) * npad + p] : -1;
#pragma unroll
          for (int u = 0; u < NBATCH; ++u) {
              const int jj = jb[u] < 0 ? i : jb[u];
              const double* qb = reinterpret_cast<const double*>(&recb[jj]);
              q0b[u] = gload4(qb); qvb[u] = gload4(qb + 4);
              rhob[u] = rho_s[jj];
          }
#pragma unroll
          for (int u = 0; u < NBATCH; ++u) {
            if (jb[u] < 0) continue;
            const PiPair t = pi_term<SqrtLib>(q0b[u], qvb[u], rhob[u], r0, rv, rho_i, cs_i);
            a_pi[u & (SPHX_SUM_PARTS - 1)] += t.pi;
            maxrel = fmax(maxrel, t.rel);
          }
        }
        const double s_pi = parts_total(a_pi);
        Pi[o] = s_pi;
        const double bw = fmax(ms_i, 0.0) * s_pi;
        bc[i].Bw = bw;
        if (BwOut) BwOut[o] = bw;
        if (ms_i > 0.0) my_ct = ct_vote_bits(h_i, maxrel);
    }
    block_min_vote<256>(my_ct, ct_bits);
}

int sphx_pass_pi(sphx_ctx* ctx, int64_t n, int k, const double* h, const double* ptype) {
    (void)ptype; (void)h;
    SPHX_TRY(sphx_ensure(ctx, ctx->Pi, (size_t)n * sizeof(double)));
    SPHX_TRY(sphx_ensure(ctx, ctx->Bw, (size_t)n * sizeof(double)));
    u64* ct = ctx->scal.as<u64>() + SC_CT_BITS;
    if (!ctx->ct_primed) SPHX_TRY(sphx_prime_ct(ctx, ct));
    ctx->ct_primed = false;
    if (ctx->qorder && ctx->blob_lists) return sphx_blob_pi(ctx, n, k, ct);
    hipLaunchKernelGGL(pass_pi_kernel, dim3((unsigned)((n + 255) / 256)), dim3(256), 0, ctx->stream,
                       (int)n, (int)sphx_pad64(n), k, ctx->nbr.as<int>(), ctx->recv.as<RecB>(),
                       ctx->rho_s.as<double>(), ctx->self_s.as<RecSelf>(), ctx->bc_s.as<RecBC>(), ctx->qorder,
                       OutMap{ctx->map_perm, ctx->map_perm ? ctx->map_nactive : (int)n},
                       ctx->Pi.as<double>(), ctx->map_perm ? ctx->Bw.as<double>() : nullptr, ct);
    HIPCHK(hipGetLastError());
    return SPHX_OK;
}

__global__ __launch_bounds__(256) void pass_visc_kernel(int n, int npad, int k, int clip,
                                                        const int* __restrict__ nbr,
                                                        const RecB* __restrict__ recb,
                                                        const RecBC* __restrict__ bc,
                                                        const int* __restrict__ qorder, OutMap om,
                                                        const double* __restrict__ m, double* va,
                                                        double* vh) {
    const int p = xcd_block(blockIdx.x, gridDim.x) * blockDim.x + threadIdx.x;
    if (p >= n) return;
    const int i = qorder ? qorder[p] : p;
    const int o = out_index(om, i);
    if (o >= om.n_active) return;
    int j0 = nbr[p];
    if (j0 < 0) j0 = i;
    const double* rq = reinterpret_cast<const double*>(&recb[j0]);
    const Q4 r0 = gload4(rq), rv = gload4(rq + 4);
    const double2 bci = *reinterpret_cast<const double2*>(&bc[i]);
    const double hi2 = recb[i].h2, ci = -6.0 * bci.y, Bi = bci.x;
    ViscAcc acc[SPHX_SUM_PARTS] = {};
    for (int kk0 = 0; kk0 < k; kk0 += NBATCH) {
      int jb[NBATCH];
      Q4 q0b[NBATCH], qvb[NBATCH];
      double2 bcb[NBATCH];
#pragma unroll
      for (int u = 0; u < NBATCH; ++u) jb[u] = (kk0 + u < k) ? nbr[(size_t)(kk0 + u) * npad + p] : -1;
#pragma unroll
      for (int u = 0; u < NBATCH; ++u) {
          const int jj = jb[u] < 0 ? i : jb[u];
          const double* qb = reinterpret_cast<const double*>(&recb[jj]);
          q0b[u] = gload4(qb); qvb[u] = gload4(qb + 4);
          bcb[u] = *reinterpret_cast<const double2*>(&bc[jj]);
      }
#pragma unroll
      for (int u = 0; u < NBATCH; ++u) {
        if (jb[u] < 0) continue;
        visc_term<SqrtLib>(acc[u & (SPHX_SUM_PARTS - 1)], q0b[u], qvb[u], bcb[u].x, bcb[u].y, r0, rv, hi2, ci, Bi, clip != 0);
      }
    }
    const double ax = parts_total(acc, &ViscAcc::x), ay = parts_total(acc, &ViscAcc::y), az = parts_total(acc, &ViscAcc::z);
    const double heat = parts_total(acc, &ViscAcc::h);
    va[3 * (size_t)o + 0] = -ax; va[3 * (size_t)o + 1] = -ay; va[3 * (size_t)o + 2] = -az;
    vh[o] = heat * m[o] / 2.0;
}

int sphx_pass_visc(sphx_ctx* ctx, int64_t n, int k, const double* m) {
    SPHX_TRY(sphx_ensure(ctx, ctx->va, (size_t)n * 3 * sizeof(double)));
    SPHX_TRY(sphx_ensure(ctx, ctx->vh, (size_t)n * sizeof(double)));
    if (ctx->qorder && ctx->blob_lists) return sphx_blob_visc(ctx, n, k, m);
    hipLaunchKernelGGL(pass_visc_kernel, dim3((unsigned)((n + 255) / 256)), dim3(256), 0, ctx->stream,
                       (int)n, (int)sphx_pad64(n), k, ctx->clip_grad, ctx->nbr.as<int>(), ctx->recv.as<RecB>(),
                       ctx->bc_s.as<RecBC>(), ctx->qorder,
                       OutMap{ctx->map_perm, ctx->map_perm ? ctx->map_nactive : (int)n}, m,
                       ctx->va.as<double>(), ctx->vh.as<double>());
    HIPCHK(hipGetLastError());
    return SPHX_OK;
}

__global__ __launch_bounds__(256) void pass_visc_pw_kernel(int n, int npad, int k, int clip,
                                                           const int* __restrict__ nbr,
                                                           const RecB* __restrict__ recb,
                                                           const double* __restrict__ rho_s,
                                                           const RecBC* __restrict__ bc,
                                                           const RecSelf* __restrict__ selfr,
                                                           const int* __restrict__ qorder, OutMap om,
                                                           const double* __restrict__ m, double* va, double* vh,
                                                           u64* ct_bits) {
    const int p = xcd_block(blockIdx.x, gridDim.x) * blockDim.x + threadIdx.x;
    u64 my_ct = SPHX_CT_NONE;
    const int i = (p < n) ? (qorder ? qorder[p] : p) : n;
    const int o = (i < n) ? out_index(om, i) : 0x7FFFFFFF;
    if (i < n && o < om.n_active) {
        int j0 = nbr[p];
        if (j0 < 0) j0 = i;
        const double* rq = reinterpret_cast<const double*>(&recb[j0]);
        const Q4 r0 = gload4(rq), rv = gload4(rq + 4);
        const RecSelf sf = selfr[i];
        const double rho_i = rho_s[i], cs_i = sf.csi, h_i = sf.h;
        const double hi2 = recb[i].h2, ci = -6.0 * bc[i].Bw;
        ViscAcc acc[SPHX_SUM_PARTS] = {};
        double maxrel = 0.0;
        for (int kk0 = 0; kk0 < k; kk0 += NBATCH) {
          int jb[NBATCH];
          Q4 q0b[NBATCH], qvb[NBATCH];
          double rhob[NBATCH], mcb[NBATCH];
#pragma unroll
          for (int u = 0; u < NBATCH; ++u) jb[u] = (kk0 + u < k) ? nbr[(size_t)(kk0 + u) * npad + p] : -1;
#pragma unroll
          for (int u = 0; u < NBATCH; ++u) {
              const int jj = jb[u] < 0 ? i : jb[u];
              const double* qb = reinterpret_cast<const double*>(&recb[jj]);
              q0b[u] = gload4(qb); qvb[u] = gload4(qb + 4);
              rhob[u] = rho_s[jj];
              mcb[u] = bc[jj].Bw;
          }
#pragma unroll
          for (int u = 0; u < NBATCH; ++u) {
            if (jb[u] < 0) continue;
            maxrel = fmax(maxrel, visc_pw_term<SqrtLib>(acc[u & (SPHX_SUM_PARTS - 1)], q0b[u], qvb[u], rhob[u], mcb[u], r0, rv,
                                                         rho_i, cs_i, hi2, ci, clip != 0));
          }
        }
        const double ax = parts_total(acc, &ViscAcc::x), ay = parts_total(acc, &ViscAcc::y), az = parts_total(acc, &ViscAcc::z);
        const double heat = parts_total(acc, &ViscAcc::h);
        va[3 * (size_t)o + 0] = -ax; va[3 * (size_t)o + 1] = -ay; va[3 * (size_t)o + 2] = -az;
        vh[o] = heat * m[o] / 2.0;
        if (sf.mg > 0.0) my_ct = ct_vote_bits(h_i, maxrel);
    }
    block_min_vote<256>(my_ct, ct_bits);
}

int sphx_pass_visc_pw(sphx_ctx* ctx, int64_t n, int k, const double* m) {
    SPHX_TRY(sphx_ensure(ctx, ctx->va, (size_t)n * 3 * sizeof(double)));
    SPHX_TRY(sphx_ensure(ctx, ctx->vh, (size_t)n * sizeof(double)));
    u64* ct = ctx->scal.as<u64>() + SC_CT_BITS;
    if (!ctx->ct_primed) SPHX_TRY(sphx_prime_ct(ctx, ct));
    ctx->ct_primed = false;
    if (ctx->qorder && ctx->blob_lists) return sphx_blob_visc_pw(ctx, n, k, m, ct);
    hipLaunchKernelGGL(pass_visc_pw_kernel, dim3((unsigned)((n + 255) / 256)), dim3(256), 0, ctx->stream,
                       (int)n, (int)sphx_pad64(n), k, ctx->clip_grad, ctx->nbr.as<int>(), ctx->recv.as<RecB>(),
                       ctx->rho_s.as<double>(), ctx->bc_s.as<RecBC>(), ctx->self_s.as<RecSelf>(), ctx->qorder,
                       OutMap{ctx->map_perm, ctx->map_perm ? ctx->map_nactive : (int)n}, m,
                       ctx->va.as<double>(), ctx->vh.as<double>(), ct);
    HIPCHK(hipGetLastError());
    return SPHX_OK;
}

__global__ __launch_bounds__(256) void drag_count_kernel(int n, int npad, int k, const int* __restrict__ nbr,
                                                         const double* __restrict__ ptype, const int* __restrict__ qorder,
                                                         int* cnt) {
    const int p = blockIdx.x * blockDim.x + threadIdx.x;
    if (p >= n) return;
    const int i = qorder ? qorder[p] : p;
    for (int kk = 0; kk < k; ++kk) {
        const int j = nbr[(size_t)kk * npad + p];
        if (j >= 0 && j != i && ptype[j] == 2.0) atomicAdd(&cnt[j], 1);
    }
}
#define DRAG_RED_BLOCKS 2048
#define DRAG_RED_U 4
template <int U>
__device__ __forceinline__ void drag_slice_sum(int s, int L, const DragEntry* __restrict__ ent,
                                               double* pk, int lane, double& acc) {
    u64 key[U];
    double vx[U], vy[U], vz[U];
    int rank[U];
#pragma unroll
    for (int u = 0; u < U; ++u) {
        const int q = lane + 64 * u;
        key[u] = ~0ull; vx[u] = vy[u] = vz[u] = 0.0;
        if (q < L) {
            const double2* e = reinterpret_cast<const double2*>(ent + s + q);
            const double2 e0 = e[0], e1 = e[1];
            key[u] = (u64)__double_as_longlong(e0.x); vx[u] = e0.y; vy[u] = e1.x; vz[u] = e1.y;
        }
        rank[u] = 0;
    }
#pragma unroll
    for (int c = 0; c < U; ++c) {
        const int lc = L - 64 * c < 64 ? L - 64 * c : 64;
        for (int t = 0; t < lc; ++t) {
            const u64 kt = ((u64)(unsigned)__builtin_amdgcn_readlane((int)(key[c] >> 32), t) << 32) |
                           (u64)(unsigned)__builtin_amdgcn_readlane((int)key[c], t);
#pragma unroll
            for (int u = 0; u < U; ++u) rank[u] += kt < key[u] ? 1 : 0;
        }
    }
#pragma unroll
    for (int u = 0; u < U; ++u) {
        const int q = lane + 64 * u;
        if (q < L) { pk[3 * rank[u]] = vx[u]; pk[3 * rank[u] + 1] = vy[u]; pk[3 * rank[u] + 2] = vz[u]; }
    }
    wave_sync();
    if (lane < 3) {
        int t = 0;
        for (; t + 8 <= L; t += 8) {
            double v[8];
#pragma unroll
            for (int q = 0; q < 8; ++q) v[q] = pk[3 * (t + q) + lane];
#pragma unroll
            for (int q = 0; q < 8; ++q) acc += v[q];
        }
        for (; t < L; ++t) acc += pk[3 * t + lane];
    }
    wave_sync();
}
__global__ __launch_bounds__(256) void drag_reduce_kernel(int n, const int* __restrict__ start,
                                                          const DragEntry* __restrict__ ent, double* react) {
    __shared__ double parked[4][64 * DRAG_RED_U * 3];
    const int lane = threadIdx.x & 63, wave = threadIdx.x >> 6;
    double* pk = parked[wave];
    for (int j0 = (blockIdx.x * 4 + wave) * 64; j0 < n; j0 += gridDim.x * 4 * 64) {
        const int jl = j0 + lane;
        int sl = 0, Ll = 0;
        if (jl < n) { sl = start[jl]; Ll = start[jl + 1] - sl; }
        if (jl < n && Ll == 0) { react[3 * (size_t)jl] = 0.0; react[3 * (size_t)jl + 1] = 0.0; react[3 * (size_t)jl + 2] = 0.0; }
        u64 todo = __builtin_amdgcn_ballot_w64(Ll > 0);
        while (todo) {
            const int t = __builtin_ctzll(todo);
            todo &= todo - 1;
            const int s = __builtin_amdgcn_readlane(sl, t), L = __builtin_amdgcn_readlane(Ll, t);
            const int j = j0 + t;
// ... 230 lines not shown
```

### sph-code_amd/sim.py

```python
import ctypes as C
import logging

import numpy as np

from . import _lib
from ._lib import dp, f64
from .compat import visc_mode_code

log = logging.getLogger("sph_code_amd")


class Simulation:
    def __init__(self, state, n_neigh=40, dist=None, device=None, with_species=False, ctx=None,
                 incremental=False, with_drag=False, gravity=None, G=6.67430e-11, clip_grad=False,
                 forms="hydro_update", d=None, gravity_order=2, agb=None, visc_mode="ref_axis0"):
        vmode = visc_mode_code(visc_mode)
        if vmode and forms == "loop":
            raise ValueError("visc_mode='pairwise' is for forms='hydro_update': the loop forms' viscosity is pairwise already")
        self.ctx = ctx if ctx is not None else _lib.Context(device)
        self.ctx.set_incremental(incremental)
        self.k = int(n_neigh)
        self.dist = 0.0 if dist is None or not np.isfinite(dist) else float(dist)
        self.first = True
        pts = f64(state["points"])
        n = pts.shape[0]
        self.n = n
        vel = f64(state["velocities"], (n, 3))
        fu = f64(state["f_un"]) if (with_species and state.get("f_un") is not None) else None
        acc = state.get("total_accel")
        acc = f64(acc, (n, 3)) if acc is not None else None
        c = self.ctx
        c.check(c.lib.sphx_state_upload(
            c.h, n, 0 if fu is None else fu.shape[1], dp(pts), dp(vel), dp(f64(state["mass"], (n,))),
            dp(f64(state["particle_type"], (n,))), dp(fu), dp(f64(state["T"], (n,))),
            dp(f64(state["mu_array"], (n,))), dp(f64(state["gamma_array"], (n,))),
            dp(f64(state["E_internal"], (n,))), dp(acc)))
        c.check(c.lib.sphx_set_clip_grad(c.h, 1 if clip_grad else 0))
        c.check(c.lib.sphx_set_visc_mode(c.h, vmode))
        if forms not in ("hydro_update", "loop"):
            raise ValueError("forms must be 'hydro_update' or 'loop'")
        if forms == "loop":
            if d is None:
                raise ValueError("forms='loop' needs the driver's global d (code_running.py:67-68)")
            c.check(c.lib.sphx_state_set_loop_forms(c.h, 1, float(d)))
        if gravity is not None:
            if gravity not in ("direct", "tree"):
                raise ValueError("gravity must be None, 'direct' or 'tree'")
            c.check(c.lib.sphx_state_set_gravity(c.h, 1 if gravity == "direct" else 2, float(G)))
            c.check(c.lib.sphx_set_gravity_order(c.h, int(gravity_order)))
        self.n_species = 0 if fu is None else fu.shape[1]
        if agb is not None:
            if fu is None:
                raise ValueError("agb needs with_species=True and a state with f_un")
            from . import compat
            splines, mapto, divisor = agb
            i32 = lambda a: np.ascontiguousarray(a, dtype=np.int32)
            ntx = i32([sp.get_knots()[0].size for sp in splines]); nty = i32([sp.get_knots()[1].size for sp in splines])
            cat = lambda parts: np.ascontiguousarray(np.concatenate([np.asarray(q, dtype=np.float64).ravel() for q in parts]))
            tx = cat([sp.get_knots()[0] for sp in splines]); ty = cat([sp.get_knots()[1] for sp in splines])
            cf = cat([sp.get_coeffs() for sp in splines]); mp = i32(mapto)
            mu = np.ascontiguousarray(compat.mu_specie[:self.n_species], dtype=np.float64)
            p32 = lambda a: a.ctypes.data_as(C.POINTER(C.c_int32))
            c.check(c.lib.sphx_state_set_agb(c.h, len(splines), p32(ntx), p32(nty), dp(tx), dp(ty), dp(cf), p32(mp),
                                             float(divisor), dp(mu), compat.solar_mass))
        self.has_agb = agb is not None
        if with_drag:
            from . import compat
            fu_all = f64(state["f_un"])
            mgm = np.ascontiguousarray(np.sum(compat.grain_mass() * fu_all, axis=1))
            mcs = np.ascontiguousarray(np.sum(compat.sigma_effective() * fu_all, axis=1))
            c.check(c.lib.sphx_state_set_drag(c.h, dp(mgm), dp(mcs)))

    def step(self, nsteps=1, fixed_dt=0.0):
        c = self.ctx
        c.check(c.lib.sphx_step(c.h, int(nsteps), self.k, self.dist, 1 if self.first else 0, float(fixed_dt)))
        self.first = False
        self._log_failures()

    FAILURE_COUNTERS = ("bad_accel", "bad_energy", "bad_state", "bad_h", "short_rows")

    def failures(self):
        st = self.ctx.stats()
        return {k_: int(st[k_]) for k_ in self.FAILURE_COUNTERS}

    def _log_failures(self):
        f = self.failures()
        seen = getattr(self, "_failures_seen", None) or dict.fromkeys(self.FAILURE_COUNTERS, 0)
        new = {k_: f[k_] - seen.get(k_, 0) for k_ in f if f[k_] > seen.get(k_, 0)}
        self._failures_seen = f
        if new:
            log.warning("sphx step: non-finite values met (particles): %s  [cumulative: %s]", new, f)

    def download(self):
        n = self.n
        out = dict(points=np.empty((n, 3)), velocities=np.empty((n, 3)), total_accel=np.empty((n, 3)),
                   E_internal=np.empty(n), T=np.empty(n), sizes=np.empty(n), densities=np.empty(n),
                   num_densities=np.empty(n), visc_heat=np.empty(n))
        dt = C.c_double(0.0)
        c = self.ctx
        c.check(c.lib.sphx_state_download(
            c.h, dp(out["points"]), dp(out["velocities"]), dp(out["total_accel"]), dp(out["E_internal"]),
            dp(out["T"]), dp(out["sizes"]), dp(out["densities"]), dp(out["num_densities"]),
            dp(out["visc_heat"]), C.cast(C.byref(dt), _lib.c_double_p)))
        out["dt"] = dt.value
        out["pressure"] = np.empty(n)
        c.check(c.lib.sphx_state_download_pressure(c.h, dp(out["pressure"])))
        return out

    def download_species(self):
        n, S = self.n, self.n_species
        if S < 1:
            raise RuntimeError("the simulation carries no composition (with_species=True and a state with f_un)")
        out = dict(f_un_neighbor=np.empty((S, n)))
        Z = A = None
        if self.has_agb:
            out["metallicity"] = Z = np.empty(n)
            out["agb_dust"] = A = np.empty((n, S))
        c = self.ctx
        c.check(c.lib.sphx_state_download_species(c.h, dp(out["f_un_neighbor"]), dp(Z), dp(A)))
        return out

    def snapshot(self, path, state):
        d = self.download()
        out = dict(points=d["points"], velocities=d["velocities"], total_accel=d["total_accel"],
                   E_internal=d["E_internal"], T=d["T"], sizes=d["sizes"], dt=np.float64(d["dt"]),
                   first=np.int64(1 if self.first else 0), n_neigh=np.int64(self.k), dist=np.float64(self.dist))
        for key in ("mass", "particle_type", "mu_array", "gamma_array"):
            out[key] = np.asarray(state[key], dtype=np.float64)
        if state.get("f_un") is not None:
            out["f_un"] = np.asarray(state["f_un"], dtype=np.float64)
        np.savez(path, **out)

    @classmethod
    def from_snapshot(cls, path, device=None, **kw):
        z = dict(np.load(path, allow_pickle=False))
        state = {k_: z[k_] for k_ in ("points", "velocities", "total_accel", "E_internal", "T", "mass",
                                       "particle_type", "mu_array", "gamma_array")}
        state["f_un"] = z.get("f_un")
        sim = cls(state, n_neigh=int(z["n_neigh"]), dist=float(z["dist"]), device=device, **kw)
        sim.first = bool(int(z["first"]))
        return sim, state

    def diagnostics(self, state):
        d = self.download()
        m = np.asarray(state["mass"], dtype=np.float64)
        mt = m.sum()
        return dict(net_accel=(d["total_accel"] * m[:, None]).sum(axis=0) / mt,
                    momentum=(d["velocities"] * m[:, None]).sum(axis=0),
                    kinetic=0.5 * float((m * (d["velocities"] ** 2).sum(axis=1)).sum()),
                    internal=float(d["E_internal"].sum()), dt=d["dt"])

    def stats(self):
        return self.ctx.stats()

    def reset_stats(self):
        self.ctx.reset_stats()
        self._failures_seen = None
```

Baseline: 821.6 million.

## Fuse leapfrog integrate update into blob viscosity kernel epilogue

Adds an UPDATE template variant of the blob viscosity kernel. Once a particle's viscous acceleration and heat are reduced, the same kernel runs the per-particle leapfrog and energy update and writes dt. The separate integrate kernel is skipped when this path is taken, which saves a launch and a re-read of va/vh and the state arrays. The path is gated on several conditions: qorder, LDS, blob lists, no map_perm, no gravity and no drag. The visc kernel gains register pressure and extra global traffic in its epilogue, which may lower occupancy.

```diff
diff --git a/include/sphx.h b/include/sphx.h
--- a/include/sphx.h
+++ b/include/sphx.h
@@ -152,6 +152,7 @@
 int sphx_state_set_gravity(sphx_ctx* ctx, int mode, double G);
 int sphx_set_gravity_order(sphx_ctx* ctx, int order);
 int sphx_step(sphx_ctx* ctx, int nsteps, int k, double dist, int first, double fixed_dt);
+int sphx_last_step_fused_update(const sphx_ctx* ctx);
 int sphx_state_download(sphx_ctx* ctx, double* pos, double* vel, double* accel,
                         double* E_internal, double* T, double* sizes, double* rho,
                         double* nden, double* visc_heat, double* dt_last);
diff --git a/sph-code_amd/_lib.py b/sph-code_amd/_lib.py
--- a/sph-code_amd/_lib.py
+++ b/sph-code_amd/_lib.py
@@ -41,6 +41,7 @@
     "sphx_version": (C.c_int, []),
     "sphx_build_info": (C.c_char_p, []),
     "sphx_tunables": (C.c_char_p, [_P]),
+    "sphx_last_step_fused_update": (C.c_int, [_P]),
     "sphx_selftest_scan": (C.c_int, [_P, C.c_int, C.c_uint, C.POINTER(C.c_longlong), C.POINTER(C.c_int)]),
     "sphx_selftest_mfma_cull": (C.c_int, [_P, C.c_double, C.c_int, C.c_uint, _D, _D, _D]),
     "sphx_host_alloc": (C.c_int, [C.POINTER(_P), C.c_size_t]),
@@ -266,6 +267,9 @@
         return {"library": self.lib.sphx_build_info().decode(), "tunables": self.lib.sphx_tunables(self.h).decode(),
                 "lib_path": LIB_PATH}
 
+    def last_step_fused_update(self):
+        return bool(self.lib.sphx_last_step_fused_update(self.h))
+
     def set_timing_detail(self, on=True):
         self.check(self.lib.sphx_set_timing_detail(self.h, 1 if on else 0))
 
diff --git a/sph-code_amd/csrc/sphx_api.hip b/sph-code_amd/csrc/sphx_api.hip
--- a/sph-code_amd/csrc/sphx_api.hip
+++ b/sph-code_amd/csrc/sphx_api.hip
@@ -53,6 +53,7 @@
 
 extern "C" const char* sphx_build_info(void) { return "gfx950 experiments=0"; }
 extern "C" const char* sphx_tunables(const sphx_ctx* ctx) { return ctx ? ctx->tunables : ""; }
+extern "C" int sphx_last_step_fused_update(const sphx_ctx* ctx) { return ctx && ctx->step_fused_update ? 1 : 0; }
 
 extern "C" int sphx_host_alloc(void** out, size_t bytes) {
     if (!out) return SPHX_E_ARG;
@@ -123,6 +124,7 @@
     if (const char* e = env("SPHX_GRAV_ORDER")) { int v = atoi(e); if (v == 1 || v == 2) ctx->grav_order = v; }
     if (const char* e = env("SPHX_GRAV_WS")) { int v = atoi(e); if (v >= 1 && v <= 4) ctx->grav_ws = v; }
     if (const char* e = env("SPHX_LDS")) ctx->use_lds = atoi(e) != 0;
+    if (const char* e = env("SPHX_FUSE_UPDATE")) ctx->fuse_update = atoi(e) != 0;
     if (const char* e = env("SPHX_BLOB_SLOTS")) ctx->blob_slots = atoi(e);
     if (const char* e = env("SPHX_BLOB_WGS")) {
         int cus = 256;
@@ -570,7 +572,7 @@
     return SPHX_OK;
 }
 
-static int step_sums(sphx_ctx* ctx, int k, hipEvent_t* ev, hipEvent_t search_end, bool detail) {
+static int step_sums(sphx_ctx* ctx, int k, hipEvent_t* ev, hipEvent_t search_end, bool detail, int first, double fixed_dt) {
     const int64_t n = ctx->n;
     StateArrays& s = ctx->st;
     const bool pairwise = ctx->visc_mode == 1 && !ctx->loop_forms;
@@ -624,7 +626,15 @@
         } else {
             SPHX_TRY(sphx_pass_pi(ctx, n, k, s.hprev.as<double>(), s.ptype.as<double>()));
             if (detail) HIPCHK(hipEventRecord(ev[5], ctx->stream));
-            SPHX_TRY(sphx_pass_visc(ctx, n, k, s.m.as<double>()));
+            if (ctx->fuse_update && ctx->qorder && ctx->use_lds && ctx->blob_lists && !ctx->map_perm && !ctx->gravity && !ctx->drag) {
+                IntegArgs upd;
+                SPHX_TRY(sphx_integrate_args(ctx, n, 1, first, fixed_dt, &upd));
+                SPHX_TRY(sphx_pass_visc(ctx, n, k, s.m.as<double>(), &upd));
+                sphx_integrate_done(ctx);
+                ctx->step_fused_update = true;
+            } else {
+                SPHX_TRY(sphx_pass_visc(ctx, n, k, s.m.as<double>()));
+            }
         }
     }
     if (ctx->drag)
@@ -649,7 +659,8 @@
     if (rec0) HIPCHK(hipEventRecord(ev[0], ctx->stream));
     SPHX_TRY(step_search(ctx, k, dist, ev));
     HIPCHK(hipEventRecord(ev[2], ctx->stream));
-    SPHX_TRY(step_sums(ctx, k, ev, ev[2], detail));
+    ctx->step_fused_update = false;
+    SPHX_TRY(step_sums(ctx, k, ev, ev[2], detail, first, fixed_dt));
     if (detail) HIPCHK(hipEventRecord(ev[6], ctx->stream));
     StateArrays& s = ctx->st;
     if (ctx->gravity) {
@@ -665,7 +676,7 @@
                                               ctx->grav.as<double>()));
     }
     if (detail) HIPCHK(hipEventRecord(ev[8], ctx->stream));
-    SPHX_TRY(sphx_integrate(ctx, n, 1, first, fixed_dt));
+    if (!ctx->step_fused_update) SPHX_TRY(sphx_integrate(ctx, n, 1, first, fixed_dt));
     if (rec7) HIPCHK(hipEventRecord(ev[7], ctx->stream));
     ctx->step_count++;
     return SPHX_OK;
diff --git a/sph-code_amd/csrc/sphx_blob.hip b/sph-code_amd/csrc/sphx_blob.hip
--- a/sph-code_amd/csrc/sphx_blob.hip
+++ b/sph-code_amd/csrc/sphx_blob.hip
@@ -4,6 +4,7 @@
 #include <float.h>
 #include <stdlib.h>
 #include <stdio.h>
+#include "sphx_leapfrog.h"
 
 #define DD_TAB 2048
 #define DD_PROBES 64
@@ -404,6 +405,9 @@
     }
 }
 
+template <bool UPDATE> struct UpdArg { IntegArgs a; };
+template <> struct UpdArg<false> { int none; };
+template <bool UPDATE>
 __global__ __launch_bounds__(PASS_T, PASS_MINW) void blob_visc_kernel(int n, int npad, int k, int nblk,
                                                            const int* __restrict__ nbr,
                                                            const u16* __restrict__ slot16,
@@ -413,7 +417,7 @@
                                                            const RecB* __restrict__ recb,
                                                            const RecBC* __restrict__ bc,
                                                            const double* __restrict__ m, double* va, double* vh,
-                                                           BlobSel sel) {
+                                                           BlobSel sel, UpdArg<UPDATE> upd) {
     extern __shared__ double2 img[];
     double* lc1 = reinterpret_cast<double*>(img + 4 * BLOB_S);
     u16* tile = reinterpret_cast<u16*>(lc1 + BLOB_S);
@@ -460,8 +464,15 @@
             }
             const double ax = group_total(a.x), ay = group_total(a.y), az = group_total(a.z), heat = group_total(a.h);
             if (!half) {
-                va[3 * (size_t)o + 0] = -ax; va[3 * (size_t)o + 1] = -ay; va[3 * (size_t)o + 2] = -az;
-                vh[o] = heat * mi / 2.0;
+                const double va3[3] = {-ax, -ay, -az};
+                const double vhi = heat * mi / 2.0;
+                va[3 * (size_t)o + 0] = va3[0]; va[3 * (size_t)o + 1] = va3[1]; va[3 * (size_t)o + 2] = va3[2];
+                vh[o] = vhi;
+                if constexpr (UPDATE) {
+                    const double dt = sphx_update_dt(upd.a);
+                    if (i == 0) *upd.a.dt_out = dt;
+                    sphx_particle_update<true>(upd.a, i, dt, va3, vhi);
+                }
             }
         }
         __syncthreads();
@@ -933,10 +944,16 @@
                        ctx->map_perm ? ctx->Bw.as<double>() : nullptr, ct_bits, sphx_blob_sel(ctx, ctx->pass_part));
 }
 
-int sphx_blob_visc(sphx_ctx* ctx, int64_t n, int k, const double* m) {
-    return blob_launch(ctx, blob_visc_kernel, 72, 0, n, k, ctx->clip_grad, ctx->map_perm, blob_n_active(ctx, n),
+int sphx_blob_visc(sphx_ctx* ctx, int64_t n, int k, const double* m, const IntegArgs* upd) {
+    if (upd) {
+        if (ctx->map_perm) return sphx_set_err(ctx, SPHX_E_STATE, "sphx_blob_visc: the update epilogue needs the state's own order");
+        return blob_launch(ctx, blob_visc_kernel<true>, 72, 0, n, k, ctx->clip_grad, ctx->map_perm, blob_n_active(ctx, n),
+                           ctx->recv.as<RecB>(), ctx->bc_s.as<RecBC>(), m, ctx->va.as<double>(), ctx->vh.as<double>(),
+                           sphx_blob_sel(ctx, ctx->pass_part), UpdArg<true>{*upd});
+    }
+    return blob_launch(ctx, blob_visc_kernel<false>, 72, 0, n, k, ctx->clip_grad, ctx->map_perm, blob_n_active(ctx, n),
                        ctx->recv.as<RecB>(), ctx->bc_s.as<RecBC>(), m, ctx->va.as<double>(), ctx->vh.as<double>(),
-                       sphx_blob_sel(ctx, ctx->pass_part));
+                       sphx_blob_sel(ctx, ctx->pass_part), UpdArg<false>{0});
 }
 
 int sphx_blob_visc_pw(sphx_ctx* ctx, int64_t n, int k, const double* m, u64* ct_bits) {
diff --git a/sph-code_amd/csrc/sphx_integrate.hip b/sph-code_amd/csrc/sphx_integrate.hip
--- a/sph-code_amd/csrc/sphx_integrate.hip
+++ b/sph-code_amd/csrc/sphx_integrate.hip
@@ -210,93 +210,18 @@
     return SPHX_OK;
 }
 
-struct IntegArgs {
-    int n;
-    double *x, *y, *z, *vx, *vy, *vz, *ax, *ay, *az;
-    double *E, *T;
-    const double *m, *mu, *gam, *ptype;
-    const double *ha, *va, *vh;
-    const double *rho, *rhod, *drag_on, *drag_re;
-    const double* grav;
-    const double* G;
-    const double* dt;
-    double m_h, kB;
-    int no_old;
-    const u64* ct_bits;
-    double* dt_out;
-    int first;
-    double fixed_dt, dt_0, max_age;
-    u64* counters;
-};
 __global__ __launch_bounds__(256) void integrate_kernel(IntegArgs a) {
     int i = blockIdx.x * blockDim.x + threadIdx.x;
     if (i >= a.n) return;
-    double dt;
-    if (a.ct_bits) {
-        if (a.fixed_dt > 0.0) {
-            dt = a.fixed_dt;
-        } else {
-            const u64 b = *a.ct_bits;
-            const double ct = sphx_ct_value(b == SPHX_CT_NONE, __longlong_as_double((long long)b), a.dt_0);
-            dt = sphx_dt_rule(ct, a.first, a.dt_0, a.max_age);
-        }
-        if (i == 0) *a.dt_out = dt;
-    } else {
-        dt = *a.dt;
-    }
-    const double g = (a.ptype[i] == 0.0) ? 1.0 : 0.0;
-    const double v[3] = {a.vx[i], a.vy[i], a.vz[i]};
-    double pa[3], vis[3];
-    bool bad_acc = false;
-#pragma unroll
-    for (int c = 0; c < 3; ++c) {
-        if (a.G) {
-            const double praw = a.G[3 * (size_t)i + c] / a.rho[i] * g;
-            pa[c] = nan_to_num(praw);
-            vis[c] = a.va[3 * (size_t)i + c];
-            bad_acc = bad_acc || !sphx_finite(praw) || !sphx_finite(vis[c]);
-        } else {
-            const double praw = -a.ha[3 * (size_t)i + c] * g, vraw = -a.va[3 * (size_t)i + c] * g;
-            pa[c] = nan_to_num(praw);
-            vis[c] = nan_to_num(vraw);
-            bad_acc = bad_acc || !sphx_finite(praw) || !sphx_finite(vraw);
-        }
-        if (a.drag_on) {
-            const double draw = a.drag_on[3 * (size_t)i + c] * a.rhod[i] / a.rho[i] * g, rraw = a.drag_re[3 * (size_t)i + c];
-            const double dg = nan_to_num(draw);
-            vis[c] = dg + nan_to_num(rraw) + vis[c];
-            bad_acc = bad_acc || !sphx_finite(draw) || !sphx_finite(rraw);
-        }
-    }
-    double x[3] = {a.x[i], a.y[i], a.z[i]};
-    double vv[3] = {v[0], v[1], v[2]};
-    double gr[3], old[3], tot[3];
-#pragma unroll
-    for (int c = 0; c < 3; ++c) gr[c] = a.grav ? a.grav[3 * (size_t)i + c] : 0.0;
-    old[0] = a.ax[i]; old[1] = a.ay[i]; old[2] = a.az[i];
-    sphx_leapfrog_update(dt, x, vv, vis, pa, a.grav ? gr : nullptr, a.no_old ? nullptr : old, tot);
-    a.x[i] = x[0]; a.y[i] = x[1]; a.z[i] = x[2];
-    a.vx[i] = vv[0]; a.vy[i] = vv[1]; a.vz[i] = vv[2];
-    a.ax[i] = tot[0]; a.ay[i] = tot[1]; a.az[i] = tot[2];
-    double E = a.E[i], T;
-    const double heat = a.vh[i];
-    const bool bad_en = !sphx_finite(E) || !sphx_finite(heat * dt);
-    sphx_energy_update(dt, heat, a.mu[i], a.gam[i], a.m[i], a.m_h, a.kB, E, T);
-    a.E[i] = E;
-    a.T[i] = T;
-    if (a.counters) {
-        bool bad_st = false;
-#pragma unroll
-        for (int c = 0; c < 3; ++c) bad_st = bad_st || !sphx_finite(x[c]) || !sphx_finite(vv[c]);
-        sphx_count_bad(a.counters, BAD_ACCEL, bad_acc);
-        sphx_count_bad(a.counters, BAD_ENERGY, bad_en);
-        sphx_count_bad(a.counters, BAD_STATE, bad_st);
-    }
-}
-
-int sphx_integrate(sphx_ctx* ctx, int64_t n, int fold_dt, int first, double fixed_dt) {
+    const double dt = sphx_update_dt(a);
+    if (a.ct_bits && i == 0) *a.dt_out = dt;
+    const double va3[3] = {a.va[3 * (size_t)i + 0], a.va[3 * (size_t)i + 1], a.va[3 * (size_t)i + 2]};
+    sphx_particle_update<false>(a, i, dt, va3, a.vh[i]);
+}
+
+int sphx_integrate_args(sphx_ctx* ctx, int64_t n, int fold_dt, int first, double fixed_dt, IntegArgs* out) {
     StateArrays& s = ctx->st;
-    IntegArgs a;
+    IntegArgs& a = *out;
     a.ct_bits = fold_dt ? ctx->scal.as<u64>() + SC_CT_BITS : nullptr;
     a.dt_out = ctx->scal.as<double>() + SC_DT;
     a.first = first; a.fixed_dt = fixed_dt; a.dt_0 = ctx->cst.dt_0; a.max_age = ctx->cst.max_age;
@@ -308,6 +233,8 @@
     a.E = s.E.as<double>(); a.T = ctx->alt.T.as<double>();
     a.m = s.m.as<double>(); a.mu = s.mu.as<double>(); a.gam = s.gam.as<double>();
     a.ptype = s.ptype.as<double>();
+    SPHX_TRY(sphx_ensure(ctx, ctx->va, (size_t)n * 3 * sizeof(double)));
+    SPHX_TRY(sphx_ensure(ctx, ctx->vh, (size_t)n * sizeof(double)));
     a.ha = ctx->ha.as<double>(); a.va = ctx->va.as<double>(); a.vh = ctx->vh.as<double>();
     a.rho = ctx->rho.as<double>(); a.rhod = ctx->rhod.as<double>();
     a.drag_on = ctx->drag ? ctx->drag_on.as<double>() : nullptr;
@@ -318,10 +245,20 @@
     a.m_h = ctx->cst.m_h; a.kB = ctx->cst.k_B;
     a.no_old = 0;
     a.counters = ctx->badc.as<u64>();
+    return SPHX_OK;
+}
+
+void sphx_integrate_done(sphx_ctx* ctx) {
+    { DevBuf t = ctx->st.T; ctx->st.T = ctx->alt.T; ctx->alt.T = t; }
+    ctx->tprev_valid = true;
+}
+
+int sphx_integrate(sphx_ctx* ctx, int64_t n, int fold_dt, int first, double fixed_dt) {
+    IntegArgs a;
+    SPHX_TRY(sphx_integrate_args(ctx, n, fold_dt, first, fixed_dt, &a));
     hipLaunchKernelGGL(integrate_kernel, dim3((unsigned)((n + 255) / 256)), dim3(256), 0, ctx->stream, a);
     HIPCHK(hipGetLastError());
-    { DevBuf t = s.T; s.T = ctx->alt.T; ctx->alt.T = t; }
-    ctx->tprev_valid = true;
+    sphx_integrate_done(ctx);
     return SPHX_OK;
 }
 
diff --git a/sph-code_amd/csrc/sphx_internal.h b/sph-code_amd/csrc/sphx_internal.h
--- a/sph-code_amd/csrc/sphx_internal.h
+++ b/sph-code_amd/csrc/sphx_internal.h
@@ -130,6 +130,7 @@
     int blob_curve = 0;
     bool use_group = true;
     bool use_lds = true;
+    bool fuse_update = true;
     bool drag_lds = true;
     bool blob_split_on = true;
     bool species_lds = true;
@@ -168,6 +169,7 @@
     int64_t step_count = 0;
     double dt_last = 0.0;
     bool tprev_valid = false;
+    bool step_fused_update = false;
     bool ct_primed = false;
     bool recs_pw = false;
     bool nbr_api_valid = false;
@@ -345,6 +347,7 @@
 };
 int sphx_badc_read(sphx_ctx* ctx);
 
+struct IntegArgs;
 int sphx_bbox(sphx_ctx* ctx, int64_t n, const double* x, const double* y, const double* z,
               double out_minmax[13], bool use_clip);
 int sphx_median(sphx_ctx* ctx, int64_t n, const double* v, double* out_dev);
@@ -370,7 +373,7 @@
                               const double* m_sorted, double* F, double* Z, double* agb, int agb_on);
 int sphx_blob_density(sphx_ctx* ctx, int64_t n, int k, bool lean);
 int sphx_blob_pi(sphx_ctx* ctx, int64_t n, int k, u64* ct_bits);
-int sphx_blob_visc(sphx_ctx* ctx, int64_t n, int k, const double* m);
+int sphx_blob_visc(sphx_ctx* ctx, int64_t n, int k, const double* m, const IntegArgs* upd);
 int sphx_blob_visc_pw(sphx_ctx* ctx, int64_t n, int k, const double* m, u64* ct_bits);
 int sphx_blob_species(sphx_ctx* ctx, int64_t n, int k, int S, const double* fun, const int* row_of, const double* m_sorted, double* F,
                       double* Z, double* agb, int agb_on);
@@ -427,7 +430,7 @@
 int sphx_prep(sphx_ctx* ctx, int64_t n, const PrepIn& in, bool pairwise, hipStream_t stream);
 int sphx_pass_density(sphx_ctx* ctx, int64_t n, int k, bool lean = false);
 int sphx_pass_pi(sphx_ctx* ctx, int64_t n, int k, const double* h, const double* ptype);
-int sphx_pass_visc(sphx_ctx* ctx, int64_t n, int k, const double* m);
+int sphx_pass_visc(sphx_ctx* ctx, int64_t n, int k, const double* m, const IntegArgs* upd = nullptr);
 int sphx_pass_visc_pw(sphx_ctx* ctx, int64_t n, int k, const double* m);
 int sphx_pass_species(sphx_ctx* ctx, int64_t n, int k, int s, const double* fun, double* F);
 int sphx_step_species(sphx_ctx* ctx, int64_t n, int k);
@@ -437,11 +440,31 @@
                        const double* coeffs, const int32_t* mapto, double divisor, const double* mu_specie, double solar_mass);
 int sphx_transpose_nbr(sphx_ctx* ctx, int64_t n, int k, const int64_t* nb_rowmajor);
 
+struct IntegArgs {
+    int n;
+    double *x, *y, *z, *vx, *vy, *vz, *ax, *ay, *az;
+    double *E, *T;
+    const double *m, *mu, *gam, *ptype;
+    const double *ha, *va, *vh;
+    const double *rho, *rhod, *drag_on, *drag_re;
+    const double* grav;
+    const double* G;
+    const double* dt;
+    double m_h, kB;
+    int no_old;
+    const u64* ct_bits;
+    double* dt_out;
+    int first;
+    double fixed_dt, dt_0, max_age;
+    u64* counters;
+};
 int sphx_clamp(sphx_ctx* ctx, int64_t n, StateArrays& s);
 int sphx_permute_state(sphx_ctx* ctx, int64_t n, bool split, hipEvent_t after_first);
 int sphx_hsum(sphx_ctx* ctx, int64_t n, const double* h, hipStream_t stream);
 int sphx_compute_dt(sphx_ctx* ctx, int first, double fixed_dt);
 int sphx_integrate(sphx_ctx* ctx, int64_t n, int fold_dt = 0, int first = 0, double fixed_dt = 0.0);
+int sphx_integrate_args(sphx_ctx* ctx, int64_t n, int fold_dt, int first, double fixed_dt, IntegArgs* out);
+void sphx_integrate_done(sphx_ctx* ctx);
 int sphx_pass_drag(sphx_ctx* ctx, int64_t n, int k, const double* m, const double* ptype, const double* mgm,
                    const double* mcs);
 int sphx_aos_to_soa3(sphx_ctx* ctx, int64_t n, const double* aos, double* x, double* y, double* z);
diff --git a/sph-code_amd/csrc/sphx_leapfrog.h b/sph-code_amd/csrc/sphx_leapfrog.h
--- a/sph-code_amd/csrc/sphx_leapfrog.h
+++ b/sph-code_amd/csrc/sphx_leapfrog.h
@@ -49,3 +49,62 @@
     E = sphx_nan_to_num(E) + sphx_nan_to_num(heat * dt);
     T = sphx_nan_to_num(E * (mu * m_h) / (gam * m * kB));
 }
+
+__device__ __forceinline__ double sphx_update_dt(const IntegArgs& a) {
+    if (!a.ct_bits) return *a.dt;
+    if (a.fixed_dt > 0.0) return a.fixed_dt;
+    const u64 b = *a.ct_bits;
+    const double ct = sphx_ct_value(b == SPHX_CT_NONE, __longlong_as_double((long long)b), a.dt_0);
+    return sphx_dt_rule(ct, a.first, a.dt_0, a.max_age);
+}
+template <bool PLAIN>
+__device__ __forceinline__ void sphx_particle_update(const IntegArgs& a, int i, double dt, const double (&va3)[3], double heat) {
+    const double g = (a.ptype[i] == 0.0) ? 1.0 : 0.0;
+    const double v[3] = {a.vx[i], a.vy[i], a.vz[i]};
+    double pa[3], vis[3];
+    bool bad_acc = false;
+#pragma unroll
+    for (int c = 0; c < 3; ++c) {
+        if (!PLAIN && a.G) {
+            const double praw = a.G[3 * (size_t)i + c] / a.rho[i] * g;
+            pa[c] = sphx_nan_to_num(praw);
+            vis[c] = va3[c];
+            bad_acc = bad_acc || !sphx_finite(praw) || !sphx_finite(vis[c]);
+        } else {
+            const double praw = -a.ha[3 * (size_t)i + c] * g, vraw = -va3[c] * g;
+            pa[c] = sphx_nan_to_num(praw);
+            vis[c] = sphx_nan_to_num(vraw);
+            bad_acc = bad_acc || !sphx_finite(praw) || !sphx_finite(vraw);
+        }
+        if (!PLAIN && a.drag_on) {
+            const double draw = a.drag_on[3 * (size_t)i + c] * a.rhod[i] / a.rho[i] * g, rraw = a.drag_re[3 * (size_t)i + c];
+            const double dg = sphx_nan_to_num(draw);
+            vis[c] = dg + sphx_nan_to_num(rraw) + vis[c];
+            bad_acc = bad_acc || !sphx_finite(draw) || !sphx_finite(rraw);
+        }
+    }
+    double x[3] = {a.x[i], a.y[i], a.z[i]};
+    double vv[3] = {v[0], v[1], v[2]};
+    double gr[3], old[3], tot[3];
+    const bool grav = !PLAIN && a.grav;
+#pragma unroll
+    for (int c = 0; c < 3; ++c) gr[c] = grav ? a.grav[3 * (size_t)i + c] : 0.0;
+    old[0] = a.ax[i]; old[1] = a.ay[i]; old[2] = a.az[i];
+    sphx_leapfrog_update(dt, x, vv, vis, pa, grav ? gr : nullptr, (PLAIN || !a.no_old) ? old : nullptr, tot);
+    a.x[i] = x[0]; a.y[i] = x[1]; a.z[i] = x[2];
+    a.vx[i] = vv[0]; a.vy[i] = vv[1]; a.vz[i] = vv[2];
+    a.ax[i] = tot[0]; a.ay[i] = tot[1]; a.az[i] = tot[2];
+    double E = a.E[i], T;
+    const bool bad_en = !sphx_finite(E) || !sphx_finite(heat * dt);
+    sphx_energy_update(dt, heat, a.mu[i], a.gam[i], a.m[i], a.m_h, a.kB, E, T);
+    a.E[i] = E;
+    a.T[i] = T;
+    if (a.counters) {
+        bool bad_st = false;
+#pragma unroll
+        for (int c = 0; c < 3; ++c) bad_st = bad_st || !sphx_finite(x[c]) || !sphx_finite(vv[c]);
+        sphx_count_bad(a.counters, BAD_ACCEL, bad_acc);
+        sphx_count_bad(a.counters, BAD_ENERGY, bad_en);
+        sphx_count_bad(a.counters, BAD_STATE, bad_st);
+    }
+}
diff --git a/sph-code_amd/csrc/sphx_sums.hip b/sph-code_amd/csrc/sphx_sums.hip
--- a/sph-code_amd/csrc/sphx_sums.hip
+++ b/sph-code_amd/csrc/sphx_sums.hip
@@ -269,10 +269,11 @@
     vh[o] = heat * m[o] / 2.0;
 }
 
-int sphx_pass_visc(sphx_ctx* ctx, int64_t n, int k, const double* m) {
+int sphx_pass_visc(sphx_ctx* ctx, int64_t n, int k, const double* m, const IntegArgs* upd) {
     SPHX_TRY(sphx_ensure(ctx, ctx->va, (size_t)n * 3 * sizeof(double)));
     SPHX_TRY(sphx_ensure(ctx, ctx->vh, (size_t)n * sizeof(double)));
-    if (ctx->qorder && ctx->blob_lists) return sphx_blob_visc(ctx, n, k, m);
+    if (ctx->qorder && ctx->blob_lists) return sphx_blob_visc(ctx, n, k, m, upd);
+    if (upd) return sphx_set_err(ctx, SPHX_E_STATE, "sphx_pass_visc: the update epilogue exists on the LDS path only");
     hipLaunchKernelGGL(pass_visc_kernel, dim3((unsigned)((n + 255) / 256)), dim3(256), 0, ctx->stream,
                        (int)n, (int)sphx_pad64(n), k, ctx->clip_grad, ctx->nbr.as<int>(), ctx->recv.as<RecB>(),
                        ctx->bc_s.as<RecBC>(), ctx->qorder,
diff --git a/sph-code_amd/sim.py b/sph-code_amd/sim.py
--- a/sph-code_amd/sim.py
+++ b/sph-code_amd/sim.py
@@ -153,6 +153,9 @@
     def stats(self):
         return self.ctx.stats()
 
+    def last_step_fused_update(self):
+        return self.ctx.last_step_fused_update()
+
     def reset_stats(self):
         self.ctx.reset_stats()
         self._failures_seen = None
```

New measurement: 756.7 million. 0.921x the previous value.
